# kernel-matrix-benchmarks/kernel-matrix-benchmarks

Hardware: AMD Instinct MI355X
Metric: point-pair interactions/s (N*M/s) + max |err| vs scipy, D=3 Gaussian (higher is better)
Workload: dtype f32

## Files before the change

include/kmvp.h:

```cpp
#ifndef KMVP_H
#define KMVP_H

#include <stdint.h>

#ifdef __cplusplus
extern "C" {
#endif

#define KMVP_ABI_VERSION 1

enum kmvp_status {
  KMVP_OK = 0,
  KMVP_E_INVALID = 1,
  KMVP_E_UNSUPPORTED = 2,
  KMVP_E_DEVICE = 3,
  KMVP_E_COMM = 4,
  KMVP_E_NOMEM = 5,
  KMVP_E_NOT_CONVERGED = 6
};

enum kmvp_dtype {
  KMVP_F32 = 0,
  KMVP_F64 = 1,
  KMVP_BF16 = 2
};

typedef struct kmvp_ctx kmvp_ctx;

int kmvp_abi_version(void);
int kmvp_device_count(void);

kmvp_ctx* kmvp_create(int device, int* status);
void kmvp_destroy(kmvp_ctx* ctx);
const char* kmvp_last_error(const kmvp_ctx* ctx);

int kmvp_set_points(kmvp_ctx* ctx, const void* y, int64_t M, const void* x_or_null, int64_t N,
                    int D, int dtype, int64_t j_offset, int64_t M_total);

int kmvp_fit(kmvp_ctx* ctx, int kernel);

int kmvp_set_signal(kmvp_ctx* ctx, const void* b_or_null, int E);

int kmvp_gaussian(kmvp_ctx* ctx);
int kmvp_gaussian_norm(kmvp_ctx* ctx);
int kmvp_absexp(kmvp_ctx* ctx);
int kmvp_absexp_norm(kmvp_ctx* ctx);
int kmvp_invdist(kmvp_ctx* ctx);
int kmvp_invdist_norm(kmvp_ctx* ctx);
int kmvp_expdot(kmvp_ctx* ctx);
int kmvp_expdot_norm(kmvp_ctx* ctx);
int kmvp_matern32(kmvp_ctx* ctx);
int kmvp_matern32_norm(kmvp_ctx* ctx);
int kmvp_matern52(kmvp_ctx* ctx);
int kmvp_matern52_norm(kmvp_ctx* ctx);

int kmvp_gaussian_grad(kmvp_ctx* ctx);
int kmvp_absexp_grad(kmvp_ctx* ctx);
int kmvp_invdist_grad(kmvp_ctx* ctx);
int kmvp_matern32_grad(kmvp_ctx* ctx);
int kmvp_matern52_grad(kmvp_ctx* ctx);

int kmvp_gaussian_dscale(kmvp_ctx* ctx);
int kmvp_absexp_dscale(kmvp_ctx* ctx);
int kmvp_matern32_dscale(kmvp_ctx* ctx);
int kmvp_matern52_dscale(kmvp_ctx* ctx);

int kmvp_gaussian_logsumexp(kmvp_ctx* ctx);
int kmvp_absexp_logsumexp(kmvp_ctx* ctx);

int kmvp_gaussian_logsumexp_grad(kmvp_ctx* ctx);
int kmvp_absexp_logsumexp_grad(kmvp_ctx* ctx);

int kmvp_nearest(kmvp_ctx* ctx, int K, int exclude_self, int64_t* out_idx, double* out_sqdist);

int kmvp_set_batches(kmvp_ctx* ctx, int B, const int64_t* y_offsets, const int64_t* x_offsets_or_null);

int kmvp_kmeans(kmvp_ctx* ctx, int C, const double* weights_or_null, double tol, int maxit, double* centroids,
                int64_t* labels, double* cluster_weight_or_null, int* iters, double* inertia, double* shift);

int kmvp_gaussian_meanshift(kmvp_ctx* ctx, double tol, int maxit, double* modes, int* iters, double* step2, int* sweeps,
                            int64_t* target_sweeps);

int kmvp_get_result(kmvp_ctx* ctx, double* out, int64_t out_len);

int kmvp_gaussian_cg_solve(kmvp_ctx* ctx, const void* a, int E, double rtol, int maxit,
                           double* out_b, int* iters, double* resid);
int kmvp_absexp_cg_solve(kmvp_ctx* ctx, const void* a, int E, double rtol, int maxit,
                         double* out_b, int* iters, double* resid);
int kmvp_matern32_cg_solve(kmvp_ctx* ctx, const void* a, int E, double rtol, int maxit,
                           double* out_b, int* iters, double* resid);
int kmvp_matern52_cg_solve(kmvp_ctx* ctx, const void* a, int E, double rtol, int maxit,
                           double* out_b, int* iters, double* resid);
int kmvp_invdist_minres_solve(kmvp_ctx* ctx, const void* a, int E, double rtol, int maxit,
                              double* out_b, int* iters, double* resid);

int kmvp_gaussian_lanczos_quadrature(kmvp_ctx* ctx, const void* z, int P, double rtol, int maxit, double* logquad,
                                     double* invquad, int* steps, double* x_or_null, double* alpha_or_null,
                                     double* beta_or_null);
int kmvp_absexp_lanczos_quadrature(kmvp_ctx* ctx, const void* z, int P, double rtol, int maxit, double* logquad,
                                   double* invquad, int* steps, double* x_or_null, double* alpha_or_null,
                                   double* beta_or_null);
int kmvp_matern32_lanczos_quadrature(kmvp_ctx* ctx, const void* z, int P, double rtol, int maxit, double* logquad,
                                     double* invquad, int* steps, double* x_or_null, double* alpha_or_null,
                                     double* beta_or_null);
int kmvp_matern52_lanczos_quadrature(kmvp_ctx* ctx, const void* z, int P, double rtol, int maxit, double* logquad,
                                     double* invquad, int* steps, double* x_or_null, double* alpha_or_null,
                                     double* beta_or_null);

int kmvp_gaussian_sinkhorn(kmvp_ctx* ctx, const double* log_a_or_null, const double* log_b_or_null, double tol, int maxit,
                           double* u, double* v, int* iters, double* err);
int kmvp_absexp_sinkhorn(kmvp_ctx* ctx, const double* log_a_or_null, const double* log_b_or_null, double tol, int maxit,
                         double* u, double* v, int* iters, double* err);

int kmvp_set_solver_diagonal(kmvp_ctx* ctx, const double* d_or_null, int64_t n, double ridge);

#define KMVP_PRECOND_MAX_RANK 128
int kmvp_set_solver_preconditioner(kmvp_ctx* ctx, int rank);
int kmvp_get_solver_preconditioner(kmvp_ctx* ctx, int* rank_built, int64_t* pivots_or_null, double* factor_or_null);
double kmvp_last_preconditioner_ms(const kmvp_ctx* ctx);

int kmvp_gaussian_lanczos_quadrature_precond(kmvp_ctx* ctx, const double* g, const double* h, int P, double rtol, int maxit,
                                             double* logdet_p, double* logquad, double* invquad, double* wnorm2, int* steps,
                                             double* x_or_null, double* pz_or_null, double* alpha_or_null,
                                             double* beta_or_null);
int kmvp_absexp_lanczos_quadrature_precond(kmvp_ctx* ctx, const double* g, const double* h, int P, double rtol, int maxit,
                                           double* logdet_p, double* logquad, double* invquad, double* wnorm2, int* steps,
                                           double* x_or_null, double* pz_or_null, double* alpha_or_null,
                                           double* beta_or_null);
int kmvp_matern32_lanczos_quadrature_precond(kmvp_ctx* ctx, const double* g, const double* h, int P, double rtol, int maxit,
                                             double* logdet_p, double* logquad, double* invquad, double* wnorm2, int* steps,
                                             double* x_or_null, double* pz_or_null, double* alpha_or_null,
                                             double* beta_or_null);
int kmvp_matern52_lanczos_quadrature_precond(kmvp_ctx* ctx, const double* g, const double* h, int P, double rtol, int maxit,
                                             double* logdet_p, double* logquad, double* invquad, double* wnorm2, int* steps,
                                             double* x_or_null, double* pz_or_null, double* alpha_or_null,
                                             double* beta_or_null);

enum kmvp_eig_operator { KMVP_EIG_KERNEL = 0, KMVP_EIG_CENTERED = 1, KMVP_EIG_NORMALIZED = 2 };
int kmvp_gaussian_eigsh(kmvp_ctx* ctx, int k, int op, const double* v0, double tol, int maxit, double* eigenvalues,
                        double* eigenvectors, double* resid, int* steps, double* alpha_or_null, double* beta_or_null,
                        double* degree_or_null);
int kmvp_absexp_eigsh(kmvp_ctx* ctx, int k, int op, const double* v0, double tol, int maxit, double* eigenvalues,
                      double* eigenvectors, double* resid, int* steps, double* alpha_or_null, double* beta_or_null,
                      double* degree_or_null);
int kmvp_matern32_eigsh(kmvp_ctx* ctx, int k, int op, const double* v0, double tol, int maxit, double* eigenvalues,
                        double* eigenvectors, double* resid, int* steps, double* alpha_or_null, double* beta_or_null,
                        double* degree_or_null);
int kmvp_matern52_eigsh(kmvp_ctx* ctx, int k, int op, const double* v0, double tol, int maxit, double* eigenvalues,
                        double* eigenvectors, double* resid, int* steps, double* alpha_or_null, double* beta_or_null,
                        double* degree_or_null);

#define KMVP_UNIQUE_ID_BYTES 128
int kmvp_comm_get_unique_id(void* id128);
int kmvp_comm_init(kmvp_ctx* ctx, const void* id128, int rank, int world);
int kmvp_comm_world(const kmvp_ctx* ctx);
int kmvp_comm_rank(const kmvp_ctx* ctx);
enum kmvp_reduce_op { KMVP_OP_SUM = 0, KMVP_OP_MIN = 1 };
typedef int (*kmvp_host_allreduce_fn)(void* user, double* buf, int64_t count, int op);
int kmvp_comm_init_host(kmvp_ctx* ctx, kmvp_host_allreduce_fn fn, void* user, int rank, int world);

int kmvp_set_option(kmvp_ctx* ctx, const char* key, int64_t value);

int64_t kmvp_device_bytes(const kmvp_ctx* ctx);
double kmvp_last_kernel_ms(const kmvp_ctx* ctx);
double kmvp_last_total_ms(const kmvp_ctx* ctx);
double kmvp_last_allreduce_ms(const kmvp_ctx* ctx);
const char* kmvp_last_kernel_name(const kmvp_ctx* ctx);
const char* kmvp_last_dispatch_note(const kmvp_ctx* ctx);


int kmvp_cell_layout(kmvp_ctx* ctx, int64_t* info, double* sigma_b, int32_t* source_cell, int32_t* target_cell,
                     double* source_centres, int64_t source_cap, double* target_centres, int64_t target_cap);

#ifdef __cplusplus
}
#endif
#endif
```

kernel_matrix_benchmarks_amd/_lib.py:

```python
import ctypes
import os

import numpy as np

_HERE = os.path.dirname(os.path.abspath(__file__))
LIB_PATH = os.environ.get("KMVP_LIB", os.path.join(_HERE, "libkmvp.so"))

KMVP_F32, KMVP_F64, KMVP_BF16 = 0, 1, 2
STATUS = {
    0: "OK", 1: "INVALID", 2: "UNSUPPORTED", 3: "DEVICE", 4: "COMM", 5: "NOMEM", 6: "NOT_CONVERGED",
}
UNIQUE_ID_BYTES = 128

_c = ctypes
SYMBOLS = [
    ("kmvp_abi_version", _c.c_int, []),
    ("kmvp_device_count", _c.c_int, []),
    ("kmvp_create", _c.c_void_p, [_c.c_int, _c.POINTER(_c.c_int)]),
    ("kmvp_destroy", None, [_c.c_void_p]),
    ("kmvp_last_error", _c.c_char_p, [_c.c_void_p]),
    ("kmvp_set_points", _c.c_int, [_c.c_void_p, _c.c_void_p, _c.c_int64, _c.c_void_p, _c.c_int64,
                                   _c.c_int, _c.c_int, _c.c_int64, _c.c_int64]),
    ("kmvp_fit", _c.c_int, [_c.c_void_p, _c.c_int]),
    ("kmvp_set_signal", _c.c_int, [_c.c_void_p, _c.c_void_p, _c.c_int]),
    ("kmvp_gaussian", _c.c_int, [_c.c_void_p]),
    ("kmvp_gaussian_norm", _c.c_int, [_c.c_void_p]),
    ("kmvp_absexp", _c.c_int, [_c.c_void_p]),
    ("kmvp_absexp_norm", _c.c_int, [_c.c_void_p]),
    ("kmvp_invdist", _c.c_int, [_c.c_void_p]),
    ("kmvp_invdist_norm", _c.c_int, [_c.c_void_p]),
    ("kmvp_expdot", _c.c_int, [_c.c_void_p]),
    ("kmvp_expdot_norm", _c.c_int, [_c.c_void_p]),
    ("kmvp_matern32", _c.c_int, [_c.c_void_p]),
    ("kmvp_matern32_norm", _c.c_int, [_c.c_void_p]),
    ("kmvp_matern52", _c.c_int, [_c.c_void_p]),
    ("kmvp_matern52_norm", _c.c_int, [_c.c_void_p]),
    ("kmvp_gaussian_grad", _c.c_int, [_c.c_void_p]),
    ("kmvp_absexp_grad", _c.c_int, [_c.c_void_p]),
    ("kmvp_invdist_grad", _c.c_int, [_c.c_void_p]),
    ("kmvp_matern32_grad", _c.c_int, [_c.c_void_p]),
    ("kmvp_matern52_grad", _c.c_int, [_c.c_void_p]),
    ("kmvp_gaussian_dscale", _c.c_int, [_c.c_void_p]),
    ("kmvp_absexp_dscale", _c.c_int, [_c.c_void_p]),
    ("kmvp_matern32_dscale", _c.c_int, [_c.c_void_p]),
    ("kmvp_matern52_dscale", _c.c_int, [_c.c_void_p]),
    ("kmvp_gaussian_logsumexp", _c.c_int, [_c.c_void_p]),
    ("kmvp_absexp_logsumexp", _c.c_int, [_c.c_void_p]),
    ("kmvp_gaussian_logsumexp_grad", _c.c_int, [_c.c_void_p]),
    ("kmvp_absexp_logsumexp_grad", _c.c_int, [_c.c_void_p]),
    ("kmvp_nearest", _c.c_int, [_c.c_void_p, _c.c_int, _c.c_int, _c.c_void_p, _c.c_void_p]),
    ("kmvp_set_batches", _c.c_int, [_c.c_void_p, _c.c_int, _c.c_void_p, _c.c_void_p]),
    ("kmvp_kmeans", _c.c_int, [_c.c_void_p, _c.c_int, _c.c_void_p, _c.c_double, _c.c_int, _c.c_void_p, _c.c_void_p,
                               _c.c_void_p, _c.POINTER(_c.c_int), _c.POINTER(_c.c_double), _c.POINTER(_c.c_double)]),
    ("kmvp_gaussian_meanshift", _c.c_int, [_c.c_void_p, _c.c_double, _c.c_int, _c.c_void_p, _c.c_void_p, _c.c_void_p,
                                           _c.POINTER(_c.c_int), _c.POINTER(_c.c_int64)]),
    ("kmvp_get_result", _c.c_int, [_c.c_void_p, _c.c_void_p, _c.c_int64]),
    ("kmvp_gaussian_cg_solve", _c.c_int, [_c.c_void_p, _c.c_void_p, _c.c_int, _c.c_double, _c.c_int,
                                          _c.c_void_p, _c.POINTER(_c.c_int), _c.POINTER(_c.c_double)]),
    ("kmvp_absexp_cg_solve", _c.c_int, [_c.c_void_p, _c.c_void_p, _c.c_int, _c.c_double, _c.c_int,
                                        _c.c_void_p, _c.POINTER(_c.c_int), _c.POINTER(_c.c_double)]),
    ("kmvp_matern32_cg_solve", _c.c_int, [_c.c_void_p, _c.c_void_p, _c.c_int, _c.c_double, _c.c_int,
                                          _c.c_void_p, _c.POINTER(_c.c_int), _c.POINTER(_c.c_double)]),
    ("kmvp_matern52_cg_solve", _c.c_int, [_c.c_void_p, _c.c_void_p, _c.c_int, _c.c_double, _c.c_int,
                                          _c.c_void_p, _c.POINTER(_c.c_int), _c.POINTER(_c.c_double)]),
    ("kmvp_invdist_minres_solve", _c.c_int, [_c.c_void_p, _c.c_void_p, _c.c_int, _c.c_double, _c.c_int,
                                             _c.c_void_p, _c.POINTER(_c.c_int), _c.POINTER(_c.c_double)]),
    ("kmvp_gaussian_lanczos_quadrature", _c.c_int, [_c.c_void_p, _c.c_void_p, _c.c_int, _c.c_double, _c.c_int] + [_c.c_void_p] * 6),
    ("kmvp_absexp_lanczos_quadrature", _c.c_int, [_c.c_void_p, _c.c_void_p, _c.c_int, _c.c_double, _c.c_int] + [_c.c_void_p] * 6),
    ("kmvp_matern32_lanczos_quadrature", _c.c_int, [_c.c_void_p, _c.c_void_p, _c.c_int, _c.c_double, _c.c_int] + [_c.c_void_p] * 6),
    ("kmvp_matern52_lanczos_quadrature", _c.c_int, [_c.c_void_p, _c.c_void_p, _c.c_int, _c.c_double, _c.c_int] + [_c.c_void_p] * 6),
    ("kmvp_gaussian_eigsh", _c.c_int, [_c.c_void_p, _c.c_int, _c.c_int, _c.c_void_p, _c.c_double, _c.c_int] + [_c.c_void_p] * 7),
    ("kmvp_absexp_eigsh", _c.c_int, [_c.c_void_p, _c.c_int, _c.c_int, _c.c_void_p, _c.c_double, _c.c_int] + [_c.c_void_p] * 7),
    ("kmvp_matern32_eigsh", _c.c_int, [_c.c_void_p, _c.c_int, _c.c_int, _c.c_void_p, _c.c_double, _c.c_int] + [_c.c_void_p] * 7),
    ("kmvp_matern52_eigsh", _c.c_int, [_c.c_void_p, _c.c_int, _c.c_int, _c.c_void_p, _c.c_double, _c.c_int] + [_c.c_void_p] * 7),
    ("kmvp_gaussian_lanczos_quadrature_precond", _c.c_int, [_c.c_void_p, _c.c_void_p, _c.c_void_p, _c.c_int, _c.c_double, _c.c_int] + [_c.c_void_p] * 9),
    ("kmvp_absexp_lanczos_quadrature_precond", _c.c_int, [_c.c_void_p, _c.c_void_p, _c.c_void_p, _c.c_int, _c.c_double, _c.c_int] + [_c.c_void_p] * 9),
    ("kmvp_matern32_lanczos_quadrature_precond", _c.c_int, [_c.c_void_p, _c.c_void_p, _c.c_void_p, _c.c_int, _c.c_double, _c.c_int] + [_c.c_void_p] * 9),
    ("kmvp_matern52_lanczos_quadrature_precond", _c.c_int, [_c.c_void_p, _c.c_void_p, _c.c_void_p, _c.c_int, _c.c_double, _c.c_int] + [_c.c_void_p] * 9),
    ("kmvp_gaussian_sinkhorn", _c.c_int, [_c.c_void_p, _c.c_void_p, _c.c_void_p, _c.c_double, _c.c_int, _c.c_void_p,
                                          _c.c_void_p, _c.POINTER(_c.c_int), _c.POINTER(_c.c_double)]),
    ("kmvp_absexp_sinkhorn", _c.c_int, [_c.c_void_p, _c.c_void_p, _c.c_void_p, _c.c_double, _c.c_int, _c.c_void_p,
                                        _c.c_void_p, _c.POINTER(_c.c_int), _c.POINTER(_c.c_double)]),
    ("kmvp_set_solver_diagonal", _c.c_int, [_c.c_void_p, _c.c_void_p, _c.c_int64, _c.c_double]),
    ("kmvp_set_solver_preconditioner", _c.c_int, [_c.c_void_p, _c.c_int]),
    ("kmvp_get_solver_preconditioner", _c.c_int, [_c.c_void_p, _c.POINTER(_c.c_int), _c.c_void_p, _c.c_void_p]),
    ("kmvp_last_preconditioner_ms", _c.c_double, [_c.c_void_p]),
    ("kmvp_comm_get_unique_id", _c.c_int, [_c.c_void_p]),
    ("kmvp_comm_init", _c.c_int, [_c.c_void_p, _c.c_void_p, _c.c_int, _c.c_int]),
    ("kmvp_comm_init_host", _c.c_int, [_c.c_void_p, _c.c_void_p, _c.c_void_p, _c.c_int, _c.c_int]),
    ("kmvp_comm_world", _c.c_int, [_c.c_void_p]),
    ("kmvp_comm_rank", _c.c_int, [_c.c_void_p]),
    ("kmvp_last_allreduce_ms", _c.c_double, [_c.c_void_p]),
    ("kmvp_set_option", _c.c_int, [_c.c_void_p, _c.c_char_p, _c.c_int64]),
    ("kmvp_device_bytes", _c.c_int64, [_c.c_void_p]),
    ("kmvp_last_kernel_ms", _c.c_double, [_c.c_void_p]),
    ("kmvp_last_total_ms", _c.c_double, [_c.c_void_p]),
    ("kmvp_cell_layout", _c.c_int, [_c.c_void_p, _c.c_void_p, _c.POINTER(_c.c_double), _c.c_void_p, _c.c_void_p, _c.c_void_p,
                                    _c.c_int64, _c.c_void_p, _c.c_int64]),
    ("kmvp_last_kernel_name", _c.c_char_p, [_c.c_void_p]),
    ("kmvp_last_dispatch_note", _c.c_char_p, [_c.c_void_p]),
]

HOST_ALLREDUCE_FN = _c.CFUNCTYPE(_c.c_int, _c.c_void_p, _c.POINTER(_c.c_double), _c.c_int64, _c.c_int)
OP_SUM, OP_MIN = 0, 1
FIT_CODES = {"gaussian": 0, "absolute-exponential": 1, "inverse-distance": 2, "matern-3/2": 3, "matern-5/2": 4}

EIG_OPERATORS = {"kernel": 0, "centered": 1, "normalized": 2}

_lib = None


class KmvpError(RuntimeError):
    def __init__(self, code, message):
        super().__init__(f"libkmvp: {STATUS.get(code, code)}: {message}")
        self.code = code


def load():
    global _lib
    if _lib is None:
        if not os.path.exists(LIB_PATH):
            raise ImportError(
                f"{LIB_PATH} is missing: build it with `python -c 'import __graft_entry__ as g; g.build()'` "
                "(or make -C kernel_matrix_benchmarks_amd/csrc).  There is no CPU fallback."
            )
        lib = ctypes.CDLL(LIB_PATH)
        for name, restype, argtypes in SYMBOLS:
            fn = getattr(lib, name)
            fn.restype = restype
            fn.argtypes = argtypes
        _lib = lib
    return _lib


def dtype_code(precision):
    if isinstance(precision, str) and precision.lower() in ("bfloat16", "bf16"):
        return KMVP_BF16, np.dtype(np.float32)
    dt = np.dtype(precision)
    if dt == np.float16:
        return KMVP_F32, np.dtype(np.float32)
    if dt == np.float64:
        return KMVP_F64, dt
    if dt == np.float32:
        return KMVP_F32, dt
    raise NotImplementedError(f"precision {precision!r} is not supported by the MI355X backend")


def input_rounding(precision):
    if isinstance(precision, str) and precision.lower() in ("bfloat16", "bf16"):
        return None
    return np.dtype(np.float16) if np.dtype(precision) == np.float16 else None


def batch_offsets(offsets, what, total=None):
    a = np.asarray(offsets)
    if a.ndim != 1 or a.size < 2:
        raise ValueError(f"{what} has shape {a.shape}, expected B + 1 offsets (B >= 1) in one dimension")
    if not np.issubdtype(a.dtype, np.integer):
        raise ValueError(f"{what} has dtype {a.dtype}, expected integers")
    a = np.ascontiguousarray(a, dtype=np.int64)
    if total is not None and (a[0] != 0 or np.any(np.diff(a) < 0) or a[-1] != total):
        raise ValueError(f"{what} must be non-decreasing from 0 to {total}")
    return a


class Context:

    def __init__(self, device=0):
        self._lib = load()
        status = ctypes.c_int(0)
        self._ctx = self._lib.kmvp_create(int(device), ctypes.byref(status))
        if not self._ctx:
            msg = self._lib.kmvp_last_error(None)
            raise KmvpError(status.value, msg.decode() if msg else "kmvp_create failed")
        self.device = int(device)
        self.comm_world = 0

    def _check(self, rc):
        if rc != 0:
            msg = self._lib.kmvp_last_error(self._ctx)
            raise KmvpError(rc, msg.decode() if msg else "")

    def close(self):
        if getattr(self, "_ctx", None):
            self._lib.kmvp_destroy(self._ctx)
            self._ctx = None

    def __del__(self):
        try:
            self.close()
        except Exception:
            pass

    def set_points(self, y, x, dtype_code_, j_offset=0, M_total=None):
        M, D = y.shape
        N = M if x is None else x.shape[0]
        if x is not None and x.shape[1] != D:
            raise ValueError(f"target points have {x.shape[1]} coordinates, source points {D}")
        self.M, self.N, self.D = M, N, D
        self._check(self._lib.kmvp_set_points(
            self._ctx, y.ctypes.data, M, None if x is None else x.ctypes.data, N, D, dtype_code_,
            int(j_offset), int(M if M_total is None else M_total)))

    def set_batches(self, y_offsets, x_offsets=None):
        if y_offsets is None:
            if x_offsets is not None:
                raise ValueError("target offsets without source offsets")
            self._check(self._lib.kmvp_set_batches(self._ctx, 0, None, None))
            return
        y_offsets = batch_offsets(y_offsets, "source_batches")
        if x_offsets is not None:
            x_offsets = batch_offsets(x_offsets, "target_batches")
            if x_offsets.size != y_offsets.size:
                raise ValueError(f"target_batches has {x_offsets.size} offsets, source_batches {y_offsets.size}: both hold B + 1")
        self._check(self._lib.kmvp_set_batches(self._ctx, y_offsets.size - 1, y_offsets.ctypes.data,
                                               None if x_offsets is None else x_offsets.ctypes.data))

    def fit(self, kernel):
        self._check(self._lib.kmvp_fit(self._ctx, FIT_CODES[kernel]))

    def set_signal(self, b):
        if b is None:
            self._check(self._lib.kmvp_set_signal(self._ctx, None, 1))
        else:
            if b.ndim != 2 or b.shape[0] != getattr(self, "M", b.shape[0]):
                raise ValueError(f"source_signal has shape {b.shape}, expected ({getattr(self, 'M', '?')}, E): one row per "
                                 "source point")
            self._check(self._lib.kmvp_set_signal(self._ctx, b.ctypes.data, b.shape[1]))

    def run(self, kernel, normalize_rows):
        entry = {
            ("gaussian", False): self._lib.kmvp_gaussian,
            ("gaussian", True): self._lib.kmvp_gaussian_norm,
            ("absolute-exponential", False): self._lib.kmvp_absexp,
            ("absolute-exponential", True): self._lib.kmvp_absexp_norm,
            ("inverse-distance", False): self._lib.kmvp_invdist,
            ("inverse-distance", True): self._lib.kmvp_invdist_norm,
            ("exp-dot", False): self._lib.kmvp_expdot,
            ("exp-dot", True): self._lib.kmvp_expdot_norm,
            ("matern-3/2", False): self._lib.kmvp_matern32,
            ("matern-3/2", True): self._lib.kmvp_matern32_norm,
            ("matern-5/2", False): self._lib.kmvp_matern52,
            ("matern-5/2", True): self._lib.kmvp_matern52_norm,
        }[(kernel, bool(normalize_rows))]
        self._check(entry(self._ctx))

    def run_grad(self, kernel):
        entry = {
            "gaussian": self._lib.kmvp_gaussian_grad,
            "absolute-exponential": self._lib.kmvp_absexp_grad,
            "inverse-distance": self._lib.kmvp_invdist_grad,
# ... 187 lines not shown
        def vector(a, n, what):
            if a is None:
                return None
            a = np.ascontiguousarray(a, dtype=np.float64)
            if a.shape != (n,):
                raise ValueError(f"{what} has shape {a.shape}, expected ({n},)")
            return a

        N, M = getattr(self, "N", 0), getattr(self, "M", 0)
        log_a, log_b = vector(log_a, N, "log_a"), vector(log_b, M, "log_b")
        u = np.zeros(N, dtype=np.float64) if u0 is None else vector(u0, N, "u0").copy()
        v = np.zeros(M, dtype=np.float64)
        iters = ctypes.c_int(0)
        err = ctypes.c_double(0.0)
        rc = entry(self._ctx, None if log_a is None else log_a.ctypes.data, None if log_b is None else log_b.ctypes.data,
                   float(tol), int(maxit), u.ctypes.data, v.ctypes.data, ctypes.byref(iters), ctypes.byref(err))
        if rc not in (0, 6):
            self._check(rc)
        return u, v, iters.value, err.value, rc == 0

    def kmeans(self, C, centroids0, weights, tol, maxit):
        C = int(C)
        N, D = getattr(self, "N", 0), getattr(self, "D", 0)
        cent = np.array(centroids0, dtype=np.float64, order="C", ndmin=2)
        if C >= 1 and cent.shape != (C, D):
            raise ValueError(f"the initial centroids have shape {cent.shape}, expected ({C}, {D})")
        if weights is not None:
            weights = np.ascontiguousarray(weights, dtype=np.float64)
            if weights.shape != (N,):
                raise ValueError(f"weights has shape {weights.shape}, expected ({N},)")
        labels = np.full(N, -1, dtype=np.int64)
        cluster_weight = np.zeros(max(C, 0), dtype=np.float64)
        iters = ctypes.c_int(0)
        inertia, shift = ctypes.c_double(0.0), ctypes.c_double(0.0)
        rc = self._lib.kmvp_kmeans(self._ctx, C, None if weights is None else weights.ctypes.data, float(tol), int(maxit),
                                   cent.ctypes.data, labels.ctypes.data, cluster_weight.ctypes.data, ctypes.byref(iters),
                                   ctypes.byref(inertia), ctypes.byref(shift))
        if rc not in (0, 6):
            self._check(rc)
        return cent, labels, cluster_weight, iters.value, inertia.value, shift.value, rc == 0

    def meanshift(self, tol, maxit):
        N, D = int(getattr(self, "N", 0)), int(getattr(self, "D", 0))
        modes = np.full((N, D), np.nan, dtype=np.float64)
        iters = np.zeros(N, dtype=np.intc)
        step2 = np.full(N, np.nan, dtype=np.float64)
        sweeps = ctypes.c_int(0)
        target_sweeps = ctypes.c_int64(0)
        rc = self._lib.kmvp_gaussian_meanshift(self._ctx, float(tol), int(maxit), modes.ctypes.data, iters.ctypes.data,
                                               step2.ctypes.data, ctypes.byref(sweeps), ctypes.byref(target_sweeps))
        if rc not in (0, 6):
            self._check(rc)
        return {"modes": modes, "iters": iters.astype(np.int64), "step2": step2, "sweeps": sweeps.value,
                "target_sweeps": target_sweeps.value, "converged": rc == 0}

    def set_solver_diagonal(self, d_or_none, ridge=0.0):
        if d_or_none is None:
            self._check(self._lib.kmvp_set_solver_diagonal(self._ctx, None, 0, float(ridge)))
            return
        d = np.ascontiguousarray(d_or_none, dtype=np.float64)
        if d.ndim != 1:
            raise ValueError(f"the solver diagonal has shape {d.shape}, expected one value per point")
        self._check(self._lib.kmvp_set_solver_diagonal(self._ctx, d.ctypes.data, d.size, float(ridge)))

    def set_solver_preconditioner(self, rank):
        self._check(self._lib.kmvp_set_solver_preconditioner(self._ctx, int(rank)))

    def get_solver_preconditioner(self):
        built = ctypes.c_int(0)
        self._check(self._lib.kmvp_get_solver_preconditioner(self._ctx, ctypes.byref(built), None, None))
        pivots = np.empty(built.value, dtype=np.int64)
        factor = np.empty((built.value, int(getattr(self, "N", 0))), dtype=np.float64)
        if built.value:
            self._check(self._lib.kmvp_get_solver_preconditioner(self._ctx, ctypes.byref(built), pivots.ctypes.data,
                                                                 factor.ctypes.data))
        return built.value, pivots, factor

    @property
    def last_preconditioner_rank(self):
        built = ctypes.c_int(0)
        self._check(self._lib.kmvp_get_solver_preconditioner(self._ctx, ctypes.byref(built), None, None))
        return built.value

    @property
    def last_preconditioner_ms(self):
        return float(self._lib.kmvp_last_preconditioner_ms(self._ctx))

    def comm_init(self, unique_id, rank, world):
        buf = (ctypes.c_char * UNIQUE_ID_BYTES).from_buffer_copy(unique_id)
        self._check(self._lib.kmvp_comm_init(self._ctx, buf, int(rank), int(world)))
        self.comm_world = int(world)

    def comm_init_host(self, allreduce, rank, world):

        def trampoline(_user, buf, count, op):
            try:
                allreduce(np.ctypeslib.as_array(buf, shape=(int(count),)), int(op))
                return 0
            except Exception as e:
                self._host_error = e
                return 1

        self._host_cb = HOST_ALLREDUCE_FN(trampoline)
        self._check(self._lib.kmvp_comm_init_host(self._ctx, ctypes.cast(self._host_cb, ctypes.c_void_p), None,
                                                  int(rank), int(world)))
        self.comm_world = int(world)

    @property
    def rccl_ranks(self):
        return int(self._lib.kmvp_comm_world(self._ctx))

    @property
    def last_allreduce_ms(self):
        return float(self._lib.kmvp_last_allreduce_ms(self._ctx))

    def set_option(self, key, value):
        self._check(self._lib.kmvp_set_option(self._ctx, key.encode(), int(value)))

    @property
    def device_bytes(self):
        return int(self._lib.kmvp_device_bytes(self._ctx))

    @property
    def last_kernel_ms(self):
        return float(self._lib.kmvp_last_kernel_ms(self._ctx))

    @property
    def last_total_ms(self):
        return float(self._lib.kmvp_last_total_ms(self._ctx))

    @property
    def last_kernel_name(self):
        return self._lib.kmvp_last_kernel_name(self._ctx).decode()

    @property
    def last_dispatch_note(self):
        return self._lib.kmvp_last_dispatch_note(self._ctx).decode()

    def cell_layout(self):
        if not self._ctx:
            raise ValueError("the context is closed")
        info = np.zeros(8, dtype=np.int64)
        sigma = ctypes.c_double(0.0)
        self._check(self._lib.kmvp_cell_layout(self._ctx, info.ctypes.data, ctypes.byref(sigma), None, None, None, 0, None, 0))
        ns, nt = int(info[0]), int(info[1])
        scell, tcell = np.empty(self.M, dtype=np.int32), np.empty(self.N, dtype=np.int32)
        scen, tcen = np.empty((max(ns, 1), 3)), np.empty((max(nt, 1), 3))
        self._check(self._lib.kmvp_cell_layout(self._ctx, info.ctypes.data, ctypes.byref(sigma), scell.ctypes.data,
                                               tcell.ctypes.data, scen.ctypes.data, ns, tcen.ctypes.data, nt))
        return {"source_cell": scell, "target_cell": tcell, "source_centres": scen[:ns], "target_centres": tcen[:nt],
                "count_cut": bool(info[2]), "tiles_per_wavefront": int(info[3]), "tile_points": int(info[4]),
                "image": int(info[5]), "main_tiles": int(info[6]), "rest_tiles": int(info[7]), "sigma_b": float(sigma.value)}


def comm_unique_id():
    buf = ctypes.create_string_buffer(UNIQUE_ID_BYTES)
    rc = load().kmvp_comm_get_unique_id(buf)
    if rc != 0:
        msg = load().kmvp_last_error(None)
        raise KmvpError(rc, msg.decode() if msg else "")
    return bytes(buf.raw)


def device_count():
    n = load().kmvp_device_count()
    return max(0, n)
```

kernel_matrix_benchmarks_amd/csrc/kmvp_api.hip:

```cpp
#include "kmvp_ctx.hpp"

namespace kmvp {

Rccl g_rccl;

namespace {
thread_local std::string g_create_error;
}

int fail(kmvp_ctx* c, int code, const std::string& msg) {
  if (c) c->err = msg;
  else g_create_error = msg;
  return code;
}
const char* create_error() { return g_create_error.c_str(); }

int ensure(kmvp_ctx* c, DevBuf& b, size_t bytes) {
  if (bytes <= b.cap && b.p) return KMVP_OK;
  if (b.p) {
    HIP_TRY(c, hipFree(b.p));
    b.p = nullptr;
    b.cap = 0;
  }
  if (bytes == 0) bytes = 16;
  HIP_TRY(c, hipMalloc(&b.p, bytes));
  b.cap = bytes;
  return KMVP_OK;
}

void release(DevBuf& b) {
  if (b.p) (void)hipFree(b.p);
  b.p = nullptr;
  b.cap = 0;
}

}

using namespace kmvp;

extern "C" {

int kmvp_abi_version(void) { return KMVP_ABI_VERSION; }

int kmvp_device_count(void) {
  int n = 0;
  if (hipGetDeviceCount(&n) != hipSuccess) return -KMVP_E_DEVICE;
  return n;
}

kmvp_ctx* kmvp_create(int device, int* status) {
  int n = 0;
  hipError_t e = hipGetDeviceCount(&n);
  if (e != hipSuccess || n <= 0) {
    fail(nullptr, KMVP_E_DEVICE, std::string("no HIP device: ") + hipGetErrorString(e));
    if (status) *status = KMVP_E_DEVICE;
    return nullptr;
  }
  if (device < 0 || device >= n) {
    fail(nullptr, KMVP_E_INVALID, "device index out of range");
    if (status) *status = KMVP_E_INVALID;
    return nullptr;
  }
  kmvp_ctx* c = new kmvp_ctx();
  c->device = device;
  bool ok = hipSetDevice(device) == hipSuccess &&
            hipStreamCreateWithFlags(&c->stream, hipStreamNonBlocking) == hipSuccess;
  for (int i = 0; ok && i < 5; ++i) ok = hipEventCreate(&c->ev[i]) == hipSuccess;
  if (!ok) {
    fail(nullptr, KMVP_E_DEVICE, "cannot create stream/events on the device");
    if (status) *status = KMVP_E_DEVICE;
    kmvp_destroy(c);
    return nullptr;
  }
  if (status) *status = KMVP_OK;
  return c;
}

void kmvp_destroy(kmvp_ctx* c) {
  if (!c) return;
  (void)hipSetDevice(c->device);
  if (c->stream) (void)hipStreamSynchronize(c->stream);
  if (c->comm && g_rccl.CommDestroy) g_rccl.CommDestroy(c->comm);
  for (DevBuf* b : {&c->y_raw, &c->x_raw, &c->b_raw, &c->xs, &c->rec, &c->x_scaled, &c->y_scaled,
                    &c->part, &c->partd, &c->aux, &c->sortbuf, &c->perm, &c->sums, &c->out, &c->scratch, &c->sdiag, &c->precond, &c->knn, &c->xchg, &c->kexp, &c->kshift, &c->xchgk, &c->kflag,
                    &c->sk_xs_x, &c->sk_rec_y, &c->sk_xs_y, &c->sk_rec_x, &c->sk_state, &c->km_xs, &c->km_rec, &c->km_part, &c->km_state, &c->ms_xs, &c->ms_state, &c->ms_tmp, &c->bt_tiles, &c->bt_tmap, &c->bt_smap, &c->bt_xs, &c->bt_rec,
                    &c->cell_tperm, &c->cell_sperm, &c->cell_tgrp, &c->cell_sgrp, &c->cell_slot, &c->cell_tmeta, &c->cell_sums, &c->cell_skey, &c->cell_scentre, &c->cell_scale, &c->cell_tcentre, &c->cell_scentre32})
    release(*b);
  for (int i = 0; i < 5; ++i)
    if (c->ev[i]) (void)hipEventDestroy(c->ev[i]);
  if (c->stream) (void)hipStreamDestroy(c->stream);
  delete c;
}

const char* kmvp_last_error(const kmvp_ctx* c) { return c ? c->err.c_str() : create_error(); }

int kmvp_set_points(kmvp_ctx* c, const void* y, int64_t M, const void* x_or_null, int64_t N, int D,
                    int dtype, int64_t j_offset, int64_t M_total) {
  if (!c) return KMVP_E_INVALID;
  if (dtype != KMVP_F32 && dtype != KMVP_F64 && dtype != KMVP_BF16)
    return fail(c, KMVP_E_INVALID, "unknown dtype");
  if (M < 0 || N < 0 || D < 1) return fail(c, KMVP_E_INVALID, "bad shape");
  if ((M > 0 && !y) || (N > 0 && !x_or_null && N != M))
    return fail(c, KMVP_E_INVALID, "same_points (x == NULL) needs N == M");
  if (M_total < M || j_offset < 0 || j_offset + M > M_total)
    return fail(c, KMVP_E_INVALID, "shard [j_offset, j_offset+M) is outside [0, M_total)");
  HIP_TRY(c, hipSetDevice(c->device));
  const size_t es = elem_size(dtype);
  int rc;
  if ((rc = ensure(c, c->y_raw, (size_t)M * D * es))) return rc;
  if (M > 0) HIP_TRY(c, hipMemcpyAsync(c->y_raw.p, y, (size_t)M * D * es, hipMemcpyHostToDevice, c->stream));
  c->same_points = (x_or_null == nullptr);
  if (!c->same_points) {
    if ((rc = ensure(c, c->x_raw, (size_t)N * D * es))) return rc;
    if (N > 0) HIP_TRY(c, hipMemcpyAsync(c->x_raw.p, x_or_null, (size_t)N * D * es, hipMemcpyHostToDevice, c->stream));
  }
  if ((rc = measure_clouds(c, dtype, M, N, D))) return rc;
  HIP_TRY(c, hipStreamSynchronize(c->stream));
  c->dtype = dtype;
  c->D = D;
  c->M = M;
  c->N = N;
  c->j_offset = j_offset;
  c->m_total = M_total;
  c->have_points = true;
  c->have_signal = false;
  c->diag_on = false;
  c->diag_n = 0;
  c->diag_ridge = c->diag_min = 0.0;
  c->precond_rank = 0;
  c->pc_used = 0;
  c->bt_on = false;
  c->bt_B = 0;
  ++c->points_ver;
  return KMVP_OK;
}

int kmvp_fit(kmvp_ctx* c, int kernel) {
  if (!c) return KMVP_E_INVALID;
  if (!c->have_points) return fail(c, KMVP_E_INVALID, "kmvp_set_points has not been called");
  if (kernel < 0 || kernel > 4) return fail(c, KMVP_E_INVALID, "kernel must be 0, 1, 2, 3 or 4");
  if (kernel > 2) return KMVP_OK;
  HIP_TRY(c, hipSetDevice(c->device));
  return prepare_points(c, kernel);
}

int kmvp_set_signal(kmvp_ctx* c, const void* b_or_null, int E) {
  if (!c) return KMVP_E_INVALID;
  if (!c->have_points) return fail(c, KMVP_E_INVALID, "kmvp_set_points must come first");
  if (E < 1) return fail(c, KMVP_E_INVALID, "E must be >= 1");
  if (!b_or_null && E != 1) return fail(c, KMVP_E_INVALID, "density estimation (b == NULL) needs E == 1");
  HIP_TRY(c, hipSetDevice(c->device));
  c->density = (b_or_null == nullptr);
  c->E = E;
  if (!c->density) {
    const size_t bytes = (size_t)c->M * E * elem_size(c->dtype);
    int rc = ensure(c, c->b_raw, bytes);
    if (rc) return rc;
    if (bytes) HIP_TRY(c, hipMemcpyAsync(c->b_raw.p, b_or_null, bytes, hipMemcpyHostToDevice, c->stream));
    HIP_TRY(c, hipStreamSynchronize(c->stream));
  }
  c->have_signal = true;
  ++c->signal_ver;
  return KMVP_OK;
}

static inline bool batched(const kmvp_ctx* c) { return c && c->bt_on; }
#define KMVP_NOT_BATCHED(c, what)                   \
  do {                                              \
    if (int rc_ = batches_refuse((c), (what))) return rc_; \
  } while (0)

int kmvp_set_batches(kmvp_ctx* c, int B, const int64_t* y_offsets, const int64_t* x_offsets_or_null) {
  return set_batches(c, B, y_offsets, x_offsets_or_null);
}

int kmvp_gaussian(kmvp_ctx* c) { return batched(c) ? run_product_batched(c, K_GAUSSIAN, false) : run_product(c, K_GAUSSIAN, false); }
int kmvp_gaussian_norm(kmvp_ctx* c) { return batched(c) ? run_product_batched(c, K_GAUSSIAN, true) : run_product(c, K_GAUSSIAN, true); }
int kmvp_absexp(kmvp_ctx* c) { return batched(c) ? run_product_batched(c, K_ABSEXP, false) : run_product(c, K_ABSEXP, false); }
int kmvp_absexp_norm(kmvp_ctx* c) { return batched(c) ? run_product_batched(c, K_ABSEXP, true) : run_product(c, K_ABSEXP, true); }
int kmvp_invdist(kmvp_ctx* c) { KMVP_NOT_BATCHED(c, "the inverse-distance product"); return run_product(c, K_INVDIST, false); }
int kmvp_invdist_norm(kmvp_ctx* c) { KMVP_NOT_BATCHED(c, "the inverse-distance product"); return run_product(c, K_INVDIST, true); }
int kmvp_expdot(kmvp_ctx* c) { KMVP_NOT_BATCHED(c, "exp(<x,y>)"); return run_product(c, K_EXPDOT, false); }
int kmvp_expdot_norm(kmvp_ctx* c) { KMVP_NOT_BATCHED(c, "exp(<x,y>)"); return run_product(c, K_EXPDOT, true); }
int kmvp_matern32(kmvp_ctx* c) { return batched(c) ? run_product_batched(c, K_MATERN32, false) : run_product(c, K_MATERN32, false); }
int kmvp_matern32_norm(kmvp_ctx* c) { return batched(c) ? run_product_batched(c, K_MATERN32, true) : run_product(c, K_MATERN32, true); }
int kmvp_matern52(kmvp_ctx* c) { return batched(c) ? run_product_batched(c, K_MATERN52, false) : run_product(c, K_MATERN52, false); }
int kmvp_matern52_norm(kmvp_ctx* c) { return batched(c) ? run_product_batched(c, K_MATERN52, true) : run_product(c, K_MATERN52, true); }
int kmvp_gaussian_grad(kmvp_ctx* c) { KMVP_NOT_BATCHED(c, "the gradient"); return run_gradient(c, K_GAUSSIAN); }
int kmvp_absexp_grad(kmvp_ctx* c) { KMVP_NOT_BATCHED(c, "the gradient"); return run_gradient(c, K_ABSEXP); }
int kmvp_invdist_grad(kmvp_ctx* c) { KMVP_NOT_BATCHED(c, "the gradient"); return run_gradient(c, K_INVDIST); }
int kmvp_matern32_grad(kmvp_ctx* c) { KMVP_NOT_BATCHED(c, "the gradient"); return run_gradient(c, K_MATERN32); }
int kmvp_matern52_grad(kmvp_ctx* c) { KMVP_NOT_BATCHED(c, "the gradient"); return run_gradient(c, K_MATERN52); }
int kmvp_gaussian_dscale(kmvp_ctx* c) { KMVP_NOT_BATCHED(c, "the length-scale derivative"); return run_dscale(c, K_GAUSSIAN); }
int kmvp_absexp_dscale(kmvp_ctx* c) { KMVP_NOT_BATCHED(c, "the length-scale derivative"); return run_dscale(c, K_ABSEXP); }
int kmvp_matern32_dscale(kmvp_ctx* c) { KMVP_NOT_BATCHED(c, "the length-scale derivative"); return run_dscale(c, K_MATERN32); }
int kmvp_matern52_dscale(kmvp_ctx* c) { KMVP_NOT_BATCHED(c, "the length-scale derivative"); return run_dscale(c, K_MATERN52); }
int kmvp_gaussian_logsumexp(kmvp_ctx* c) { KMVP_NOT_BATCHED(c, "the log-sum-exp"); return run_logsumexp(c, K_GAUSSIAN); }
int kmvp_absexp_logsumexp(kmvp_ctx* c) { KMVP_NOT_BATCHED(c, "the log-sum-exp"); return run_logsumexp(c, K_ABSEXP); }
int kmvp_gaussian_logsumexp_grad(kmvp_ctx* c) { KMVP_NOT_BATCHED(c, "the gradient of the log-sum-exp"); return run_logsumexp_grad(c, K_GAUSSIAN); }
int kmvp_absexp_logsumexp_grad(kmvp_ctx* c) { KMVP_NOT_BATCHED(c, "the gradient of the log-sum-exp"); return run_logsumexp_grad(c, K_ABSEXP); }
int kmvp_nearest(kmvp_ctx* c, int K, int exclude_self, int64_t* out_idx, double* out_sqdist) {
  if (batched(c)) return run_nearest_batched(c, K, exclude_self, out_idx, out_sqdist);
  return run_nearest(c, K, exclude_self, out_idx, out_sqdist);
}
int kmvp_kmeans(kmvp_ctx* c, int C, const double* weights, double tol, int maxit, double* centroids, int64_t* labels,
                double* cluster_weight, int* iters, double* inertia, double* shift) {
  KMVP_NOT_BATCHED(c, "k-means");
  return kmeans_solve(c, C, weights, tol, maxit, centroids, labels, cluster_weight, iters, inertia, shift);
}
int kmvp_gaussian_meanshift(kmvp_ctx* c, double tol, int maxit, double* modes, int* iters, double* step2, int* sweeps,
                            int64_t* target_sweeps) {
  KMVP_NOT_BATCHED(c, "mean-shift");
  return meanshift_solve(c, tol, maxit, modes, iters, step2, sweeps, target_sweeps);
}

int kmvp_get_result(kmvp_ctx* c, double* out, int64_t out_len) {
  if (!c) return KMVP_E_INVALID;
  const int64_t n = c->out_n * c->out_e;
  if (!c->out.p && n > 0) return fail(c, KMVP_E_INVALID, "no result: run a product first");
  if (out_len < n || (n > 0 && !out)) return fail(c, KMVP_E_INVALID, "output buffer too small");
// ... 74 lines not shown
    return cg_lanczos_precond(c, K, g, h, P, rtol, maxit, logdet_p, logquad, invquad, wnorm2, steps, x, pz, alpha, beta);    \
  }
KMVP_LANCZOS_PRECOND_ENTRY(gaussian, K_GAUSSIAN)
KMVP_LANCZOS_PRECOND_ENTRY(absexp, K_ABSEXP)
KMVP_LANCZOS_PRECOND_ENTRY(matern32, K_MATERN32)
KMVP_LANCZOS_PRECOND_ENTRY(matern52, K_MATERN52)
#undef KMVP_LANCZOS_PRECOND_ENTRY

int kmvp_gaussian_sinkhorn(kmvp_ctx* c, const double* log_a, const double* log_b, double tol, int maxit, double* u, double* v,
                           int* iters, double* err) {
  KMVP_NOT_BATCHED(c, "the Sinkhorn iteration");
  return sinkhorn_solve(c, K_GAUSSIAN, log_a, log_b, tol, maxit, u, v, iters, err);
}
int kmvp_absexp_sinkhorn(kmvp_ctx* c, const double* log_a, const double* log_b, double tol, int maxit, double* u, double* v,
                         int* iters, double* err) {
  KMVP_NOT_BATCHED(c, "the Sinkhorn iteration");
  return sinkhorn_solve(c, K_ABSEXP, log_a, log_b, tol, maxit, u, v, iters, err);
}

int kmvp_set_solver_diagonal(kmvp_ctx* c, const double* d, int64_t n, double ridge) {
  if (!c) return KMVP_E_INVALID;
  if (!std::isfinite(ridge)) return fail(c, KMVP_E_INVALID, "solver diagonal: ridge is not finite");
  if (n < 0 || (d == nullptr) != (n == 0)) return fail(c, KMVP_E_INVALID, "solver diagonal: pass n values, or NULL and n = 0");
  ++c->diag_ver;
  if (!d) {
    c->diag_on = ridge != 0.0;
    c->diag_n = 0;
    c->diag_ridge = c->diag_min = ridge;
    return KMVP_OK;
  }
  std::vector<double> eff((size_t)n);
  double lo = INFINITY;
  for (int64_t i = 0; i < n; ++i) {
    eff[i] = ridge + d[i];
    if (!std::isfinite(eff[i])) return fail(c, KMVP_E_INVALID, "solver diagonal: d[" + std::to_string(i) + "] is not finite");
    lo = std::min(lo, eff[i]);
  }
  HIP_TRY(c, hipSetDevice(c->device));
  if (int rc = ensure(c, c->sdiag, sizeof(double) * (size_t)n)) return rc;
  c->diag_on = false;
  HIP_TRY(c, hipMemcpyAsync(c->sdiag.p, eff.data(), sizeof(double) * (size_t)n, hipMemcpyHostToDevice, c->stream));
  HIP_TRY(c, hipStreamSynchronize(c->stream));
  c->diag_on = true;
  c->diag_n = n;
  c->diag_ridge = ridge;
  c->diag_min = lo;
  return KMVP_OK;
}

int kmvp_set_solver_preconditioner(kmvp_ctx* c, int rank) {
  if (!c) return KMVP_E_INVALID;
  if (rank < 0) return fail(c, KMVP_E_INVALID, "preconditioner: rank must be >= 0");
  if (rank > KMVP_PRECOND_MAX_RANK)
    return fail(c, KMVP_E_UNSUPPORTED, "preconditioner: rank " + std::to_string(rank) + " is beyond " + std::to_string(KMVP_PRECOND_MAX_RANK));
  c->precond_rank = rank;
  return KMVP_OK;
}
int kmvp_get_solver_preconditioner(kmvp_ctx* c, int* rank_built, int64_t* pivots, double* factor) {
  return precond_read(c, rank_built, pivots, factor);
}
double kmvp_last_preconditioner_ms(const kmvp_ctx* c) { return c ? c->last_precond_ms : 0.0; }

int kmvp_comm_get_unique_id(void* id128) {
  if (!id128) return KMVP_E_INVALID;
  if (!g_rccl.load()) return fail(nullptr, KMVP_E_COMM, g_rccl.error);
  static_assert(sizeof(ncclUniqueId) == KMVP_UNIQUE_ID_BYTES, "ncclUniqueId size");
  ncclUniqueId id;
  ncclResult_t r = g_rccl.GetUniqueId(&id);
  if (r != ncclSuccess) return fail(nullptr, KMVP_E_COMM, std::string("ncclGetUniqueId: ") + g_rccl.GetErrorString(r));
  memcpy(id128, &id, sizeof(id));
  return KMVP_OK;
}

int kmvp_comm_init(kmvp_ctx* c, const void* id128, int rank, int world) {
  if (!c || !id128 || world < 1 || rank < 0 || rank >= world) return fail(c, KMVP_E_INVALID, "bad communicator arguments");
  if (!g_rccl.load()) return fail(c, KMVP_E_COMM, g_rccl.error);
  HIP_TRY(c, hipSetDevice(c->device));
  if (c->comm) {
    g_rccl.CommDestroy(c->comm);
    c->comm = nullptr;
  }
  c->host_xchg = nullptr;
  c->host_user = nullptr;
  ncclUniqueId id;
  memcpy(&id, id128, sizeof(id));
  ncclResult_t r = g_rccl.CommInitRank(&c->comm, world, id, rank);
  if (r != ncclSuccess) {
    c->comm = nullptr;
    return fail(c, KMVP_E_COMM, std::string("ncclCommInitRank: ") + g_rccl.GetErrorString(r));
  }
  int count = -1, user_rank = -1, dev = -1;
  ncclResult_t r1 = g_rccl.CommCount(c->comm, &count);
  ncclResult_t r2 = g_rccl.CommUserRank(c->comm, &user_rank);
  (void)g_rccl.CommCuDevice(c->comm, &dev);
  if (r1 != ncclSuccess || r2 != ncclSuccess || count != world || user_rank != rank) {
    g_rccl.CommDestroy(c->comm);
    c->comm = nullptr;
    c->comm_count = 1;
    c->rank = 0;
    c->world = 1;
    return fail(c, KMVP_E_COMM, "RCCL communicator mismatch: asked for rank " + std::to_string(rank) + " of " +
                                    std::to_string(world) + " on device " + std::to_string(c->device) + ", RCCL reports rank " +
                                    std::to_string(user_rank) + " of " + std::to_string(count) + " on device " +
                                    std::to_string(dev));
  }
  c->comm_count = count;
  c->rank = rank;
  c->world = world;
  return KMVP_OK;
}

int kmvp_comm_init_host(kmvp_ctx* c, kmvp_host_allreduce_fn fn, void* user, int rank, int world) {
  if (!c || !fn || world < 1 || rank < 0 || rank >= world) return fail(c, KMVP_E_INVALID, "bad communicator arguments");
  if (c->comm) {
    g_rccl.CommDestroy(c->comm);
    c->comm = nullptr;
  }
  c->host_xchg = fn;
  c->host_user = user;
  c->comm_count = world;
  c->rank = rank;
  c->world = world;
  return KMVP_OK;
}

int kmvp_comm_world(const kmvp_ctx* c) { return (c && c->exchanges()) ? c->comm_count : 1; }
int kmvp_comm_rank(const kmvp_ctx* c) { return (c && c->exchanges()) ? c->rank : 0; }

int kmvp_set_option(kmvp_ctx* c, const char* key, int64_t value) {
  if (!c || !key) return KMVP_E_INVALID;
  const std::string k(key);
  if (k == "feed") {
    if (value < -1 || value > 1) return fail(c, KMVP_E_INVALID, "feed must be -1 (auto), 0 or 1");
    c->opt_feed = (int)value;
  } else if (k == "targets_per_lane") {
    if (value != 0 && value != 1 && value != 2 && value != 4 && value != 8)
      return fail(c, KMVP_E_INVALID, "targets_per_lane must be 0 (auto), 1, 2, 4 or 8");
    c->opt_T = (int)value;
  } else if (k == "segments") {
    if (value < 0 || value > 65535) return fail(c, KMVP_E_INVALID, "segments out of range");
    c->opt_segments = (int)value;
  } else if (k == "fast_sqdists") {
    if (value < -1 || value > 4) return fail(c, KMVP_E_INVALID, "fast_sqdists must be -1 (auto), 0, 1, 2, 3 or 4");
    c->opt_fast = (int)value;
  } else if (k == "cellmm_shape") {
    if (value < -1 || value > 1) return fail(c, KMVP_E_INVALID, "cellmm_shape must be -1 (by size), 0 (32x32x16) or 1 (16x16x32)");
    c->opt_cellmm_shape = (int)value;
  } else if (k == "cell_fused") {
    if (value < -1 || value > 1) return fail(c, KMVP_E_INVALID, "cell_fused must be -1 (automatic), 0 (two launches) or 1 (one launch where it applies)");
    c->opt_cell_fused = (int)value;
  } else if (k == "cell_balance") {
    if (value < -1 || value > 1) return fail(c, KMVP_E_INVALID, "cell_balance must be -1 (automatic), 0 (never) or 1 (wherever count-cut cells apply)");
    c->opt_cell_balance = (int)value;
  } else if (k == "cell_shared_build") {
    if (value < -1 || value > 1) return fail(c, KMVP_E_INVALID, "cell_shared_build must be -1 (automatic), 0 (never) or 1 (wherever a workgroup is one-cell)");
    c->opt_cell_shared_build = (int)value;
  } else if (k == "mfma_variant") {
    if (value != -1 && value != 0 && value != 1 && value != 4 && value != 5)
      return fail(c, KMVP_E_INVALID, "mfma_variant must be -1 (by kernel), 0, 1, 4 or 5");
    c->opt_mfma_variant = (int)value;
  } else if (k == "same_points_global") {
    c->opt_same_global = value != 0;
  } else if (k == "partial_shard") {
    c->opt_partial = value != 0;
  } else if (k == "fast_tiles") {
    if (value != 0 && value != 1 && value != 2 && value != 4 && value != 8)
      return fail(c, KMVP_E_INVALID, "fast_tiles must be 0 (auto), 1, 2, 4 or 8");
    c->opt_fast_tiles = (int)value;
  } else if (k == "meanshift_compact") {
    if (value < -1 || value > 1) return fail(c, KMVP_E_INVALID, "meanshift_compact must be -1 (default), 0 or 1");
    c->opt_meanshift_compact = (int)value;
  } else if (k == "chunk") {
    if (value < 8 || value > (1 << 24)) return fail(c, KMVP_E_INVALID, "chunk out of range");
    c->opt_chunk = (int)value;
  } else {
    return fail(c, KMVP_E_INVALID, "unknown option " + k);
  }
  return KMVP_OK;
}

int64_t kmvp_device_bytes(const kmvp_ctx* c) {
  if (!c) return 0;
  size_t t = 0;
  for (const DevBuf* b : {&c->y_raw, &c->x_raw, &c->b_raw, &c->xs, &c->rec, &c->x_scaled,
                          &c->y_scaled, &c->part, &c->partd, &c->aux, &c->sortbuf, &c->perm, &c->sums, &c->out, &c->scratch, &c->sdiag, &c->precond, &c->knn, &c->xchg, &c->kexp, &c->kshift, &c->xchgk, &c->kflag,
                    &c->sk_xs_x, &c->sk_rec_y, &c->sk_xs_y, &c->sk_rec_x, &c->sk_state, &c->km_xs, &c->km_rec, &c->km_part, &c->km_state, &c->ms_xs, &c->ms_state, &c->ms_tmp, &c->bt_tiles, &c->bt_tmap, &c->bt_smap, &c->bt_xs, &c->bt_rec,
                          &c->cell_tperm, &c->cell_sperm, &c->cell_tgrp, &c->cell_sgrp, &c->cell_slot, &c->cell_tmeta, &c->cell_sums, &c->cell_skey, &c->cell_scentre, &c->cell_scale, &c->cell_tcentre, &c->cell_scentre32})
    t += b->cap;
  return (int64_t)t;
}
double kmvp_last_kernel_ms(const kmvp_ctx* c) { return c ? c->last_kernel_ms : 0.0; }
double kmvp_last_total_ms(const kmvp_ctx* c) { return c ? c->last_total_ms : 0.0; }
double kmvp_last_allreduce_ms(const kmvp_ctx* c) { return c ? c->last_allreduce_ms : 0.0; }
int kmvp_cell_layout(kmvp_ctx* c, int64_t* info, double* sigma_b, int32_t* source_cell, int32_t* target_cell,
                     double* source_centres, int64_t source_cap, double* target_centres, int64_t target_cap) {
  if (!c) return KMVP_E_INVALID;
  return cell_layout_read(c, info, sigma_b, source_cell, target_cell, source_centres, source_cap, target_centres, target_cap);
}
const char* kmvp_last_kernel_name(const kmvp_ctx* c) { return c ? c->last_kernel_name : ""; }
const char* kmvp_last_dispatch_note(const kmvp_ctx* c) { return c ? c->note.c_str() : ""; }

}
```

kernel_matrix_benchmarks_amd/csrc/kmvp_cellmm.hpp:

```cpp
#pragma once
#include <hip/hip_runtime.h>
#include <stdint.h>

#include "kmvp_cell.hpp"

namespace kmvp {

#ifndef CMM_BF16
#define CMM_BF16 0
#endif
#if CMM_BF16
typedef __bf16 cmm_half;
#else
typedef _Float16 cmm_half;
#endif
typedef cmm_half f16x8 __attribute__((ext_vector_type(8)));
typedef cmm_half f16x2 __attribute__((ext_vector_type(2)));

constexpr int CMM_STAGE_TILES = 12;
constexpr int CMM_STAGE_BYTES = 8192;
constexpr int CMM_E_OFF = 0;
constexpr int CMM_B_OFF = CMM_STAGE_TILES * CELL_TILE * 16;
constexpr int CMM_HDR_OFF = CMM_B_OFF + CMM_STAGE_TILES * CELL_TILE * 4;
static_assert(CMM_HDR_OFF + CMM_STAGE_TILES * 16 <= CMM_STAGE_BYTES, "stage image too small");
// ... 142 lines not shown
  float S0c = 0.f;
  float D1[3] = {0.f, 0.f, 0.f};

  auto fold = [&]() {
    const float s0 = cellmm_half_sum(S0) * CMM_TARGET_SCALE;
#pragma unroll
    for (int tt = 0; tt < TT; ++tt) {
      const f32x16 d = acc[tt];
      f32x2 p0 = f32x2{d[0], d[1]} + f32x2{d[2], d[3]};
      f32x2 p1 = f32x2{d[4], d[5]} + f32x2{d[6], d[7]};
      f32x2 p2 = f32x2{d[8], d[9]} + f32x2{d[10], d[11]};
      f32x2 p3 = f32x2{d[12], d[13]} + f32x2{d[14], d[15]};
      p0 = p0 + p1;
      p2 = p2 + p3;
      p0 = p0 + p2;
      const float v = cellmm_cross_half_add(p0[0] + p0[1]);
      outd[tt] += (double)(U[tt] * ((v - vprev[tt]) + s0));
      vprev[tt] = v;
    }
    S0 = 0.f;
    S0c = 0.f;
  };
  auto new_cell = [&](const f32x4 cs, int ks) {
    if (key_s >= 0) fold();
    key_s = ks;
#pragma unroll
    for (int c = 0; c < 3; ++c) D1[c] = (cT[c] - cs[c]) * LOG2E;
#pragma unroll
    for (int tt = 0; tt < TT; ++tt) {
      f32x4 dv;
      if constexpr (!HOLD_D) dv = *reinterpret_cast<const f32x4*>(&dsh[wave][tt][r][0]);
      float s2 = 0.f;
#pragma unroll
      for (int c = 0; c < 3; ++c) {
        float df;
        if constexpr (HOLD_D) df = dl[tt][c] + (cT[c] - cs[c]);
        else df = dv[c] + (cT[c] - cs[c]);
        s2 = fmaf(df, df, s2);
      }
      U[tt] = kexp2(s2 * -LOG2E);
    }
  };

  for (int64_t s = s_begin; s < s_end; ++s) {
    const int buf = (int)((s - s_begin) & 1);
    if (s + 1 < s_end) fetch(s + 1);
    const unsigned char* base = &lds[buf][0];
    const unsigned char* p_ef = base + CMM_E_OFF + r * 16;
    const unsigned char* p_b = base + CMM_B_OFF + r * 4;
    const f32x4* hdr = reinterpret_cast<const f32x4*>(base + CMM_HDR_OFF);
#pragma unroll 1
    for (int q = 0; q < CMM_STAGE_TILES; ++q) {
      const f32x4 cs = hdr[q];
      const int ks = __builtin_amdgcn_readfirstlane(__float_as_int(cs[3]));
      if (ks < 0) break;
      if (ks != key_s) new_cell(cs, ks);
      const f32x4 ef = *reinterpret_cast<const f32x4*>(p_ef);
      const float bq = *reinterpret_cast<const float*>(p_b);
      p_ef += CELL_TILE * 16;
      p_b += CELL_TILE * 4;
      const f32x4 a14 = h ? f32x4{ef[2], ef[0] * ef[2], ef[2] * ef[2], ef[0] * ef[1]}
                          : f32x4{ef[0], ef[1], ef[0] * ef[0], ef[1] * ef[1]};
      const float a5 = h ? ef[1] * ef[2] : ef[1];
      const float arg = fmaf(ef[0], D1[0], fmaf(ef[1], D1[1], fmaf(ef[2], D1[2], ef[3])));
      const float wb = kexp2(arg) * bq;
      {
        const float yk = wb - S0c;
        const float tk = S0 + yk;
        S0c = (tk - S0) - yk;
        S0 = tk;
      }
      const float u1 = a14[0] * wb, u2 = a14[1] * wb;
      const f16x2 R0 = cellmm_pk(u1, u2);
      const float c1 = (float)R0[0], c2 = (float)R0[1];
      const f16x2 R1 = cellmm_pk(u1 - c1, u2 - c2);
      const f16x2 R3 = cellmm_pk(a14[2] * wb, a14[3] * wb);
      const f16x2 R2 = cellmm_pk(c1, a5 * wb);
      i32x4 yw;
      yw[0] = __builtin_bit_cast(int, R0);
      yw[1] = __builtin_bit_cast(int, R1);
      yw[2] = __builtin_bit_cast(int, R2);
      yw[3] = __builtin_bit_cast(int, R3);
      const f16x8 ya = __builtin_bit_cast(f16x8, yw);
#pragma unroll
      for (int tt = 0; tt < TT; ++tt) {
#if CMM_BF16
        acc[tt] = __builtin_amdgcn_mfma_f32_32x32x16_bf16(ya, xb[tt], acc[tt], 0, 0, 0);
#else
        acc[tt] = __builtin_amdgcn_mfma_f32_32x32x16_f16(ya, xb[tt], acc[tt], 0, 0, 0);
#endif
      }
    }
    if (s + 1 < s_end) commit(buf ^ 1);
    __syncthreads();
  }
  if (key_s >= 0) fold();

  const double inv = (double)a.scale[1];
#pragma unroll
  for (int tt = 0; tt < TT; ++tt)
    if (h == 0) a.part[(int64_t)seg * a.n_slots + (tile0 + tt - a.tile_base) * CELL_TILE + r] = outd[tt] * inv;
}


__device__ __forceinline__ float cellmm16_fold4(float a, float b, float c, float d) {
  const auto p = __builtin_amdgcn_permlane16_swap(__float_as_uint(a), __float_as_uint(b), false, false);
  const float w0 = __uint_as_float(p[0]) + __uint_as_float(p[1]);
  const auto q = __builtin_amdgcn_permlane16_swap(__float_as_uint(c), __float_as_uint(d), false, false);
  const float w1 = __uint_as_float(q[0]) + __uint_as_float(q[1]);
  const auto r = __builtin_amdgcn_permlane32_swap(__float_as_uint(w0), __float_as_uint(w1), false, false);
  return __uint_as_float(r[0]) + __uint_as_float(r[1]);
}
__device__ __forceinline__ float cellmm16_sources_sum(float v) {
  v += cellmm_dpp<0x111, 0xf>(v);
  v += cellmm_dpp<0x112, 0xf>(v);
  v += cellmm_dpp<0x114, 0xf>(v);
  v += cellmm_dpp<0x118, 0xf>(v);
  return __int_as_float(__builtin_amdgcn_readlane(__float_as_int(v), 15)) +
         __int_as_float(__builtin_amdgcn_readlane(__float_as_int(v), 47));
}

__device__ __forceinline__ void cellmm16_operand(const f32x4 ef, float bq, float d1x, float d1y, float d1z, int h, f16x8& ya,
                                                 float& wexp) {
  const float m0 = h ? ef[2] : ef[0];
  const float m1 = h ? ef[0] : ef[1];
  const float m2 = h ? ef[2] : 1.f;
  const f32x4 a14 = f32x4{m0, m1 * m2, m0 * m0, m1 * ef[1]};
  const float a5 = ef[1] * m2;
  const float arg = fmaf(ef[0], d1x, fmaf(ef[1], d1y, fmaf(ef[2], d1z, ef[3])));
  wexp = kexp2(arg);
  const float wb = wexp * bq;
  const float u1 = a14[0] * wb, u2 = a14[1] * wb;
  const f16x2 R0 = cellmm_pk(u1, u2);
  const float c1 = (float)R0[0], c2 = (float)R0[1];
  const f16x2 R1 = cellmm_pk(fmaf(a14[0], wb, -c1), fmaf(a14[1], wb, -c2));
  const f16x2 R3 = cellmm_pk(a14[2] * wb, a14[3] * wb);
  const f16x2 R2 = cellmm_pk(c1, a5 * wb);
  i32x4 yw;
  yw[0] = __builtin_bit_cast(int, R0);
  yw[1] = __builtin_bit_cast(int, R1);
  yw[2] = __builtin_bit_cast(int, R2);
  yw[3] = __builtin_bit_cast(int, R3);
  ya = __builtin_bit_cast(f16x8, yw);
}
__device__ __forceinline__ void cellmm16_weight_sum(float bq, float wexp, float& S0, float& S0c) {
  const float yk = fmaf(bq, wexp, -S0c);
  const float tk = S0 + yk;
  S0c = (tk - S0) - yk;
  S0 = tk;
}

#ifndef CMM16_NOFOLD
#define CMM16_NOFOLD 0
#endif
#ifndef CMM16_BUILD_PROBE
#define CMM16_BUILD_PROBE 0
#endif

constexpr int CMM16_ABUF_BYTES = CMM_STAGE_TILES * 64 * 16;
constexpr int CMM16_WBUF_OFF = 2 * CMM16_ABUF_BYTES;
constexpr int CMM16_WBUF_BYTES = CMM_STAGE_TILES * CELL_TILE * 8;
constexpr int CMM16_SHARED_LDS_BYTES = CMM16_WBUF_OFF + 2 * CMM16_WBUF_BYTES;
constexpr int CMM16_SHARED_OWN = CMM_STAGE_TILES / WAVES_PER_BLOCK;
static_assert(CMM_STAGE_TILES % WAVES_PER_BLOCK == 0 && CMM_STAGE_TILES <= 64, "a stage's tiles: equal shares, one header lane each");
constexpr bool cellmm16_has_shared(int TT) { return TT >= 8; }
constexpr int cellmm16_lds_bytes(int TT) { return cellmm16_has_shared(TT) ? CMM16_SHARED_LDS_BYTES : 2 * CMM_STAGE_BYTES; }

template <int TT, bool SHARED>
__device__ __forceinline__ void cellmm16_body(const CellmmArgs& a, int bid, unsigned char* lds) {
  static_assert(!CMM_BF16, "f16 operands only");
  static_assert(!SHARED || cellmm16_has_shared(TT), "no shared-build body at this tile count");
  constexpr int SB = CMM_STAGE_BYTES;
  constexpr int PIECES = SB / (16 * BLOCK_THREADS);
  constexpr float LOG2E = 1.4426950408889634f;
  constexpr int HT = 2 * TT;
  constexpr int NG = (HT + 3) / 4;
  constexpr int OWN = CMM16_SHARED_OWN;

  int tb, seg;
  block_to_work(bid, a.segments, a.tile_blocks, tb, seg);
  const int lane = threadIdx.x & 63;
  const int wave = threadIdx.x >> 6;
  const int cc = lane & 15;
  const int kg = lane >> 4;
  const int h = kg & 1;
  const int rs = 16 * (kg >> 1) + cc;
  const int64_t tile0 = a.tile_base + ((int64_t)tb * WAVES_PER_BLOCK + wave) * TT;

  float cT[3];
  f16x8 xb[HT];
#pragma unroll
  for (int u = 0; u < HT; ++u) {
    const f32x4 v = *reinterpret_cast<const f32x4*>(a.xd + ((tile0 + (u >> 1)) * CELL_TILE + 16 * (u & 1) + cc) * 4);
    xb[u] = cellmm_target_operand(v, h);
  }
  {
    const f32x4 m = *reinterpret_cast<const f32x4*>(a.tmeta + tile0 * 4);
#pragma unroll
    for (int c = 0; c < 3; ++c) cT[c] = __int_as_float(__builtin_amdgcn_readfirstlane(__float_as_int(m[c])));
  }
  float dl[NG][3], U[NG], vprev[NG];
  double outd[NG];
#pragma unroll
  for (int g = 0; g < NG; ++g) {
    const int u = 4 * g + kg < HT ? 4 * g + kg : HT - 1;
    const f32x4 v = *reinterpret_cast<const f32x4*>(a.xd + ((tile0 + (u >> 1)) * CELL_TILE + 16 * (u & 1) + cc) * 4);
#pragma unroll
    for (int c = 0; c < 3; ++c) dl[g][c] = v[c];
    U[g] = 0.f;
    vprev[g] = 0.f;
    outd[g] = 0.0;
  }

  f32x4 acc[HT];
#pragma unroll
  for (int u = 0; u < HT; ++u)
#pragma unroll
    for (int k = 0; k < 4; ++k) acc[u][k] = 0.f;

  const int64_t s_begin = (int64_t)seg * a.seg_stages;
  int64_t s_end = s_begin + a.seg_stages;
  if (s_end > a.m_stages) s_end = a.m_stages;

  f32x4 pre[SHARED ? 1 : PIECES];
  auto fetch = [&](int64_t s) {
    const unsigned char* src = a.img + s * SB;
#pragma unroll
    for (int p = 0; p < PIECES; ++p)
      pre[p] = *reinterpret_cast<const f32x4*>(src + (p * BLOCK_THREADS + (int)threadIdx.x) * 16);
  };
  auto commit = [&](int buf) {
#pragma unroll
    for (int p = 0; p < PIECES; ++p)
      *reinterpret_cast<f32x4*>(lds + buf * SB + (p * BLOCK_THREADS + (int)threadIdx.x) * 16) = pre[p];
  };

  const int wave_u = __builtin_amdgcn_readfirstlane(wave);
  const int hl = lane < CMM_STAGE_TILES ? lane : 0;
  f32x4 raw_ef[SHARED ? OWN : 1];
  float raw_b[SHARED ? OWN : 1];
  f32x4 hcur = {0.f, 0.f, 0.f, 0.f}, hnext = hcur, hfar = hcur;
  auto load_hdr = [&](int64_t s) { return *reinterpret_cast<const f32x4*>(a.img + s * SB + CMM_HDR_OFF + hl * 16); };
  auto load_raw = [&](int64_t s, int j) {
    const unsigned char* src = a.img + s * SB;
    const int row = (wave_u * OWN + j) * CELL_TILE + rs;
    raw_ef[j] = *reinterpret_cast<const f32x4*>(src + CMM_E_OFF + row * 16);
    raw_b[j] = *reinterpret_cast<const float*>(src + CMM_B_OFF + row * 4);
  };
  auto build_tile = [&](int buf, const f32x4 hd, int j) {
    const int t = wave_u * OWN + j;
    if (__builtin_amdgcn_readlane(__float_as_int(hd[3]), t) < 0) return;
    float d1[3];
#pragma unroll
    for (int c = 0; c < 3; ++c)
      d1[c] = (cT[c] - __int_as_float(__builtin_amdgcn_readlane(__float_as_int(hd[c]), t))) * LOG2E;
    f16x8 ya;
    float wexp;
    cellmm16_operand(raw_ef[j], raw_b[j], d1[0], d1[1], d1[2], h, ya, wexp);
    *reinterpret_cast<f16x8*>(lds + buf * CMM16_ABUF_BYTES + (t * 64 + lane) * 16) = ya;
    if (h == 0)
      *reinterpret_cast<f32x2*>(lds + CMM16_WBUF_OFF + buf * CMM16_WBUF_BYTES + (t * CELL_TILE + rs) * 8) = f32x2{raw_b[j], wexp};
  };

  if constexpr (SHARED) {
    if (s_begin < s_end) {
      hcur = load_hdr(s_begin);
#pragma unroll
      for (int j = 0; j < OWN; ++j) load_raw(s_begin, j);
#pragma unroll
      for (int j = 0; j < OWN; ++j) build_tile(0, hcur, j);
      if (s_begin + 1 < s_end) {
        hnext = load_hdr(s_begin + 1);
#pragma unroll
        for (int j = 0; j < OWN; ++j) load_raw(s_begin + 1, j);
      }
    }
  } else {
    if (s_begin < s_end) {
      fetch(s_begin);
      commit(0);
    }
  }
  __syncthreads();

  int key_s = -2;
  float S0 = 0.f, S0c = 0.f;
  float D1[3] = {0.f, 0.f, 0.f};
#if CMM16_BUILD_PROBE
  f16x8 ya_probe = {};
  float wexp_probe = 0.f;
#endif

  auto fold = [&]() {
#if CMM16_NOFOLD
    asm volatile("" ::"v"(S0), "v"(S0c));
#else
    const float s0 = cellmm16_sources_sum(S0) * CMM_TARGET_SCALE;
    float x[4 * NG];
#pragma unroll
    for (int u = 0; u < 4 * NG; ++u) x[u] = u < HT ? (acc[u][0] + acc[u][1]) + (acc[u][2] + acc[u][3]) : 0.f;
#pragma unroll
    for (int g = 0; g < NG; ++g) {
      const float v = cellmm16_fold4(x[4 * g], x[4 * g + 1], x[4 * g + 2], x[4 * g + 3]);
      outd[g] += (double)(U[g] * ((v - vprev[g]) + s0));
      vprev[g] = v;
    }
#endif
    S0 = 0.f;
    S0c = 0.f;
  };
  auto new_cell = [&](const f32x4 cs, int ks) {
    if (key_s >= 0) fold();
    key_s = ks;
#pragma unroll
    for (int c = 0; c < 3; ++c) D1[c] = (cT[c] - cs[c]) * LOG2E;
#if !CMM16_NOFOLD
#pragma unroll
    for (int g = 0; g < NG; ++g) {
      float s2 = 0.f;
#pragma unroll
      for (int c = 0; c < 3; ++c) {
        const float df = dl[g][c] + (cT[c] - cs[c]);
        s2 = fmaf(df, df, s2);
      }
      U[g] = kexp2(s2 * -LOG2E);
    }
#endif
  };

  for (int64_t s = s_begin; s < s_end; ++s) {
    const int buf = (int)((s - s_begin) & 1);
    if constexpr (SHARED) {
      if (s + 1 < s_end) {
#pragma unroll
        for (int j = 0; j < OWN; ++j) build_tile(buf ^ 1, hnext, j);
      }
      if (s + 2 < s_end) {
        hfar = load_hdr(s + 2);
#pragma unroll
        for (int j = 0; j < OWN; ++j) load_raw(s + 2, j);
      }
      const unsigned char* p_ya = lds + buf * CMM16_ABUF_BYTES + lane * 16;
      const unsigned char* p_w = lds + CMM16_WBUF_OFF + buf * CMM16_WBUF_BYTES + rs * 8;
      const int keys = lane < CMM_STAGE_TILES ? __float_as_int(hcur[3]) : -1;
#pragma unroll 1
      for (int q = 0; q < CMM_STAGE_TILES; ++q) {
        const int ks = __builtin_amdgcn_readlane(keys, q);
        if (ks < 0) break;
        if (ks != key_s) {
          f32x4 cs;
#pragma unroll
          for (int c = 0; c < 3; ++c) cs[c] = __int_as_float(__builtin_amdgcn_readlane(__float_as_int(hcur[c]), q));
          cs[3] = 0.f;
          new_cell(cs, ks);
        }
        const f16x8 ya = *reinterpret_cast<const f16x8*>(p_ya);
        const f32x2 w = *reinterpret_cast<const f32x2*>(p_w);
        p_ya += 64 * 16;
        p_w += CELL_TILE * 8;
        cellmm16_weight_sum(w[0], w[1], S0, S0c);
#pragma unroll
        for (int u = 0; u < HT; ++u) acc[u] = __builtin_amdgcn_mfma_f32_16x16x32_f16(ya, xb[u], acc[u], 0, 0, 0);
      }
      hcur = hnext;
      hnext = hfar;
    } else {
      if (s + 1 < s_end) fetch(s + 1);
      const unsigned char* base = lds + buf * SB;
      const unsigned char* p_ef = base + CMM_E_OFF + rs * 16;
      const unsigned char* p_b = base + CMM_B_OFF + rs * 4;
      const f32x4* hdr = reinterpret_cast<const f32x4*>(base + CMM_HDR_OFF);
      const int keys = lane < CMM_STAGE_TILES ? __float_as_int(hdr[hl][3]) : -1;
#pragma unroll 1
      for (int q = 0; q < CMM_STAGE_TILES; ++q) {
        const int ks = __builtin_amdgcn_readlane(keys, q);
        if (ks < 0) break;
        if (ks != key_s) new_cell(hdr[q], ks);
        const f32x4 ef = *reinterpret_cast<const f32x4*>(p_ef);
        const float bq = *reinterpret_cast<const float*>(p_b);
        p_ef += CELL_TILE * 16;
        p_b += CELL_TILE * 4;
#if CMM16_BUILD_PROBE
        if ((q & 3) == wave_u) {
          cellmm16_operand(ef, bq, D1[0], D1[1], D1[2], h, ya_probe, wexp_probe);
        } else {
          asm volatile("" ::"v"(ef[0]), "v"(ef[1]), "v"(ef[2]), "v"(ef[3]));
        }
        asm volatile("" ::"v"(bq), "v"(S0));
        const f16x8 ya = ya_probe;
        const float wexp = wexp_probe;
#else
        f16x8 ya;
        float wexp;
        cellmm16_operand(ef, bq, D1[0], D1[1], D1[2], h, ya, wexp);
#endif
        cellmm16_weight_sum(bq, wexp, S0, S0c);
#pragma unroll
        for (int u = 0; u < HT; ++u) acc[u] = __builtin_amdgcn_mfma_f32_16x16x32_f16(ya, xb[u], acc[u], 0, 0, 0);
      }
      if (s + 1 < s_end) commit(buf ^ 1);
    }
    __syncthreads();
  }
  if (key_s >= 0) fold();
#if CMM16_NOFOLD
#pragma unroll
  for (int u = 0; u < HT; ++u) asm volatile("" ::"v"(acc[u][0]), "v"(acc[u][1]), "v"(acc[u][2]), "v"(acc[u][3]));
#endif

  const double inv = (double)a.scale[1];
#pragma unroll
  for (int g = 0; g < NG; ++g)
    if (4 * g + kg < HT)
      a.part[(int64_t)seg * a.n_slots + (tile0 + 2 * g + (kg >> 1) - a.tile_base) * CELL_TILE + 16 * h + cc] = outd[g] * inv;
}

template <int TT>
__device__ __forceinline__ bool cellmm16_one_cell(const CellmmArgs& a, int bid) {
  int tb, seg;
  block_to_work(bid, a.segments, a.tile_blocks, tb, seg);
  const int* m = reinterpret_cast<const int*>(a.tmeta) + (a.tile_base + (int64_t)tb * WAVES_PER_BLOCK * TT) * 4;
  int differ = 0;
#pragma unroll
  for (int w = 1; w < WAVES_PER_BLOCK; ++w)
#pragma unroll
    for (int c = 0; c < 3; ++c) differ |= m[(int64_t)w * TT * 4 + c] ^ m[c];
  return __builtin_amdgcn_readfirstlane(differ) == 0;
}

template <int TT>
__global__ void __launch_bounds__(BLOCK_THREADS) __attribute__((amdgpu_waves_per_eu(TT >= 8 ? 2 : 1)))
cellmm16_kernel(const CellmmArgs a, const CellmmArgs rest, const int main_grid) {
  __shared__ __attribute__((aligned(16))) unsigned char lds[cellmm16_lds_bytes(TT)];
  if constexpr (TT > CELL_REST_TT) {
    const FusedCellWork w = fused_cell_work((int64_t)blockIdx.x, (int64_t)main_grid);
    if (w.list) {
      cellmm16_body<CELL_REST_TT, false>(rest, (int)w.local, lds);
      return;
    }
  }
  if constexpr (cellmm16_has_shared(TT)) {
    if (a.shared_build && cellmm16_one_cell<TT>(a, (int)blockIdx.x)) {
      cellmm16_body<TT, true>(a, (int)blockIdx.x, lds);
      return;
    }
  }
  cellmm16_body<TT, false>(a, (int)blockIdx.x, lds);
}

hipError_t launch_cellmm_gaussian(int TT, int shape, const CellmmArgs& args, dim3 grid, hipStream_t stream, const char** kernel_name);
hipError_t launch_cellmm16_fused(int TT, const CellmmArgs& main, const CellmmArgs& rest, int64_t main_grid, int64_t rest_grid,
                                 hipStream_t stream, const char** kernel_name);

}
```

kernel_matrix_benchmarks_amd/csrc/kmvp_cellmm_inst.hip:

```cpp
#include <stdlib.h>
#include "kmvp_internal.hpp"
#include "kmvp_cellmm.hpp"

namespace kmvp {

static size_t cmm_dbg_lds() {
  static const size_t v = getenv("KMVP_DBG_LDS") ? (size_t)atol(getenv("KMVP_DBG_LDS")) : 0;
  return v;
}
template <typename K, typename... Rest>
static void cmm_launch(K kernel, const CellmmArgs& args, dim3 grid, hipStream_t stream, Rest... rest) {
  if (cmm_dbg_lds()) (void)hipFuncSetAttribute((const void*)kernel, hipFuncAttributeMaxDynamicSharedMemorySize, (int)cmm_dbg_lds());
  hipLaunchKernelGGL(kernel, grid, dim3(BLOCK_THREADS), cmm_dbg_lds(), stream, args, rest...);
}

hipError_t launch_cellmm_gaussian(int TT, int shape, const CellmmArgs& args, dim3 grid, hipStream_t stream, const char** kernel_name) {
  if (kernel_name) *kernel_name = shape == 1 ? "cellmm16_kernel" : "cellmm_kernel";
  if (shape == 1) {
    const int all = (int)grid.x;
    switch (TT) {
      case 1: cmm_launch(cellmm16_kernel<1>, args, grid, stream, args, all); break;
      case 2: cmm_launch(cellmm16_kernel<2>, args, grid, stream, args, all); break;
      case 4: cmm_launch(cellmm16_kernel<4>, args, grid, stream, args, all); break;
      case 8: cmm_launch(cellmm16_kernel<8>, args, grid, stream, args, all); break;
      default: return hipErrorInvalidValue;
    }
    return hipGetLastError();
  }
  switch (TT) {
    case 1: cmm_launch(cellmm_kernel<1>, args, grid, stream); break;
    case 2: cmm_launch(cellmm_kernel<2>, args, grid, stream); break;
    case 4: cmm_launch(cellmm_kernel<4>, args, grid, stream); break;
    case 8: cmm_launch(cellmm_kernel<8>, args, grid, stream); break;
    default: return hipErrorInvalidValue;
  }
  return hipGetLastError();
}

hipError_t launch_cellmm16_fused(int TT, const CellmmArgs& main, const CellmmArgs& rest, int64_t main_grid, int64_t rest_grid,
                                 hipStream_t stream, const char** kernel_name) {
  if (kernel_name) *kernel_name = "cellmm16_kernel";
  if (main_grid + rest_grid > MAX_GRID) return hipErrorInvalidConfiguration;
  const dim3 grid((unsigned)(main_grid + rest_grid));
  switch (TT) {
    case 4: cmm_launch(cellmm16_kernel<4>, main, grid, stream, rest, (int)main_grid); break;
    case 8: cmm_launch(cellmm16_kernel<8>, main, grid, stream, rest, (int)main_grid); break;
    default: return hipErrorInvalidValue;
  }
  return hipGetLastError();
}

}
```

kernel_matrix_benchmarks_amd/csrc/kmvp_ctx.hpp:

```cpp
#pragma once
#include <dlfcn.h>
#include <hip/hip_runtime.h>
#include <rccl/rccl.h>
#include <stdint.h>
#include <stdlib.h>
#include <string.h>

#include <algorithm>
#include <cmath>
#include <string>
#include <vector>

#include "../../include/kmvp.h"
#include "kmvp_internal.hpp"

namespace kmvp {

enum : int { LAYOUT_LOWD = 0, LAYOUT_FAST = 1, LAYOUT_MFMA = 2, LAYOUT_CFAST = 3, LAYOUT_CELL = 4, LAYOUT_CELL64 = 5, LAYOUT_CELLMM = 6, LAYOUT_FASTMM = 7, LAYOUT_CFASTMM = 8 };

struct DevBuf {
  void* p = nullptr;
  size_t cap = 0;
};

struct Rccl {
  void* handle = nullptr;
  ncclResult_t (*GetUniqueId)(ncclUniqueId*) = nullptr;
  ncclResult_t (*CommInitRank)(ncclComm_t*, int, ncclUniqueId, int) = nullptr;
  ncclResult_t (*AllReduce)(const void*, void*, size_t, ncclDataType_t, ncclRedOp_t, ncclComm_t,
                            hipStream_t) = nullptr;
  ncclResult_t (*CommDestroy)(ncclComm_t) = nullptr;
  ncclResult_t (*CommCount)(const ncclComm_t, int*) = nullptr;
  ncclResult_t (*CommUserRank)(const ncclComm_t, int*) = nullptr;
  ncclResult_t (*CommCuDevice)(const ncclComm_t, int*) = nullptr;
  const char* (*GetErrorString)(ncclResult_t) = nullptr;
  std::string error, path;
  bool load() {
    if (handle) return true;
    std::vector<std::string> names;
    Dl_info info;
    if (dladdr((void*)&hipGetDeviceCount, &info) && info.dli_fname) {
      char resolved[4096];
      std::string hip_path = realpath(info.dli_fname, resolved) ? resolved : info.dli_fname;
      const size_t slash = hip_path.rfind('/');
      if (slash != std::string::npos) {
        const std::string dir = hip_path.substr(0, slash + 1);
        names.push_back(dir + "librccl.so.1");
        names.push_back(dir + "librccl.so");
      }
    }
    names.push_back("librccl.so.1");
    names.push_back("librccl.so");
    names.push_back("/opt/rocm/lib/librccl.so.1");
    for (const std::string& n : names) {
      handle = dlopen(n.c_str(), RTLD_NOW | RTLD_LOCAL);
      if (handle) {
        path = n;
        break;
      }
    }
    if (!handle) {
      error = std::string("cannot load librccl: ") + dlerror();
      return false;
    }
    GetUniqueId = (decltype(GetUniqueId))dlsym(handle, "ncclGetUniqueId");
    CommInitRank = (decltype(CommInitRank))dlsym(handle, "ncclCommInitRank");
    AllReduce = (decltype(AllReduce))dlsym(handle, "ncclAllReduce");
    CommDestroy = (decltype(CommDestroy))dlsym(handle, "ncclCommDestroy");
    GetErrorString = (decltype(GetErrorString))dlsym(handle, "ncclGetErrorString");
    CommCount = (decltype(CommCount))dlsym(handle, "ncclCommCount");
    CommUserRank = (decltype(CommUserRank))dlsym(handle, "ncclCommUserRank");
    CommCuDevice = (decltype(CommCuDevice))dlsym(handle, "ncclCommCuDevice");
    if (!GetUniqueId || !CommInitRank || !AllReduce || !CommDestroy || !GetErrorString || !CommCount || !CommUserRank ||
        !CommCuDevice) {
      error = "librccl lacks an expected symbol";
      return false;
    }
    return true;
  }
};extern Rccl g_rccl;

}

struct kmvp_ctx {
  using DevBuf = kmvp::DevBuf;
  int device = 0;
  hipStream_t stream = nullptr;
  hipEvent_t ev[5] = {nullptr, nullptr, nullptr, nullptr, nullptr};
  std::string err;

  int dtype = -1;
  int D = 0, E = 0;
  int64_t M = 0, N = 0, j_offset = 0, m_total = 0;
  bool same_points = false;
  bool have_points = false, have_signal = false, density = false;
  bool async_product = false;
  bool diag_on = false;
  int64_t diag_n = 0;
  double diag_ridge = 0.0, diag_min = 0.0;

  DevBuf y_raw, x_raw, b_raw;
  DevBuf xs, rec;
  DevBuf partd;
  DevBuf aux;
  DevBuf sortbuf, perm;
  DevBuf x_scaled, y_scaled;
  DevBuf cell_tperm, cell_sperm, cell_tgrp, cell_sgrp, cell_slot, cell_tmeta, cell_sums, cell_skey, cell_scentre, cell_scale;
  DevBuf cell_tcentre, cell_scentre32;
  DevBuf part, sums, out;
  DevBuf xchg;
  DevBuf kexp, kshift, xchgk;
  DevBuf kflag;
  DevBuf scratch;
  DevBuf knn;
  DevBuf sdiag;
  DevBuf precond;
  int precond_rank = 0;
  int pc_built = 0;
  int pc_used = 0;
  int pc_kernel = -1, pc_rank = 0;
  uint64_t pc_points_ver = 0, pc_diag_ver = 0;
  uint64_t diag_ver = 0;
  float last_precond_ms = 0.f;
  double pc_logdet_c = 0.0;
  DevBuf sk_xs_x, sk_rec_y, sk_xs_y, sk_rec_x, sk_state;
  uint64_t sk_points_ver = 0;
  DevBuf km_xs, km_rec, km_part, km_state;
  uint64_t km_points_ver = 0;
  DevBuf ms_xs, ms_state, ms_tmp;
  DevBuf bt_tiles, bt_tmap, bt_smap, bt_xs, bt_rec;
  bool bt_on = false;
  int bt_B = 0;
  int64_t bt_n_pad = 0, bt_m_alloc = 0;
  uint64_t bt_ver = 0;
  uint64_t bt_xs_points_ver = 0, bt_xs_ver = 0;
  uint64_t bt_rec_points_ver = 0, bt_rec_ver = 0;
  int bt_rec_R = 0;
  uint64_t bt_sig_ver = 0;
  int bt_sig_EB = -1;
  uint64_t points_ver = 0, signal_ver = 0;
  int packed_layout = -1;
  int packed_kernel = -1, packed_sig = -1, packed_T = -1;
  uint64_t packed_points_ver = 0, packed_signal_ver = 0;
  int gen_kernel = -1;
  uint64_t gen_points_ver = 0;
  int64_t out_n = 0;
  int out_e = 0;

  int opt_feed = -1, opt_T = 0, opt_segments = 0, opt_chunk = 512;
  int opt_fast = -1, opt_fast_tiles = 0;
  int opt_cellmm_shape = -1;
  int opt_cell_shared_build = -1;
  int opt_cell_balance = -1;
  int opt_cell_fused = -1;
  int opt_mfma_variant = -1;
  int opt_meanshift_compact = -1;
  int opt_same_global = 0;
  int opt_partial = 0;
  uint64_t perm_ver = 0;
  uint64_t cell_ver = 0;
  int cell_state = 0;
  int cell_balance_req = -1;
  bool cell_balanced = false;
  float cell_zw = 0.f;
  int cell_tt = 0, cell_tt_req = 0;
  float cell_lo[3] = {0.f, 0.f, 0.f}, cell_hh[3] = {1.f, 1.f, 1.f};
  int cell_g[3] = {1, 1, 1};
  int64_t cell_n_tiles = 0, cell_m_tiles = 0;
  int64_t cell_n_main = 0, cell_n_rest = 0;
  float cloud_radius2 = INFINITY;
  uint64_t centre_ver = 0;

  ncclComm_t comm = nullptr;
  int rank = 0, world = 1;
  kmvp_host_allreduce_fn host_xchg = nullptr;
  void* host_user = nullptr;
  std::vector<double> host_buf;
  bool exchanges() const { return comm != nullptr || host_xchg != nullptr; }

  int comm_count = 1;
  float last_kernel_ms = 0.f, last_total_ms = 0.f, last_allreduce_ms = 0.f;
  const char* last_kernel_name = "";
  std::string note;
};

namespace kmvp {

int fail(kmvp_ctx* c, int code, const std::string& msg);
const char* create_error();

#define HIP_TRY(c, expr)                                                                     \
  do {                                                                                       \
    hipError_t e_ = (expr);                                                                  \
    if (e_ != hipSuccess)                                                                    \
      return kmvp::fail((c), e_ == hipErrorOutOfMemory ? KMVP_E_NOMEM : KMVP_E_DEVICE,       \
                        std::string(#expr) + ": " + hipGetErrorString(e_));                  \
  } while (0)

inline size_t elem_size(int dtype) { return dtype == KMVP_F64 ? 8 : 4; }
inline unsigned blocks_for(int64_t n, int threads = 256) { return (unsigned)((n + threads - 1) / threads); }

int ensure(kmvp_ctx* c, DevBuf& b, size_t bytes);
void release(DevBuf& b);

struct PackKey {
  int layout, kernel, T;
};
inline bool points_stale(const kmvp_ctx* c, PackKey k) {
  return c->packed_points_ver != c->points_ver || c->packed_kernel != k.kernel || c->packed_layout != k.layout ||
         c->packed_T != k.T;
}
inline bool signal_stale(const kmvp_ctx* c, PackKey k, int sig) {
  return points_stale(c, k) || sig < 0 || c->packed_signal_ver != c->signal_ver || c->packed_sig != sig;
}
inline void record_packed(kmvp_ctx* c, PackKey k, int sig) {
  c->packed_points_ver = c->points_ver;
  c->packed_signal_ver = c->signal_ver;
  c->packed_layout = k.layout;
  c->packed_kernel = k.kernel;
  c->packed_T = k.T;
  c->packed_sig = sig;
}

int run_product(kmvp_ctx* c, int kernel, bool normalise);
int measure_clouds(kmvp_ctx* c, int dtype, int64_t M, int64_t N, int D);
int prepare_points(kmvp_ctx* c, int kernel);
int run_gradient(kmvp_ctx* c, int kernel);
int run_dscale(kmvp_ctx* c, int kernel);
int run_logsumexp(kmvp_ctx* c, int kernel);
int run_logsumexp_grad(kmvp_ctx* c, int kernel);
int run_nearest(kmvp_ctx* c, int K, int exclude_self, int64_t* out_idx, double* out_sqdist);

struct Diag {
  const double* dg;
  double ridge;
  __device__ __forceinline__ double at(int64_t i) const { return dg ? dg[i] : ridge; }
};
inline Diag solver_diag(const kmvp_ctx* c) { return Diag{c->diag_n ? (const double*)c->sdiag.p : nullptr, c->diag_ridge}; }

int precond_prepare(kmvp_ctx* c, int kernel);
constexpr int PC_APPLY_BLOCKS = 256;
inline size_t precond_scratch(int R, int E) { return (size_t)(PC_APPLY_BLOCKS + 1) * (size_t)R * (size_t)E; }
void precond_apply(kmvp_ctx* c, const double* r, double* z, int E, double* scratch, double* rz_partial, int rz_blocks,
                   const double* stop);
void precond_probes(kmvp_ctx* c, const double* g, const double* h, int P, double* z);
constexpr int PC_LOGD_BLOCKS = 64;
void precond_logdiag(kmvp_ctx* c, double* out);
int precond_read(kmvp_ctx* c, int* rank_built, int64_t* pivots, double* factor);

int cell_layout_read(kmvp_ctx* c, int64_t* info, double* sigma_b, int32_t* source_cell, int32_t* target_cell,
                     double* source_centres, int64_t source_cap, double* target_centres, int64_t target_cap);

int cg_solve(kmvp_ctx* c, int kernel, const void* a_host, int E, double rtol, int maxit, double* out_b,
             int* iters, double* resid);
int minres_solve(kmvp_ctx* c, int kernel, const void* a_host, int E, double rtol, int maxit,
                 double* out_b, int* iters, double* resid);
int cg_lanczos(kmvp_ctx* c, int kernel, const void* z_host, int P, double rtol, int maxit, double* logquad, double* invquad,
               int* steps, double* x_out, double* alpha_out, double* beta_out);
int cg_lanczos_precond(kmvp_ctx* c, int kernel, const double* g_host, const double* h_host, int P, double rtol, int maxit,
                       double* logdet_p, double* logquad, double* invquad, double* wnorm2, int* steps, double* x_out,
                       double* pz_out, double* alpha_out, double* beta_out);
struct Krylov {
  int64_t m = 0;
  int E = 0;
  size_t n = 0;
  size_t stop = 0;
  double *vecs = nullptr, *partial = nullptr, *state = nullptr;
  double* vec(int i) const { return vecs + (size_t)i * n; }
};
struct SolveGuard {
  kmvp_ctx* c;
  ~SolveGuard() { c->async_product = false; c->have_signal = false; }
};
int solver_shape(kmvp_ctx* c);
int cg_apply(kmvp_ctx* c, int kernel, const double* v, const Krylov& k);

int eigsh_solve(kmvp_ctx* c, int kernel, int k, int op, const double* v0, double tol, int maxit, double* eigenvalues,
                double* eigenvectors, double* resid, int* steps, double* alpha_out, double* beta_out, double* degree_out);

int sinkhorn_solve(kmvp_ctx* c, int kernel, const double* log_a, const double* log_b, double tol, int maxit, double* u,
                   double* v, int* iters, double* err);

int kmeans_solve(kmvp_ctx* c, int C, const double* weights, double tol, int maxit, double* centroids, int64_t* labels,
                 double* cluster_weight, int* iters, double* inertia, double* shift);

int set_batches(kmvp_ctx* c, int B, const int64_t* y_offsets, const int64_t* x_offsets_or_null);
int run_product_batched(kmvp_ctx* c, int kernel, bool normalise);
int run_nearest_batched(kmvp_ctx* c, int K, int exclude_self, int64_t* out_idx, double* out_sqdist);
int batches_refuse(kmvp_ctx* c, const char* what);

int meanshift_solve(kmvp_ctx* c, double tol, int maxit, double* modes, int* iters, double* step2, int* sweeps,
                    int64_t* target_sweeps);

}
```

kernel_matrix_benchmarks_amd/csrc/kmvp_plan.hpp:

```cpp
#pragma once
#include <algorithm>
#include <cstdint>
#include <vector>

namespace kmvp {

constexpr int WAVES_PER_BLOCK = 4;
constexpr int CELL_TILE = 32;
constexpr int CELL_REST_TT = 2;
constexpr int STAGED_TILE = 32;
constexpr int64_t SMALL_PROBLEM_TARGETS = 32768;
constexpr int SEG_SPLIT_FROM = 16;
constexpr int64_t MAX_GRID = 0x7fffffff;

inline int64_t round_up(int64_t v, int64_t q) { return (v + q - 1) / q * q; }
inline bool small_problem(int64_t N) { return N < SMALL_PROBLEM_TARGETS; }


struct SegmentRule {
  int64_t stage_bytes;
  int cols;
  int64_t min_seg = 1;
  bool small = false;
  int64_t l2_seg_bytes = 2 << 20;
  int64_t target_blocks = 16384;
  SegmentRule(int64_t stage_bytes_, int cols_) : stage_bytes(stage_bytes_), cols(cols_) {}
};

inline int choose_segments(int opt_segments, int64_t tile_blocks, int64_t units, int64_t n_pad, const SegmentRule& r) {
  int64_t seg;
  if (opt_segments > 0) {
    seg = opt_segments;
  } else {
    seg = 8 * std::max<int64_t>(1, (units * r.stage_bytes + 8 * r.l2_seg_bytes - 1) / (8 * r.l2_seg_bytes));
    const int64_t target_blocks = r.small ? 4096 : r.target_blocks;
    const int64_t for_parallelism = (target_blocks + tile_blocks - 1) / tile_blocks;
    if (for_parallelism > seg) seg = (for_parallelism + 7) / 8 * 8;
    const int64_t cap_len = std::max<int64_t>(1, units / r.min_seg);
    const int64_t cap_mem = std::max<int64_t>(1, (int64_t)(4e9 / ((double)r.cols * n_pad * 8)));
    seg = std::min(seg, std::min(cap_len, cap_mem));
    if (seg >= 8) seg = seg / 8 * 8;
  }
  seg = std::max<int64_t>(1, std::min<int64_t>(seg, 65535));
  return (int)seg;
}

inline int settle_segments(int64_t units, int seg) {
  auto settled = [&](int64_t cand) { return (units + (units + cand - 1) / cand - 1) / ((units + cand - 1) / cand); };
  if (seg >= 8 && units >= 8)
    for (int step = 0; step <= 64; step += 8)
      for (int64_t cand : {(int64_t)seg + step, (int64_t)seg - step})
        if (cand >= 8 && cand <= units && cand % 8 == 0 && settled(cand) == cand) return (int)cand;
  seg = (int)std::max<int64_t>(1, std::min<int64_t>(seg, std::max<int64_t>(units, 1)));
  return (int)settled(seg);
}

inline int stage_segments(int opt_segments, int64_t tile_blocks, int64_t m_stages, int64_t n_pad, const SegmentRule& r) {
  return settle_segments(m_stages, choose_segments(opt_segments, tile_blocks, m_stages, n_pad, r));
}


struct StagePlan {
  int64_t n_pad, tile_blocks, m_stages, seg_stages, grid;
  int TT, segments;
  bool ok;
};
inline StagePlan plan_stages(int64_t N, int64_t m_stages, int opt_tiles, int tt_max, int tt_default, int opt_segments,
                             SegmentRule r) {
  StagePlan p;
  r.small = small_problem(N);
  if (r.small) r.min_seg = 1;
  p.TT = opt_tiles > 0 ? std::min(opt_tiles, tt_max) : (r.small ? 1 : std::min(tt_default, tt_max));
  const int64_t tile = (int64_t)STAGED_TILE * p.TT * WAVES_PER_BLOCK;
  p.n_pad = round_up(N, tile);
  p.tile_blocks = p.n_pad / tile;
  p.m_stages = m_stages;
  p.segments = stage_segments(opt_segments, p.tile_blocks, m_stages, p.n_pad, r);
  p.seg_stages = (m_stages + p.segments - 1) / p.segments;
  p.grid = p.tile_blocks * p.segments;
  p.ok = p.grid <= MAX_GRID;
  return p;
}


template <class F>
void for_each_key_run(const unsigned* keys, int64_t n, F&& f) {
  for (int64_t p = 0; p < n;) {
    int64_t e = p + 1;
    while (e < n && keys[e] == keys[p]) ++e;
    f(p, e - p, keys[p]);
    p = e;
  }
}

struct TileList {
  std::vector<int> start, count;
  std::vector<unsigned> key;
  size_t size() const { return start.size(); }
  void reserve(size_t tiles) {
    start.reserve(tiles);
    count.reserve(tiles);
    key.reserve(tiles);
  }
  void add_cell(int64_t first, int64_t at, int64_t end, unsigned k, int64_t live, int64_t empty, int tile) {
    for (int64_t t = 0; t < live; ++t, at += tile) push((int)at, (int)std::min<int64_t>(tile, end - at), k);
    for (int64_t t = 0; t < empty; ++t) push((int)first, 0, k);
  }
  void pad_to(size_t mult) {
    while (!start.empty() && start.size() % mult) push(start.back(), 0, key.back());
  }
  void append(const TileList& o) {
    start.insert(start.end(), o.start.begin(), o.start.end());
    count.insert(count.end(), o.count.begin(), o.count.end());
    key.insert(key.end(), o.key.begin(), o.key.end());
  }

 private:
  void push(int s, int c, unsigned k) {
    start.push_back(s);
    count.push_back(c);
    key.push_back(k);
  }
};

inline TileList cell_tiles(const unsigned* keys, int64_t n, int tile = CELL_TILE) {
  TileList l;
  l.reserve((size_t)n / 24 + 16);
  for_each_key_run(keys, n, [&](int64_t p, int64_t cnt, unsigned k) { l.add_cell(p, p, p + cnt, k, (cnt + tile - 1) / tile, 0, tile); });
  return l;
}

struct CellTiles {
  int64_t main_live, main_empty, rest_live, rest_empty;
};
inline CellTiles split_cell_tiles(int64_t tiles, int TT) {
  const int64_t rem = tiles % TT;
  if (TT > CELL_REST_TT && rem > 0 && rem <= TT / 2) return {tiles - rem, 0, rem, round_up(rem, CELL_REST_TT) - rem};
  return {tiles, round_up(tiles, TT) - tiles, 0, 0};
}

inline void cell_split_count(const unsigned* keys, int64_t n, int TT, int64_t* n_main, int64_t* n_rest) {
  *n_main = *n_rest = 0;
  for_each_key_run(keys, n, [&](int64_t, int64_t cnt, unsigned) {
    const CellTiles s = split_cell_tiles((cnt + CELL_TILE - 1) / CELL_TILE, TT);
    *n_main += s.main_live + s.main_empty;
    *n_rest += s.rest_live + s.rest_empty;
  });
}

inline TileList cell_tiles_split(const unsigned* keys, int64_t n, int TT, int64_t* n_main, int64_t* n_rest) {
  TileList main, rest;
  main.reserve((size_t)n / 24 + 64);
  for_each_key_run(keys, n, [&](int64_t p, int64_t cnt, unsigned k) {
    const CellTiles s = split_cell_tiles((cnt + CELL_TILE - 1) / CELL_TILE, TT);
    main.add_cell(p, p, p + cnt, k, s.main_live, s.main_empty, CELL_TILE);
    rest.add_cell(p, p + s.main_live * CELL_TILE, p + cnt, k, s.rest_live, s.rest_empty, CELL_TILE);
  });
  main.pad_to((size_t)TT * WAVES_PER_BLOCK);
  rest.pad_to((size_t)CELL_REST_TT * WAVES_PER_BLOCK);
  *n_main = (int64_t)main.size();
  *n_rest = (int64_t)rest.size();
  main.append(rest);
  return main;
}

struct CellSplit {
  int64_t m_stages, n_slots;
  int64_t blocks[2], slots[2], seg_stages[2];
  int segments[2];
  int64_t grid(int r) const { return blocks[r] * segments[r]; }
  size_t region_offset(int cols, int r) const { return r ? (size_t)segments[0] * cols * slots[0] : 0; }
  size_t part_doubles(int cols) const { return ((size_t)segments[0] * slots[0] + (size_t)segments[1] * slots[1]) * cols; }
};

inline CellSplit cell_split(int64_t N, int64_t m_tiles, int64_t n_main, int64_t n_rest, int tt, int opt_segments,
                            int stage_tiles, SegmentRule main) {
  CellSplit s;
  main.small = small_problem(N);
  if (main.small) main.min_seg = 1;
  s.m_stages = (m_tiles + stage_tiles - 1) / stage_tiles;
  s.n_slots = (n_main + n_rest) * CELL_TILE;
  s.blocks[0] = n_main / (tt * WAVES_PER_BLOCK);
  s.blocks[1] = n_rest / (CELL_REST_TT * WAVES_PER_BLOCK);
  s.slots[0] = n_main * CELL_TILE;
  s.slots[1] = n_rest * CELL_TILE;
  s.segments[0] = stage_segments(opt_segments, std::max<int64_t>(1, s.blocks[0]), s.m_stages, s.n_slots, main);
  s.seg_stages[0] = (s.m_stages + s.segments[0] - 1) / s.segments[0];
  s.segments[1] = 0;
  s.seg_stages[1] = 1;
  if (s.blocks[1] > 0) {
    SegmentRule rest = main;
    rest.min_seg = 1;
    rest.target_blocks = 1536;
    const int seg = choose_segments(opt_segments, s.blocks[1], s.m_stages, s.n_slots, rest);
    s.seg_stages[1] = (s.m_stages + seg - 1) / seg;
    s.segments[1] = (int)((s.m_stages + s.seg_stages[1] - 1) / s.seg_stages[1]);
  }
  return s;
}


struct FusedCellWork {
  int list;
  int64_t local;
};
constexpr FusedCellWork fused_cell_work(int64_t bid, int64_t main_grid) {
  return bid < main_grid ? FusedCellWork{0, bid} : FusedCellWork{1, bid - main_grid};
}

struct FusedCellGrid {
  bool fused;
  int64_t main_grid, rest_grid, total;
};
inline FusedCellGrid fused_cell_grid(const CellSplit& s, int tt, int opt_fused) {
  FusedCellGrid g;
  g.main_grid = s.grid(0);
  g.rest_grid = s.grid(1);
  g.total = g.main_grid + g.rest_grid;
  g.fused = opt_fused != 0 && tt > CELL_REST_TT && s.blocks[1] > 0 && g.total <= MAX_GRID;
  return g;
}


constexpr int CELL_SHARED_TT = 8;

constexpr bool cell_shared_build(int tt, int opt) { return opt != 0 && tt >= CELL_SHARED_TT; }

inline int64_t count_one_cell_blocks(const unsigned* keys, int64_t n_main, int tt) {
  const int64_t per_block = (int64_t)tt * WAVES_PER_BLOCK;
  int64_t one = 0;
  for (int64_t t = 0; t + per_block <= n_main; t += per_block) {
    bool same = true;
    for (int w = 1; w < WAVES_PER_BLOCK; ++w) same = same && keys[t + (int64_t)w * tt] == keys[t];
    one += same ? 1 : 0;
  }
  return one;
}


constexpr int CELL_ZQ_BITS = 12;
constexpr int CELL_ZQ = 1 << CELL_ZQ_BITS;
constexpr int CELL_BALANCE_MIN_CAP = 16;

struct CountCell {
  int64_t first, count;
  int zlo, zhi;
  unsigned column;
};

inline std::vector<CountCell> count_cut_cells(const unsigned* fine, int64_t n, int cap, int64_t quantum, int64_t full) {
  std::vector<CountCell> cells;
  cells.reserve((size_t)(n / std::max<int64_t>(full, 1)) + 16);
  const unsigned zmask = (unsigned)CELL_ZQ - 1u;
  for (int64_t p = 0; p < n;) {
    const unsigned column = fine[p] >> CELL_ZQ_BITS;
    const int zlo = (int)(fine[p] & zmask);
    int64_t e = p + 1;
    while (e < n && e - p < full && (fine[e] >> CELL_ZQ_BITS) == column && (int)(fine[e] & zmask) - zlo < cap) ++e;
    const bool by_cap = e < n && e - p < full && (fine[e] >> CELL_ZQ_BITS) == column;
    int64_t count = e - p;
    if (by_cap && count >= quantum) count = count / quantum * quantum;
    cells.push_back({p, count, zlo, (int)(fine[p + count - 1] & zmask), column});
    p += count;
  }
  return cells;
}

inline float count_cell_zcentre(double lo, double bw, int zlo, int zhi) { return (float)(lo + 0.5 * (double)(zlo + zhi + 1) * bw); }

inline TileList count_cell_source_tiles(const std::vector<CountCell>& cells, int tile = CELL_TILE) {
  TileList l;
  l.reserve(cells.size() * 33 + 16);
  for (size_t i = 0; i < cells.size(); ++i) {
    const CountCell& c = cells[i];
    l.add_cell(c.first, c.first, c.first + c.count, (unsigned)i, (c.count + tile - 1) / tile, 0, tile);
  }
  return l;
}

inline TileList count_cell_target_tiles(const std::vector<CountCell>& cells, int TT, int64_t* n_main, int64_t* n_rest) {
  TileList main, rest;
  main.reserve(cells.size() * 33 + 64);
  const int64_t per_block = (int64_t)TT * WAVES_PER_BLOCK;
  for (int pass = 0; pass < 2; ++pass)
    for (size_t i = 0; i < cells.size(); ++i) {
      const CountCell& c = cells[i];
      const CellTiles s = split_cell_tiles((c.count + CELL_TILE - 1) / CELL_TILE, TT);
      const int64_t m = s.main_live + s.main_empty;
      if ((m > 0 && m % per_block == 0) != (pass == 0)) continue;
      main.add_cell(c.first, c.first, c.first + c.count, (unsigned)i, s.main_live, s.main_empty, CELL_TILE);
      rest.add_cell(c.first, c.first + s.main_live * CELL_TILE, c.first + c.count, (unsigned)i, s.rest_live, s.rest_empty, CELL_TILE);
    }
  main.pad_to((size_t)per_block);
  rest.pad_to((size_t)CELL_REST_TT * WAVES_PER_BLOCK);
  *n_main = (int64_t)main.size();
  *n_rest = (int64_t)rest.size();
  main.append(rest);
  return main;
}

constexpr bool cell_balance_applies(int D, bool f32, int tt, int cap) {
  return D == 3 && f32 && tt == CELL_SHARED_TT && cap >= CELL_BALANCE_MIN_CAP;
}
constexpr int64_t CELLMM16_AUTO_N = 500000, CELLMM16_AUTO_M = 100000;
constexpr bool cell_balance_taken(int opt, bool applies, int64_t N, int64_t M) {
  return opt != 0 && applies && (opt > 0 || (N >= CELLMM16_AUTO_N && M >= CELLMM16_AUTO_M));
}

}
```

kernel_matrix_benchmarks_amd/csrc/kmvp_product.hip:

```cpp
#include "kmvp_ctx.hpp"
#include <array>
#include <cstring>
#include <map>
#include <vector>
#include "kmvp_cell_pack.hpp"
#include "kmvp_cell64_pack.hpp"
#include "kmvp_cellmm_pack.hpp"
#include "kmvp_cfast_pack.hpp"
#include "kmvp_fast_pack.hpp"
#include "kmvp_fastmm_pack.hpp"
#include "kmvp_cfastmm_pack.hpp"
#include "kmvp_mfma_pack.hpp"

namespace kmvp {
namespace {

template <typename real>
hipError_t launch_lowd(int kernel, int D, int E, int sig, LowdTuning tune,
                       const LowdArgs<real>& args, dim3 grid, hipStream_t s, const char** name);
template <>
hipError_t launch_lowd<float>(int kernel, int D, int E, int sig, LowdTuning tune,
                              const LowdArgs<float>& args, dim3 grid, hipStream_t s,
                              const char** name) {
  switch (kernel) {
// ... 1174 lines not shown
bool cell_make_grid(const float* aux, int D, float h_max, CellGrid& grid) {
  for (int a = 0; a < 3; ++a) {
    grid.lo[a] = 0.f;
    grid.g[a] = 1;
    grid.h[a] = h_max;
    grid.inv_h[a] = 1.f / h_max;
  }
  for (int a = 0; a < D; ++a) {
    const float half = aux[FAST_AUX_HALF + a];
    grid.lo[a] = aux[a] - half;
    const double cells = std::max(1.0, std::ceil(2.0 * half / h_max));
    if (!(cells <= CELL_MAX_GRID)) return false;
    grid.g[a] = (int)cells;
    if (half > 0.f) {
      grid.h[a] = (float)(2.0 * half / cells);
      grid.inv_h[a] = 1.f / grid.h[a];
    }
  }
  return true;
}
void cell_store_grid(kmvp_ctx* c, const CellGrid& grid) {
  for (int a = 0; a < 3; ++a) {
    c->cell_lo[a] = grid.lo[a];
    c->cell_g[a] = grid.g[a];
    c->cell_hh[a] = grid.h[a];
  }
}
void cell_load_grid(const kmvp_ctx* c, CellGrid& grid) {
  for (int a = 0; a < 3; ++a) {
    grid.lo[a] = c->cell_lo[a];
    grid.g[a] = c->cell_g[a];
    grid.h[a] = c->cell_hh[a];
    grid.inv_h[a] = 1.f / c->cell_hh[a];
  }
  grid.centres = nullptr;
}
CellGrid cell_side_grid(const kmvp_ctx* c, CellGrid grid, bool targets) {
  if (c->cell_balanced) grid.centres = (const float*)((targets && !c->same_points) ? c->cell_tcentre.p : c->cell_scentre32.p);
  return grid;
}


constexpr float CELL_Z_WIDTH_MAX = 0.125f;
constexpr float CMM_F_LATTICE = 0.104f;
int cell_balance_cap(const CellGrid& grid, double* zq_per_unit, double* bucket) {
  const double room = 2.0 * CELL_T_MAX - (double)grid.h[0] * grid.h[0] - (double)grid.h[1] * grid.h[1];
  const double extent = (double)grid.g[2] * grid.h[2];
  *bucket = extent / CELL_ZQ;
  *zq_per_unit = CELL_ZQ / extent;
  if (!(room > 0.0) || !(extent > 0.0)) return 0;
  const double width = std::min(std::sqrt(room), (double)CELL_Z_WIDTH_MAX);
  return (int)std::min<double>(CELL_ZQ, std::floor(width / *bucket));
}

int upload_cell_centres(kmvp_ctx* c, const CellGrid& grid, double bucket, const std::vector<CountCell>& cells, kmvp_ctx::DevBuf& buf) {
  std::vector<float> tab(4 * std::max<size_t>(cells.size(), 1), 0.f);
  for (size_t i = 0; i < cells.size(); ++i) {
    tab[4 * i + 0] = cell_centre(cells[i].column, 0, grid);
    tab[4 * i + 1] = cell_centre(cells[i].column, 1, grid);
    tab[4 * i + 2] = count_cell_zcentre(grid.lo[2], bucket, cells[i].zlo, cells[i].zhi);
  }
  int rc;
  if ((rc = ensure(c, buf, tab.size() * sizeof(float)))) return rc;
  HIP_TRY(c, hipMemcpyAsync(buf.p, tab.data(), tab.size() * sizeof(float), hipMemcpyHostToDevice, c->stream));
  HIP_TRY(c, hipStreamSynchronize(c->stream));
  return KMVP_OK;
}

int cell_prepare_balanced(kmvp_ctx* c, const CellGrid& grid, int TT, int cap, double zq_per_unit, double bucket) {
  const int64_t quantum = (int64_t)CELL_TILE * TT, full = quantum * WAVES_PER_BLOCK;
  int rc;
  std::vector<unsigned> keys;
  if ((rc = cell_sort(c, c->y_raw.p, c->M, grid, c->cell_sperm, keys, nullptr, zq_per_unit))) return rc;
  std::vector<CountCell> cells = count_cut_cells(keys.data(), c->M, cap, c->same_points ? quantum : (int64_t)CELL_TILE, full);
  const TileList sources = count_cell_source_tiles(cells);
  if ((rc = upload_tiles(c, sources, c->cell_sgrp))) return rc;
  c->cell_m_tiles = (int64_t)sources.size();
  if ((rc = upload_cell_centres(c, grid, bucket, cells, c->cell_scentre32))) return rc;
  if (!c->same_points) {
    if ((rc = cell_sort(c, c->x_raw.p, c->N, grid, c->cell_tperm, keys, nullptr, zq_per_unit))) return rc;
    cells = count_cut_cells(keys.data(), c->N, cap, quantum, full);
    if ((rc = upload_cell_centres(c, grid, bucket, cells, c->cell_tcentre))) return rc;
  }
  return upload_tiles(c, count_cell_target_tiles(cells, TT, &c->cell_n_main, &c->cell_n_rest), c->cell_tgrp);
}

inline double cell_ps_per_tile(int TT) { return TT >= 8 ? CMM_PS_PER_TILE_MAIN : (TT >= 4 ? CMM_PS_PER_TILE_TT4 : CMM_PS_PER_TILE_REST); }

int cell_prepare(kmvp_ctx* c, int TT) {
  if (c->cell_ver == c->points_ver && c->cell_state != 0 && c->cell_balance_req == c->opt_cell_balance &&
      (c->cell_state < 0 || c->cell_tt_req == TT))
    return KMVP_OK;
  c->cell_tt_req = TT;
  c->cell_balance_req = c->opt_cell_balance;
  c->cell_ver = c->points_ver;
  c->cell_state = -1;
  const int D = c->D;
  if (D > CELL_MAX_D || !(c->cloud_radius2 < INFINITY) || c->N > 0x3fffffff || c->M > 0x3fffffff) return KMVP_OK;
  float aux[FAST_AUX_FLOATS];
  HIP_TRY(c, hipMemcpyAsync(aux, c->aux.p, sizeof(aux), hipMemcpyDeviceToHost, c->stream));
  HIP_TRY(c, hipStreamSynchronize(c->stream));
  CellGrid grid;
  if (!cell_make_grid(aux, D, (float)(std::sqrt(2.f * CELL_T_MAX / (float)D)), grid)) return KMVP_OK;
  int rc;
  std::vector<unsigned> keys;
  if ((rc = cell_sort(c, c->y_raw.p, c->M, grid, c->cell_sperm, keys))) return rc;
  const TileList sources = cell_tiles(keys.data(), c->M);
  if ((rc = upload_tiles(c, sources, c->cell_sgrp))) return rc;
  c->cell_m_tiles = (int64_t)sources.size();
  if (!c->same_points && (rc = cell_sort(c, c->x_raw.p, c->N, grid, c->cell_tperm, keys))) return rc;
  if (TT == 0) {
    double best = INFINITY;
    for (int t : {8, 4, 2}) {
      int64_t nm, nr;
      cell_split_count(keys.data(), (int64_t)keys.size(), t, &nm, &nr);
      const double cost = cell_ps_per_tile(t) * (double)nm + cell_ps_per_tile(2) * (double)nr;
      if (cost < best) {
        best = cost;
        TT = t;
      }
    }
  }
  double zq_per_unit, bucket;
  const int cap = cell_balance_cap(grid, &zq_per_unit, &bucket);
  c->cell_balanced = false;
  if (cell_balance_taken(c->opt_cell_balance, cell_balance_applies(D, c->dtype == KMVP_F32, TT, cap), c->N, c->M)) {
    c->cell_balanced = true;
    c->cell_zw = (float)((double)cap * bucket);
    if ((rc = cell_prepare_balanced(c, grid, TT, cap, zq_per_unit, bucket))) return rc;
  } else if ((rc = upload_tiles(c, cell_tiles_split(keys.data(), (int64_t)keys.size(), TT, &c->cell_n_main, &c->cell_n_rest), c->cell_tgrp)))
    return rc;
  c->cell_n_tiles = c->cell_n_main + c->cell_n_rest;
  c->cell_tt = TT;
  cell_store_grid(c, grid);
  c->cell_state = 1;
  c->packed_layout = -1;
  return KMVP_OK;
}

double cell_padding(const kmvp_ctx* c) {
  const double t = (double)c->cell_n_tiles * CELL_TILE / (double)std::max<int64_t>(c->N, 1);
  const double s = (double)c->cell_m_tiles * CELL_TILE / (double)std::max<int64_t>(c->M, 1);
  return std::max(t, s);
}

CellSplit cell_plan(const kmvp_ctx* c, int stage_tiles, SegmentRule main) {
  return cell_split(c->N, c->cell_m_tiles, c->cell_n_main, c->cell_n_rest, c->cell_tt, c->opt_segments, stage_tiles, main);
}
double* cell_region(const kmvp_ctx* c, const CellSplit& s, int cols, int r) { return (double*)c->part.p + s.region_offset(cols, r); }
template <class Args>
void cell_args(const kmvp_ctx* c, const CellSplit& s, int cols, int r, Args& a) {
  a.part = cell_region(c, s, cols, r);
  a.n_slots = s.slots[r];
  a.tile_base = r ? c->cell_n_main : 0;
  a.seg_stages = s.seg_stages[r];
  a.segments = s.segments[r];
  a.tile_blocks = (int)s.blocks[r];
}
inline int cell_tt(const kmvp_ctx* c, int r) { return r ? CELL_REST_TT : c->cell_tt; }

int pack_cell_targets(kmvp_ctx* c, const CellGrid& grid) {
  const int64_t n_tiles = c->cell_n_tiles;
  const float* x_raw = (const float*)(c->same_points ? c->y_raw.p : c->x_raw.p);
  const int* tperm = (const int*)(c->same_points ? c->cell_sperm.p : c->cell_tperm.p);
  const int* tgrp = (const int*)c->cell_tgrp.p;
  int rc;
  if ((rc = ensure(c, c->xs, (size_t)n_tiles * CELL_TILE * 4 * sizeof(float)))) return rc;
  if ((rc = ensure(c, c->cell_tmeta, (size_t)n_tiles * 4 * sizeof(float)))) return rc;
  if ((rc = ensure(c, c->cell_slot, (size_t)c->N * sizeof(int)))) return rc;
  hipLaunchKernelGGL(pack_cell_targets_kernel, dim3((unsigned)n_tiles), dim3(CELL_TILE), 0, c->stream, x_raw, tperm,
                     tgrp, tgrp + n_tiles, (const unsigned*)(tgrp + 2 * n_tiles), n_tiles, c->D,
                     cell_side_grid(c, grid, true), (float*)c->xs.p, (float*)c->cell_tmeta.p, (int*)c->cell_slot.p);
  return KMVP_OK;
}


int run_product_cell(kmvp_ctx* c, int sig) {
  const int D = c->D;
  const int E = 1;
  const int NE = sig == SIG_NORM ? 2 : 1;
  const int64_t N = c->N;
  SegmentRule rule(CELL_STAGE_BYTES, NE);
  rule.min_seg = 4;
  const CellSplit s = cell_plan(c, CELL_STAGE_TILES, rule);
  const int64_t m_stages = s.m_stages, n_slots = s.n_slots;
  int rc;
  CellGrid grid;
  cell_load_grid(c, grid);

  const PackKey key = {LAYOUT_CELL, K_GAUSSIAN, c->cell_tt};
  const int* sgrp = (const int*)c->cell_sgrp.p;
  if (points_stale(c, key) && (rc = pack_cell_targets(c, grid))) return rc;
  if (signal_stale(c, key, sig)) {
    if ((rc = ensure(c, c->rec, (size_t)m_stages * CELL_STAGE_BYTES))) return rc;
    hipLaunchKernelGGL(pack_cell_sources_kernel, dim3((unsigned)(m_stages * CELL_STAGE_TILES)), dim3(CELL_TILE), 0,
                       c->stream, (const float*)c->y_raw.p,
                       sig == SIG_DENSITY ? (const float*)nullptr : (const float*)c->b_raw.p,
                       (const int*)c->cell_sperm.p, sgrp, sgrp + c->cell_m_tiles,
                       (const unsigned*)(sgrp + 2 * c->cell_m_tiles), c->cell_m_tiles, D, cell_side_grid(c, grid, false),
                       (unsigned char*)c->rec.p);
  }
  HIP_TRY(c, hipGetLastError());
  record_packed(c, key, sig);

  if ((rc = ensure(c, c->part, s.part_doubles(NE) * sizeof(double)))) return rc;
  CellArgs a;
  a.xd = (const float*)c->xs.p;
  a.tmeta = (const float*)c->cell_tmeta.p;
  a.img = (const unsigned char*)c->rec.p;
  a.m_stages = m_stages;
  a.chunk_stages = std::max(1, c->opt_chunk / (CELL_TILE * CELL_STAGE_TILES));
  HIP_TRY(c, mark(c, 0));
  hipError_t le = hipSuccess;
  for (int r = 0; r < 2 && le == hipSuccess; ++r)
    if (s.blocks[r] > 0) {
      cell_args(c, s, NE, r, a);
      le = launch_cell_gaussian(sig, cell_tt(c, r), a, dim3((unsigned)s.grid(r)), c->stream, &c->last_kernel_name);
    }
  if (le == hipErrorInvalidValue) return fail(c, KMVP_E_UNSUPPORTED, "fast_tiles must be 1, 2, 4 or 8");
  HIP_TRY(c, le);
  HIP_TRY(c, mark(c, 1));

  if ((rc = ensure(c, c->sums, (size_t)NE * N * sizeof(double)))) return rc;
  if ((rc = ensure(c, c->cell_sums, (size_t)NE * n_slots * sizeof(double)))) return rc;
  for (int r = 0; r < 2; ++r)
    if (s.blocks[r] > 0)
      hipLaunchKernelGGL(reduce_region_kernel, dim3(blocks_for((int64_t)NE * s.slots[r])), dim3(256), 0, c->stream,
                         (const double*)cell_region(c, s, NE, r), (double*)c->cell_sums.p, s.slots[r], NE, s.segments[r], n_slots,
                         r ? s.slots[0] : (int64_t)0);
  hipLaunchKernelGGL(gather_cells_kernel, dim3(blocks_for((int64_t)NE * N)), dim3(256), 0, c->stream,
                     (const double*)c->cell_sums.p, (const int*)c->cell_slot.p, (double*)c->sums.p, N, n_slots, NE);
  HIP_TRY(c, hipGetLastError());
  return finish_product(c, (int64_t)NE * N, N, N, E, sig);
}


int cellmm_wlog2(const kmvp_ctx* c) {
  double arg = 0.0;
  for (int a = 0; a < c->D; ++a) {
    const double w = (c->cell_balanced && a == 2) ? (double)c->cell_zw : (double)c->cell_hh[a];
    arg += w * ((double)c->cell_g[a] * c->cell_hh[a]);
  }
  return (int)std::ceil(arg * 1.4426950408889634);
}
float cellmm_fmax(const kmvp_ctx* c) { return c->cell_balanced ? std::max(CMM_F_LATTICE, c->cell_zw) : CMM_F_LATTICE; }

int run_product_cellmm(kmvp_ctx* c, int sig) {
  const int D = c->D;
  const int E = sig == SIG_DENSITY ? 1 : c->E;
  const int NE = sig == SIG_NORM ? E + 1 : E;
  const int64_t N = c->N;
  const int TT = c->cell_tt;
  SegmentRule rule(CMM_STAGE_BYTES, 1);
  rule.min_seg = 2;
  rule.l2_seg_bytes = 3 << 20;
  rule.target_blocks = 7168;
  const CellSplit s = cell_plan(c, CMM_STAGE_TILES, rule);
  const int64_t m_stages = s.m_stages, n_slots = s.n_slots;
  int rc;
  CellGrid grid;
  cell_load_grid(c, grid);

  const PackKey key = {LAYOUT_CELLMM, K_GAUSSIAN, TT};
  const int image_sig = NE > 1 ? -1 : sig;
  const bool sig_stale = signal_stale(c, key, image_sig);
  const int* sgrp = (const int*)c->cell_sgrp.p;
  if ((rc = ensure(c, c->cell_scale, 64))) return rc;
  float* scale = (float*)c->cell_scale.p;
  unsigned* bmax = (unsigned*)c->cell_scale.p + 4;
  HIP_TRY(c, mark(c, 0));
  if (points_stale(c, key)) {
    if ((rc = pack_cell_targets(c, grid))) return rc;
    if ((rc = ensure(c, c->rec, (size_t)m_stages * CMM_STAGE_BYTES))) return rc;
    hipLaunchKernelGGL(pack_cellmm_points_kernel, dim3((unsigned)(m_stages * CMM_STAGE_TILES)), dim3(CELL_TILE), 0,
                       c->stream, (const float*)c->y_raw.p, (const int*)c->cell_sperm.p, sgrp, sgrp + c->cell_m_tiles,
                       (const unsigned*)(sgrp + 2 * c->cell_m_tiles), c->cell_m_tiles, D, cell_side_grid(c, grid, false),
                       (unsigned char*)c->rec.p);
    HIP_TRY(c, hipGetLastError());
  }
  record_packed(c, key, image_sig);

  if ((rc = ensure(c, c->part, s.part_doubles(1) * sizeof(double)))) return rc;
  if ((rc = ensure(c, c->sums, (size_t)NE * N * sizeof(double)))) return rc;
  if ((rc = ensure(c, c->cell_sums, (size_t)NE * n_slots * sizeof(double)))) return rc;
  const int shape = c->opt_cellmm_shape >= 0 ? c->opt_cellmm_shape : ((TT >= 8 && c->N >= CELLMM16_AUTO_N && c->M >= CELLMM16_AUTO_M) ? 1 : 0);
  FusedCellGrid fg = fused_cell_grid(s, TT, c->opt_cell_fused);
  if (shape != 1) fg.fused = false;
  CellmmArgs a;
  a.xd = (const float*)c->xs.p;
  a.tmeta = (const float*)c->cell_tmeta.p;
  a.img = (const unsigned char*)c->rec.p;
  a.scale = scale;
  a.m_stages = m_stages;
  a.shared_build = cell_shared_build(TT, c->opt_cell_shared_build) ? 1 : 0;
  if (NE == 1 && !sig_stale) HIP_TRY(c, mark(c, 0));
  for (int col = 0; col < NE; ++col) {
    if (sig_stale) {
      const float* b = (sig == SIG_DENSITY || col == E) ? (const float*)nullptr : (const float*)c->b_raw.p;
      HIP_TRY(c, hipMemsetAsync(bmax, 0, sizeof(unsigned), c->stream));
      if (b)
        hipLaunchKernelGGL(cellmm_absmax_kernel, dim3((unsigned)std::min<int64_t>(1024, (c->M + 255) / 256)), dim3(256), 0,
                           c->stream, b, c->M, E, col, bmax);
      hipLaunchKernelGGL(cellmm_scale_kernel, dim3(1), dim3(1), 0, c->stream, (const unsigned*)bmax, cellmm_wlog2(c),
                         cellmm_fmax(c), b ? 0 : 1, scale);
      hipLaunchKernelGGL(pack_cellmm_signal_kernel, dim3((unsigned)(m_stages * CMM_STAGE_TILES)), dim3(CELL_TILE), 0,
                         c->stream, b, E, col, (const int*)c->cell_sperm.p, sgrp, sgrp + c->cell_m_tiles, c->cell_m_tiles,
                         (const float*)scale, (unsigned char*)c->rec.p);
      HIP_TRY(c, hipGetLastError());
      if (NE == 1) HIP_TRY(c, mark(c, 0));
    }
    hipError_t le = hipSuccess;
    if (fg.fused) {
      CellmmArgs ar = a;
      cell_args(c, s, 1, 0, a);
      cell_args(c, s, 1, 1, ar);
      le = launch_cellmm16_fused(TT, a, ar, fg.main_grid, fg.rest_grid, c->stream, &c->last_kernel_name);
    } else {
      for (int r = 0; r < 2 && le == hipSuccess; ++r)
        if (s.blocks[r] > 0) {
          cell_args(c, s, 1, r, a);
          le = launch_cellmm_gaussian(cell_tt(c, r), shape, a, dim3((unsigned)s.grid(r)), c->stream, &c->last_kernel_name);
        }
    }
    if (le == hipErrorInvalidValue) return fail(c, KMVP_E_UNSUPPORTED, "fast_tiles must be 1, 2, 4 or 8");
    HIP_TRY(c, le);
    if (NE == 1) HIP_TRY(c, mark(c, 1));
    double* col_sums = (double*)c->cell_sums.p + (size_t)col * n_slots;
    for (int r = 0; r < 2; ++r)
      if (s.blocks[r] > 0)
        hipLaunchKernelGGL(reduce_segments_kernel, dim3(blocks_for(s.slots[r])), dim3(256), 0, c->stream,
                           (const double*)cell_region(c, s, 1, r), col_sums + (r ? s.slots[0] : 0), s.slots[r], s.segments[r], 0);
    HIP_TRY(c, hipGetLastError());
  }
  if (NE > 1) HIP_TRY(c, mark(c, 1));

  hipLaunchKernelGGL(gather_cells_kernel, dim3(blocks_for((int64_t)NE * N)), dim3(256), 0, c->stream,
                     (const double*)c->cell_sums.p, (const int*)c->cell_slot.p, (double*)c->sums.p, N, n_slots, NE);
  HIP_TRY(c, hipGetLastError());
  return finish_product(c, (int64_t)NE * N, N, N, E, sig);
}


int cell64_prepare(kmvp_ctx* c) {
  if (c->cell_ver == c->points_ver && c->cell_state != 0) return KMVP_OK;
  c->cell_ver = c->points_ver;
  c->cell_state = -1;
  const int D = c->D;
  if (D > CELL_MAX_D || !(c->cloud_radius2 < INFINITY) || c->N > 0x3fffffff || c->M > 0x3fffffff) return KMVP_OK;
  float aux[FAST_AUX_FLOATS];
  HIP_TRY(c, hipMemcpyAsync(aux, c->aux.p, sizeof(aux), hipMemcpyDeviceToHost, c->stream));
  HIP_TRY(c, hipStreamSynchronize(c->stream));
  CellGrid grid;
  if (!cell_make_grid(aux, D, (float)((float)std::sqrt(2.0 * CELL64_T_MAX / (double)D)), grid)) return KMVP_OK;
  int rc;
  std::vector<unsigned> keys;
  if ((rc = cell_sort(c, c->y_raw.p, c->M, grid, c->cell_sperm, keys, &c->cell_skey))) return rc;
  std::vector<int> runs;
  std::vector<double> centres;
  for_each_key_run(keys.data(), c->M, [&](int64_t first, int64_t count, unsigned key) {
    runs.push_back((int)first);
    runs.push_back((int)count);
    for (int a = 0; a < 3; ++a) centres.push_back(a < D ? cell64_centre(key, a, grid) : 0.0);
    centres.push_back(0.0);
  });
  c->cell_m_tiles = (int64_t)runs.size() / 2;
  if ((rc = ensure(c, c->cell_sgrp, runs.size() * sizeof(int)))) return rc;
  if ((rc = ensure(c, c->cell_scentre, centres.size() * sizeof(double)))) return rc;
  HIP_TRY(c, hipMemcpyAsync(c->cell_sgrp.p, runs.data(), runs.size() * sizeof(int), hipMemcpyHostToDevice, c->stream));
  HIP_TRY(c, hipMemcpyAsync(c->cell_scentre.p, centres.data(), centres.size() * sizeof(double), hipMemcpyHostToDevice, c->stream));
  HIP_TRY(c, hipStreamSynchronize(c->stream));
  if (!c->same_points && (rc = cell_sort(c, c->x_raw.p, c->N, grid, c->cell_tperm, keys))) return rc;
  const TileList targets = cell_tiles(keys.data(), (int64_t)keys.size(), CELL64_TILE);
  if ((rc = upload_tiles(c, targets, c->cell_tgrp))) return rc;
  c->cell_n_tiles = (int64_t)targets.size();
  c->cell_tt = 1;
  cell_store_grid(c, grid);
  c->cell_state = 1;
  c->packed_layout = -1;
  return KMVP_OK;
}

int run_product_cell64(kmvp_ctx* c, int sig) {
  const int D = c->D;
  const int NE = sig == SIG_NORM ? 2 : 1;
  const int64_t N = c->N, M = c->M;
  const int64_t n_tiles = round_up(c->cell_n_tiles, WAVES_PER_BLOCK);
  const int64_t n_slots = n_tiles * CELL64_TILE;
  const int64_t tile_blocks = n_tiles / WAVES_PER_BLOCK;
  const int n_scells = (int)c->cell_m_tiles;
  int rc;
  CellGrid grid;
  cell_load_grid(c, grid);
  int64_t seg = c->opt_segments > 0 ? c->opt_segments : (8192 + tile_blocks - 1) / tile_blocks;
  seg = std::max<int64_t>(1, std::min<int64_t>(seg, n_scells));
  const int seg_cells = (int)((n_scells + seg - 1) / seg);
  const int segments = (n_scells + seg_cells - 1) / seg_cells;

  const PackKey key = {LAYOUT_CELL64, K_GAUSSIAN, 1};
  const double* x_raw = (const double*)(c->same_points ? c->y_raw.p : c->x_raw.p);
  const int* tperm = (const int*)(c->same_points ? c->cell_sperm.p : c->cell_tperm.p);
  const int* tgrp = (const int*)c->cell_tgrp.p;
  if (points_stale(c, key)) {
    if ((rc = ensure(c, c->xs, (size_t)n_slots * 4 * sizeof(double)))) return rc;
    if ((rc = ensure(c, c->cell_tmeta, (size_t)n_tiles * 4 * sizeof(double)))) return rc;
    if ((rc = ensure(c, c->cell_slot, (size_t)N * sizeof(int)))) return rc;
    hipLaunchKernelGGL(pack_cell64_targets_kernel, dim3((unsigned)n_tiles), dim3(CELL64_TILE), 0, c->stream, x_raw, tperm,
                       tgrp, tgrp + c->cell_n_tiles, (const unsigned*)(tgrp + 2 * c->cell_n_tiles), c->cell_n_tiles, D,
                       grid, (double*)c->xs.p, (double*)c->cell_tmeta.p, (int*)c->cell_slot.p);
  }
  if (signal_stale(c, key, sig)) {
    const int64_t m_alloc = M + 64;
    if ((rc = ensure(c, c->rec, (size_t)m_alloc * 4 * sizeof(double)))) return rc;
    hipLaunchKernelGGL(pack_cell64_sources_kernel, dim3(blocks_for(m_alloc)), dim3(256), 0, c->stream,
                       (const double*)c->y_raw.p, sig == SIG_DENSITY ? (const double*)nullptr : (const double*)c->b_raw.p,
                       (const int*)c->cell_sperm.p, (const unsigned*)c->cell_skey.p, M, m_alloc, D, grid, (double*)c->rec.p);
  }
  HIP_TRY(c, hipGetLastError());
  record_packed(c, key, sig);

  if ((rc = ensure(c, c->part, (size_t)segments * NE * n_slots * sizeof(double)))) return rc;
  Cell64Args a;
  a.xd = (const double*)c->xs.p;
  a.tmeta = (const double*)c->cell_tmeta.p;
  a.srec = (const double*)c->rec.p;
  a.scell = (const int*)c->cell_sgrp.p;
  a.scentre = (const double*)c->cell_scentre.p;
  a.part = (double*)c->part.p;
  a.n_slots = n_slots;
  a.n_scells = n_scells;
  a.seg_cells = seg_cells;
  a.segments = segments;
  a.tile_blocks = (int)tile_blocks;
  const dim3 grid_dim((unsigned)(tile_blocks * segments));
  HIP_TRY(c, mark(c, 0));
  HIP_TRY(c, launch_cell64_gaussian(sig, a, grid_dim, c->stream, &c->last_kernel_name));
  HIP_TRY(c, mark(c, 1));

  if ((rc = ensure(c, c->sums, (size_t)NE * N * sizeof(double)))) return rc;
  if ((rc = ensure(c, c->cell_sums, (size_t)NE * n_slots * sizeof(double)))) return rc;
  hipLaunchKernelGGL(reduce_segments_kernel, dim3(blocks_for((int64_t)NE * n_slots)), dim3(256), 0, c->stream,
                     (const double*)c->part.p, (double*)c->cell_sums.p, (int64_t)NE * n_slots, segments, 0);
  hipLaunchKernelGGL(gather_cells_kernel, dim3(blocks_for((int64_t)NE * N)), dim3(256), 0, c->stream,
                     (const double*)c->cell_sums.p, (const int*)c->cell_slot.p, (double*)c->sums.p, N, n_slots, NE);
  HIP_TRY(c, hipGetLastError());
  return finish_product(c, (int64_t)NE * N, N, N, 1, sig);
}


float scaled_radius2(const kmvp_ctx* c, int kernel) {
  const float sc = scale_for<float>(kernel);
  return c->cloud_radius2 * sc * sc;
}
bool radius_ok(const kmvp_ctx* c, int kernel) { return scaled_radius2(c, kernel) <= FAST_AUTO_RADIUS2; }

bool big_clouds(const kmvp_ctx* c) { return c->N >= SMALL_PROBLEM_TARGETS && c->M >= SMALL_PROBLEM_TARGETS; }

int cell_tiles_request(const kmvp_ctx* c) {
  return c->opt_fast_tiles > 0 ? c->opt_fast_tiles : (c->N < SMALL_PROBLEM_TARGETS ? 1 : 0);
}

bool cellmm_in_range(const kmvp_ctx* c) { return radius_ok(c, K_GAUSSIAN) && cellmm_wlog2(c) <= CMM_MAX_WLOG2; }

bool cells_considered(const kmvp_ctx* c, bool several) {
  if (several && (c->opt_fast == 4 || !radius_ok(c, K_GAUSSIAN))) return false;
  return c->opt_fast >= 3 || (c->opt_fast < 0 && radius_ok(c, K_GAUSSIAN) && big_clouds(c));
}

int cells_usable(kmvp_ctx* c, bool several, bool& ok) {
  const bool forced = c->opt_fast >= 3;
  ok = false;
  if (cells_considered(c, several)) {
    const int rc = cell_prepare(c, cell_tiles_request(c));
    if (rc) return rc;
    ok = c->cell_state == 1 && (forced || cell_padding(c) <= CELL_AUTO_MAX_PAD) && (!several || cellmm_in_range(c));
    if (ok) return KMVP_OK;
  }
  char buf[256];
  if (c->opt_fast >= 0 && !forced) {
    snprintf(buf, sizeof buf, "cell form not considered: fast_sqdists = %d was requested", c->opt_fast);
  } else if (!radius_ok(c, K_GAUSSIAN)) {
    snprintf(buf, sizeof buf, "cell form not taken: squared half-diagonal of the clouds' bounding box %.3g > %.3g (radius rule)",
             (double)scaled_radius2(c, K_GAUSSIAN), (double)FAST_AUTO_RADIUS2);
  } else if (!big_clouds(c)) {
    snprintf(buf, sizeof buf, "cell form not taken: fewer than %lld points in a cloud (N = %lld, M = %lld)",
// ... 118 lines not shown
  return finish_product(c, count, N, n_pad, E, sig);
}

}

int measure_clouds(kmvp_ctx* c, int dtype, int64_t M, int64_t N, int D) {
  c->cloud_radius2 = INFINITY;
  const bool f64_cells = dtype == KMVP_F64 && D <= CELL_MAX_D;
  if ((dtype != KMVP_F32 && !f64_cells) || D > FMM_MAX_D || M <= 0 || N <= 0) return KMVP_OK;
  int rc;
  if ((rc = ensure(c, c->aux, (FAST_AUX_FLOATS + 2 * (size_t)FAST_BBOX_BLOCKS * D) * sizeof(float)))) return rc;
  float* part = (float*)c->aux.p + FAST_AUX_FLOATS;
  if (f64_cells)
    hipLaunchKernelGGL((fast_bbox_partial_kernel<double>), dim3(FAST_BBOX_BLOCKS), dim3(256), 0, c->stream,
                       (const double*)c->y_raw.p, M, c->same_points ? (const double*)nullptr : (const double*)c->x_raw.p, N,
                       D, part);
  else
    hipLaunchKernelGGL((fast_bbox_partial_kernel<float>), dim3(FAST_BBOX_BLOCKS), dim3(256), 0, c->stream,
                       (const float*)c->y_raw.p, M, c->same_points ? (const float*)nullptr : (const float*)c->x_raw.p, N,
                       D, part);
  hipLaunchKernelGGL(fast_center_kernel, dim3(1), dim3(FAST_BBOX_BLOCKS), 0, c->stream, (const float*)part, D,
                     (float*)c->aux.p);
  HIP_TRY(c, hipGetLastError());
  HIP_TRY(c, hipMemcpyAsync(&c->cloud_radius2, (float*)c->aux.p + FAST_AUX_RADIUS2, sizeof(float),
                            hipMemcpyDeviceToHost, c->stream));
  c->centre_ver = c->points_ver + 1;
  return KMVP_OK;
}

int prepare_points(kmvp_ctx* c, int kernel) {
  if (kernel != K_GAUSSIAN || c->D > CELL_MAX_D || c->N == 0 || c->M == 0 || c->centre_ver != c->points_ver) return KMVP_OK;
  if (c->dtype == KMVP_F32 && cells_considered(c, false)) return cell_prepare(c, cell_tiles_request(c));
  if (c->dtype == KMVP_F64 && cells64_considered(c)) return cell64_prepare(c);
  return KMVP_OK;
}

int cell_layout_read(kmvp_ctx* c, int64_t* info, double* sigma_b, int32_t* source_cell, int32_t* target_cell,
                     double* source_centres, int64_t source_cap, double* target_centres, int64_t target_cap) {
  if (!info) return fail(c, KMVP_E_INVALID, "kmvp_cell_layout: info is NULL");
  const int layout = c->packed_layout;
  const bool f64 = layout == LAYOUT_CELL64;
  if (!c->have_points || c->cell_state != 1 || c->cell_ver != c->points_ver || c->packed_points_ver != c->points_ver ||
      (layout != LAYOUT_CELL && layout != LAYOUT_CELLMM && !f64) || f64 != (c->dtype == KMVP_F64))
    return fail(c, KMVP_E_INVALID, "kmvp_cell_layout: no product on the cell form has run on the current points");
  const int64_t M = c->M, N = c->N;
  const int tile = f64 ? CELL64_TILE : CELL_TILE;
  const int* sperm_d = (const int*)c->cell_sperm.p;
  std::vector<int> sperm((size_t)M);
  HIP_TRY(c, hipMemcpyAsync(sperm.data(), sperm_d, (size_t)M * sizeof(int), hipMemcpyDeviceToHost, c->stream));

  std::vector<int32_t> scell((size_t)M, -1);
  std::vector<double> scen;
  auto assign = [](std::vector<int32_t>& of, int64_t idx, int64_t n, int32_t id) {
    if (idx < 0 || idx >= n) return false;
    of[(size_t)idx] = of[(size_t)idx] == -1 ? id : -2;
    return true;
  };
  bool sound = true;
  if (f64) {
    const int64_t cells = c->cell_m_tiles;
    std::vector<int> runs((size_t)cells * 2);
    std::vector<double> cen((size_t)cells * 4);
    HIP_TRY(c, hipMemcpyAsync(runs.data(), c->cell_sgrp.p, runs.size() * sizeof(int), hipMemcpyDeviceToHost, c->stream));
    HIP_TRY(c, hipMemcpyAsync(cen.data(), c->cell_scentre.p, cen.size() * sizeof(double), hipMemcpyDeviceToHost, c->stream));
    HIP_TRY(c, hipStreamSynchronize(c->stream));
    for (int64_t sc = 0; sc < cells; ++sc) {
      for (int a = 0; a < 3; ++a) scen.push_back(cen[(size_t)sc * 4 + a]);
      for (int64_t p = runs[2 * sc]; p < (int64_t)runs[2 * sc] + runs[2 * sc + 1]; ++p)
        sound = sound && p >= 0 && p < M && assign(scell, sperm[(size_t)p], M, (int32_t)sc);
    }
  } else {
    const int stage_tiles = layout == LAYOUT_CELL ? CELL_STAGE_TILES : CMM_STAGE_TILES;
    const int hdr_off = layout == LAYOUT_CELL ? CELL_HDR_OFF : CMM_HDR_OFF;
    const int stage_bytes = layout == LAYOUT_CELL ? CELL_STAGE_BYTES : CMM_STAGE_BYTES;
    const int64_t m_tiles = c->cell_m_tiles, m_stages = (m_tiles + stage_tiles - 1) / stage_tiles;
    std::vector<int> grp((size_t)m_tiles * 3);
    std::vector<float> hdr((size_t)m_stages * stage_tiles * 4);
    HIP_TRY(c, hipMemcpyAsync(grp.data(), c->cell_sgrp.p, grp.size() * sizeof(int), hipMemcpyDeviceToHost, c->stream));
    if (m_stages > 0)
      HIP_TRY(c, hipMemcpy2DAsync(hdr.data(), (size_t)stage_tiles * 16, (const unsigned char*)c->rec.p + hdr_off, (size_t)stage_bytes,
                                  (size_t)stage_tiles * 16, (size_t)m_stages, hipMemcpyDeviceToHost, c->stream));
    HIP_TRY(c, hipStreamSynchronize(c->stream));
    int key_s = -2;
    for (int64_t t = 0; t < m_tiles; ++t) {
      const float* h = &hdr[(size_t)t * 4];
      int key;
      memcpy(&key, h + 3, sizeof key);
      if (key != key_s) {
        key_s = key;
        for (int a = 0; a < 3; ++a) scen.push_back((double)h[a]);
      }
      const int32_t id = (int32_t)(scen.size() / 3) - 1;
      const int64_t start = grp[(size_t)t], count = grp[(size_t)m_tiles + t];
      sound = sound && key >= 0 && count >= 0 && count <= CELL_TILE && start >= 0 && start + count <= M;
      for (int64_t k = 0; sound && k < count; ++k) sound = assign(scell, sperm[(size_t)(start + k)], M, id);
    }
  }
  if (!sound) return fail(c, KMVP_E_DEVICE, "kmvp_cell_layout: the source tile list points outside the cloud");

  const int64_t n_tiles = f64 ? round_up(c->cell_n_tiles, WAVES_PER_BLOCK) : c->cell_n_tiles;
  std::vector<int> slot((size_t)N);
  std::vector<double> tmeta((size_t)n_tiles * 4);
  HIP_TRY(c, hipMemcpyAsync(slot.data(), c->cell_slot.p, (size_t)N * sizeof(int), hipMemcpyDeviceToHost, c->stream));
  if (f64) {
    HIP_TRY(c, hipMemcpyAsync(tmeta.data(), c->cell_tmeta.p, tmeta.size() * sizeof(double), hipMemcpyDeviceToHost, c->stream));
    HIP_TRY(c, hipStreamSynchronize(c->stream));
  } else {
    std::vector<float> m32((size_t)n_tiles * 4);
    HIP_TRY(c, hipMemcpyAsync(m32.data(), c->cell_tmeta.p, m32.size() * sizeof(float), hipMemcpyDeviceToHost, c->stream));
    HIP_TRY(c, hipStreamSynchronize(c->stream));
    for (size_t q = 0; q < m32.size(); ++q) tmeta[q] = (q & 3) == 3 ? 0.0 : (double)m32[q];
  }
  std::vector<int32_t> tcell((size_t)N, -1);
  std::vector<double> tcen;
  std::map<std::array<double, 3>, int32_t> ids;
  std::vector<char> taken((size_t)n_tiles * tile, 0);
  for (int64_t i = 0; i < N; ++i) {
    const int64_t sl = slot[(size_t)i];
    if (sl < 0 || sl >= n_tiles * tile) continue;
    const double* m = &tmeta[(size_t)(sl / tile) * 4];
    const std::array<double, 3> key = {m[0], m[1], m[2]};
    auto it = ids.find(key);
    if (it == ids.end()) {
      it = ids.emplace(key, (int32_t)(tcen.size() / 3)).first;
      tcen.insert(tcen.end(), key.begin(), key.end());
    }
    tcell[(size_t)i] = taken[(size_t)sl] ? -2 : it->second;
    taken[(size_t)sl] = 1;
  }

  const int64_t ns = (int64_t)scen.size() / 3, nt = (int64_t)tcen.size() / 3;
  info[0] = ns;
  info[1] = nt;
  info[2] = c->cell_balanced ? 1 : 0;
  info[3] = c->cell_tt;
  info[4] = tile;
  info[5] = layout == LAYOUT_CELL ? 0 : (layout == LAYOUT_CELLMM ? 1 : 2);
  info[6] = f64 ? 0 : c->cell_n_main;
  info[7] = f64 ? 0 : c->cell_n_rest;
  if (sigma_b) {
    float sc = 0.f;
    if (layout == LAYOUT_CELLMM) {
      HIP_TRY(c, hipMemcpyAsync(&sc, c->cell_scale.p, sizeof sc, hipMemcpyDeviceToHost, c->stream));
      HIP_TRY(c, hipStreamSynchronize(c->stream));
    }
    *sigma_b = (double)sc;
  }
  if ((source_centres && source_cap < ns) || (target_centres && target_cap < nt))
    return fail(c, KMVP_E_INVALID, "kmvp_cell_layout: room for fewer centres than there are cells (info[0], info[1])");
  if (source_cell) memcpy(source_cell, scell.data(), (size_t)M * sizeof(int32_t));
  if (target_cell) memcpy(target_cell, tcell.data(), (size_t)N * sizeof(int32_t));
  if (source_centres) memcpy(source_centres, scen.data(), scen.size() * sizeof(double));
  if (target_centres) memcpy(target_centres, tcen.data(), tcen.size() * sizeof(double));
  return KMVP_OK;
}

int run_product(kmvp_ctx* c, int kernel, bool normalise) {
  if (!c) return KMVP_E_INVALID;
  c->note.clear();
  if (!c->have_points) return fail(c, KMVP_E_INVALID, "kmvp_set_points has not been called");
  if (!c->have_signal) return fail(c, KMVP_E_INVALID, "kmvp_set_signal has not been called");
  HIP_TRY(c, hipSetDevice(c->device));
  const bool matern = kernel == K_MATERN32 || kernel == K_MATERN52;
  if (matern) {
    if (c->dtype == KMVP_BF16)
      return fail(c, KMVP_E_UNSUPPORTED, "Matern kernels: built for float32 and float64 contexts, not for bfloat16");
    if (c->opt_fast >= 1)
      return fail(c, KMVP_E_UNSUPPORTED, "Matern kernels: fast_sqdists = " + std::to_string(c->opt_fast) +
                                             " asks for a matrix-core form that is not built for them (-1 or 0: the difference form)");
  }
  if (c->M < c->m_total && !(c->exchanges() && c->world > 1) && !c->opt_partial)
    return fail(c, KMVP_E_INVALID,
                "the sources are a shard (M < M_total) but no multi-rank communicator is attached: call kmvp_comm_init, "
                "or set option partial_shard = 1 to get this shard's partial sums on purpose");
  const int sig = c->density ? SIG_DENSITY : (normalise ? SIG_NORM : SIG_PRODUCT);
  if (c->M == 0 && c->N > 0 && c->exchanges() && c->world > 1) {
    const int E = c->density ? 1 : c->E;
    const int64_t NE = sig == SIG_NORM ? E + 1 : E;
    int rc = ensure(c, c->sums, (size_t)NE * c->N * sizeof(double));
    if (rc) return rc;
    HIP_TRY(c, mark(c, 0));
    HIP_TRY(c, hipMemsetAsync(c->sums.p, 0, (size_t)NE * c->N * sizeof(double), c->stream));
    HIP_TRY(c, mark(c, 1));
    c->last_kernel_name = "none";
    if (c->density && normalise) {
    } else if (takes_shifted_tail(c, kernel)) {
      if ((rc = ensure(c, c->kshift, (size_t)c->N * sizeof(double)))) return rc;
      hipLaunchKernelGGL(fill_kernel, dim3(blocks_for(c->N)), dim3(256), 0, c->stream, (double*)c->kshift.p, c->N,
                         (double)INFINITY);
      HIP_TRY(c, hipGetLastError());
      return finish_product_shifted(c, c->N, c->N, E, sig);
    } else {
      return finish_product(c, NE * c->N, c->N, c->N, E, sig);
    }
  }
  if (c->N == 0 || c->M == 0) {
    const int E = c->density ? 1 : c->E;
    int rc = ensure(c, c->out, (size_t)std::max<int64_t>(c->N, 1) * E * sizeof(double));
    if (rc) return rc;
    if (c->N > 0) {
      hipLaunchKernelGGL(fill_kernel, dim3(blocks_for(c->N * E)), dim3(256), 0, c->stream,
                         (double*)c->out.p, c->N * E,
                         normalise ? std::nan("") : 0.0);
      HIP_TRY(c, hipStreamSynchronize(c->stream));
    }
    c->out_n = c->N;
    c->out_e = E;
    c->last_kernel_ms = c->last_total_ms = 0.f;
    return KMVP_OK;
  }
  if (c->density && normalise) {
    int rc = ensure(c, c->out, (size_t)c->N * sizeof(double));
    if (rc) return rc;
    hipLaunchKernelGGL(fill_kernel, dim3(blocks_for(c->N)), dim3(256), 0, c->stream,
                       (double*)c->out.p, c->N, 1.0);
    HIP_TRY(c, hipStreamSynchronize(c->stream));
    c->out_n = c->N;
    c->out_e = 1;
    c->last_kernel_ms = c->last_total_ms = 0.f;
    c->last_kernel_name = "fill_kernel";
    return KMVP_OK;
  }
  if (kernel == K_EXPDOT) {
    if (c->density) return fail(c, KMVP_E_UNSUPPORTED, "exp(<x,y>): pass a signal of ones for density estimation");
    if (c->dtype == KMVP_BF16) return run_product_mfma(c, K_EXPDOT, sig);
    if (c->dtype != KMVP_F32 || c->D > FMM_MAX_D)
      return fail(c, KMVP_E_UNSUPPORTED,
                  "exp(<x,y>) is built for float32 at D <= 64 and for bfloat16 (other cases: the plugin's Gaussian identity)");
    return run_product_fastmm(c, K_GAUSSIAN, sig, true);
  }
  if (c->dtype == KMVP_BF16) return run_product_mfma(c, kernel, sig);
  if (matern) {
    if (c->D <= LOWD_MAX_D && !c->density && c->E > LOWD_MAX_E)
      return c->dtype == KMVP_F64 ? run_product_blocked<double>(c, kernel, sig) : run_product_blocked<float>(c, kernel, sig);
    return c->dtype == KMVP_F64 ? run_product_t<double>(c, kernel, sig) : run_product_t<float>(c, kernel, sig);
  }
  const bool f32 = c->dtype == KMVP_F32 && c->centre_ver == c->points_ver;
  bool cells = false;
  if (f32 && kernel == K_GAUSSIAN && c->D <= CELL_MAX_D) {
    const int rc = cells_usable(c, !c->density && c->E > 1, cells);
    if (rc) return rc;
  }
  if (f32 && kernel == K_GAUSSIAN && !c->density && (c->E > 1 || c->D > FAST_MAX_D) &&
      (c->opt_fast < 0 || c->opt_fast == 1 || c->opt_fast == 3)) {
    const int cols = c->E + (normalise ? 1 : 0);
    const bool fmm_ok = c->D <= FMM_MAX_D && (c->opt_fast == 1 || (c->opt_fast < 0 && radius_ok(c, kernel)));
    const double t_cell = cells ? (double)cols * (double)c->cell_m_tiles *
                                      (cell_ps_per_tile(c->cell_tt) * (double)c->cell_n_main + cell_ps_per_tile(2) * (double)c->cell_n_rest)
                                : INFINITY;
    char cost[224];
    double t_fmm = INFINITY;
    if (fmm_ok) {
      const double tiles = std::ceil((double)c->N / FAST_TILE) * std::ceil((double)c->M / FAST_TILE);
      t_fmm = tiles * ((cols + FMM_MAX_COLS - 1) / FMM_MAX_COLS) * (cols > 16 ? FMM_PS_PER_TILE_32 : FMM_PS_PER_TILE_16);
    }
    snprintf(cost, sizeof cost, " [cost model, %d columns: fastmm_kernel %.3g ms, cellmm_kernel %.3g ms (%lld + %lld target x %lld source tiles)]",
             cols, t_fmm * 1e-9, t_cell * 1e-9, (long long)c->cell_n_main, (long long)c->cell_n_rest, (long long)c->cell_m_tiles);
    if (fmm_ok && (c->opt_fast == 1 || t_fmm <= t_cell)) {
      c->note.clear();
      const int rc = run_product_fastmm(c, K_GAUSSIAN, sig);
      if (c->opt_fast < 0) c->note += cost;
      return rc;
    }
    if (cells) {
      c->note.clear();
      const int rc = run_product_cellmm(c, sig);
      if (c->opt_fast < 0) c->note += cost;
      return rc;
    }
  }
  if (f32 && kernel == K_ABSEXP && !c->density && c->D > CFAST_MAX_D && c->D <= FMM_MAX_D && (c->opt_fast < 0 || c->opt_fast == 1)) {
    const bool pays = c->D > LOWD_MAX_D || c->E + (normalise ? 1 : 0) > LOWD_MAX_E;
    if (radius_ok(c, kernel) && (c->opt_fast == 1 || pays)) {
      c->note.clear();
      return run_product_fastmm(c, K_ABSEXP, sig);
    }
  }
  const bool invdist_square = kernel == K_INVDIST && (c->same_points || c->opt_same_global) && c->N == c->m_total;
  if (f32 && (kernel == K_GAUSSIAN || kernel == K_ABSEXP || invdist_square) && !c->density && c->E > 1 && c->D <= CFAST_MAX_D &&
      (c->opt_fast == 2 || (c->opt_fast < 0 && c->E + (normalise ? 1 : 0) >= CFMM_AUTO_MIN_COLS))) {
    c->note.clear();
    return run_product_cfastmm(c, kernel, sig);
  }
  if (f32 && c->D <= FAST_MAX_D && (c->density || c->E == 1)) {
    const bool global_ok = kernel == K_GAUSSIAN && radius_ok(c, kernel);
    const bool centred_ok = c->D <= CFAST_MAX_D && (kernel != K_INVDIST || invdist_square);
    if (cells) {
      c->note = c->cell_balanced ? "count-cut cells: the lattice's columns cut along z by point count (cell_balance)" : "";
      if (c->opt_fast != 4 && cellmm_in_range(c))
        return run_product_cellmm(c, sig);
      if (c->opt_fast != 4)
        c->note = std::string(c->note.empty() ? "" : c->note + "; ") +
                  "cell_kernel instead of cellmm_kernel: the clouds are outside the radius rule (f16 operand range)";
      return run_product_cell(c, sig);
    }
    if (c->opt_fast == 1 || (c->opt_fast < 0 && global_ok)) return run_product_fast(c, kernel, sig);
    if (centred_ok && (c->opt_fast == 2 || c->opt_fast < 0)) return run_product_cfast(c, kernel, sig);
  }
  if (c->dtype == KMVP_F64 && kernel == K_GAUSSIAN && c->D <= CELL_MAX_D && (c->density || c->E == 1) &&
      c->centre_ver == c->points_ver && cells64_considered(c)) {
    int rc = cell64_prepare(c);
    if (rc) return rc;
    if (c->cell_state == 1 &&
        (c->opt_fast == 3 || (double)c->cell_n_tiles * CELL64_TILE <= CELL_AUTO_MAX_PAD * (double)c->N))
      return run_product_cell64(c, sig);
  }
// ... 286 lines not shown
```

Before: 46270 billion.

## Split partial last wave of fused cellmm16 grid into a finer-segmented tail list

Adds a third cell list (tail) to the fused cellmm16 launch. When the main list's block count does not fill whole rounds of resident workgroups, the leftover target blocks are re-split into more source segments so the last round keeps the device busy. The kernel routes blockIdx into main, tail, or rest arguments, and the reduction and slot offsets are generalised to three lists. The change adds extra segment partials and reduction work for the tail blocks, and relies on a resident-workgroup estimate taken from the CU count. It is enabled automatically for TT=8 at large N and M, and a diagnostic API for reading the lists is added.

Measured after the change: 47750 billion (median of 6 runs). 3.2% higher.

```diff
diff --git a/include/kmvp.h b/include/kmvp.h
--- a/include/kmvp.h
+++ b/include/kmvp.h
@@ -172,6 +172,8 @@
 int kmvp_cell_layout(kmvp_ctx* ctx, int64_t* info, double* sigma_b, int32_t* source_cell, int32_t* target_cell,
                      double* source_centres, int64_t source_cap, double* target_centres, int64_t target_cap);
 
+int kmvp_cell_lists(kmvp_ctx* ctx, int64_t* info, int32_t* target_list);
+
 #ifdef __cplusplus
 }
 #endif
diff --git a/kernel_matrix_benchmarks_amd/_lib.py b/kernel_matrix_benchmarks_amd/_lib.py
--- a/kernel_matrix_benchmarks_amd/_lib.py
+++ b/kernel_matrix_benchmarks_amd/_lib.py
@@ -97,6 +97,7 @@
     ("kmvp_last_total_ms", _c.c_double, [_c.c_void_p]),
     ("kmvp_cell_layout", _c.c_int, [_c.c_void_p, _c.c_void_p, _c.POINTER(_c.c_double), _c.c_void_p, _c.c_void_p, _c.c_void_p,
                                     _c.c_int64, _c.c_void_p, _c.c_int64]),
+    ("kmvp_cell_lists", _c.c_int, [_c.c_void_p, _c.c_void_p, _c.c_void_p]),
     ("kmvp_last_kernel_name", _c.c_char_p, [_c.c_void_p]),
     ("kmvp_last_dispatch_note", _c.c_char_p, [_c.c_void_p]),
 ]
@@ -590,6 +591,15 @@
                 "count_cut": bool(info[2]), "tiles_per_wavefront": int(info[3]), "tile_points": int(info[4]),
                 "image": int(info[5]), "main_tiles": int(info[6]), "rest_tiles": int(info[7]), "sigma_b": float(sigma.value)}
 
+    def cell_lists(self):
+        if not self._ctx:
+            raise ValueError("the context is closed")
+        info = np.zeros(8, dtype=np.int64)
+        lists = np.empty(self.N, dtype=np.int32)
+        self._check(self._lib.kmvp_cell_lists(self._ctx, info.ctypes.data, lists.ctypes.data))
+        return {"blocks": tuple(int(v) for v in info[0:3]), "segments": tuple(int(v) for v in info[3:6]),
+                "resident": int(info[6]), "fused": bool(info[7]), "target_list": lists}
+
 
 def comm_unique_id():
     buf = ctypes.create_string_buffer(UNIQUE_ID_BYTES)
diff --git a/kernel_matrix_benchmarks_amd/csrc/kmvp_api.hip b/kernel_matrix_benchmarks_amd/csrc/kmvp_api.hip
--- a/kernel_matrix_benchmarks_amd/csrc/kmvp_api.hip
+++ b/kernel_matrix_benchmarks_amd/csrc/kmvp_api.hip
@@ -66,6 +66,7 @@
   bool ok = hipSetDevice(device) == hipSuccess &&
             hipStreamCreateWithFlags(&c->stream, hipStreamNonBlocking) == hipSuccess;
   for (int i = 0; ok && i < 5; ++i) ok = hipEventCreate(&c->ev[i]) == hipSuccess;
+  ok = ok && hipDeviceGetAttribute(&c->device_cus, hipDeviceAttributeMultiprocessorCount, device) == hipSuccess;
   if (!ok) {
     fail(nullptr, KMVP_E_DEVICE, "cannot create stream/events on the device");
     if (status) *status = KMVP_E_DEVICE;
@@ -446,6 +447,12 @@
   } else if (k == "cell_balance") {
     if (value < -1 || value > 1) return fail(c, KMVP_E_INVALID, "cell_balance must be -1 (automatic), 0 (never) or 1 (wherever count-cut cells apply)");
     c->opt_cell_balance = (int)value;
+  } else if (k == "cell_tail") {
+    if (value < -1 || value > 1) return fail(c, KMVP_E_INVALID, "cell_tail must be -1 (automatic), 0 (never) or 1 (wherever the fused grid has a partial last round)");
+    c->opt_cell_tail = (int)value;
+  } else if (k == "cell_tail_resident") {
+    if (value < 0 || value > 65536) return fail(c, KMVP_E_INVALID, "cell_tail_resident must be 0 (the device's: two workgroups per compute unit) or a number of workgroups up to 65536");
+    c->opt_cell_tail_resident = (int)value;
   } else if (k == "cell_shared_build") {
     if (value < -1 || value > 1) return fail(c, KMVP_E_INVALID, "cell_shared_build must be -1 (automatic), 0 (never) or 1 (wherever a workgroup is one-cell)");
     c->opt_cell_shared_build = (int)value;
@@ -491,6 +498,11 @@
   if (!c) return KMVP_E_INVALID;
   return cell_layout_read(c, info, sigma_b, source_cell, target_cell, source_centres, source_cap, target_centres, target_cap);
 }
+
+int kmvp_cell_lists(kmvp_ctx* c, int64_t* info, int32_t* target_list) {
+  if (!c) return KMVP_E_INVALID;
+  return cell_lists_read(c, info, target_list);
+}
 const char* kmvp_last_kernel_name(const kmvp_ctx* c) { return c ? c->last_kernel_name : ""; }
 const char* kmvp_last_dispatch_note(const kmvp_ctx* c) { return c ? c->note.c_str() : ""; }
 
diff --git a/kernel_matrix_benchmarks_amd/csrc/kmvp_cellmm.hpp b/kernel_matrix_benchmarks_amd/csrc/kmvp_cellmm.hpp
--- a/kernel_matrix_benchmarks_amd/csrc/kmvp_cellmm.hpp
+++ b/kernel_matrix_benchmarks_amd/csrc/kmvp_cellmm.hpp
@@ -318,6 +318,9 @@
 
 #ifndef CMM16_NOFOLD
 #define CMM16_NOFOLD 0
+#endif
+#ifndef CMM16_WHOLE_ROUNDS
+#define CMM16_WHOLE_ROUNDS 0
 #endif
 #ifndef CMM16_BUILD_PROBE
 #define CMM16_BUILD_PROBE 0
@@ -596,26 +599,36 @@
 
 template <int TT>
 __global__ void __launch_bounds__(BLOCK_THREADS) __attribute__((amdgpu_waves_per_eu(TT >= 8 ? 2 : 1)))
-cellmm16_kernel(const CellmmArgs a, const CellmmArgs rest, const int main_grid) {
+cellmm16_kernel(const CellmmArgs a, const CellmmArgs rest, const int main_grid, const CellmmArgs tail, const int tail_grid) {
   __shared__ __attribute__((aligned(16))) unsigned char lds[cellmm16_lds_bytes(TT)];
+  CellmmArgs m = a;
+  int bid = (int)blockIdx.x;
   if constexpr (TT > CELL_REST_TT) {
-    const FusedCellWork w = fused_cell_work((int64_t)blockIdx.x, (int64_t)main_grid);
-    if (w.list) {
+    const FusedCellWork w = fused_cell_work((int64_t)blockIdx.x, (int64_t)main_grid, (int64_t)tail_grid);
+    if (w.list == 1) {
       cellmm16_body<CELL_REST_TT, false>(rest, (int)w.local, lds);
       return;
     }
+    const bool t = w.list == 2;
+    m.part = t ? tail.part : a.part;
+    m.n_slots = t ? tail.n_slots : a.n_slots;
+    m.tile_base = t ? tail.tile_base : a.tile_base;
+    m.seg_stages = t ? tail.seg_stages : a.seg_stages;
+    m.segments = t ? tail.segments : a.segments;
+    m.tile_blocks = t ? tail.tile_blocks : a.tile_blocks;
+    bid = (int)w.local;
   }
   if constexpr (cellmm16_has_shared(TT)) {
-    if (a.shared_build && cellmm16_one_cell<TT>(a, (int)blockIdx.x)) {
-      cellmm16_body<TT, true>(a, (int)blockIdx.x, lds);
+    if (m.shared_build && cellmm16_one_cell<TT>(m, bid)) {
+      cellmm16_body<TT, true>(m, bid, lds);
       return;
     }
   }
-  cellmm16_body<TT, false>(a, (int)blockIdx.x, lds);
+  cellmm16_body<TT, false>(m, bid, lds);
 }
 
 hipError_t launch_cellmm_gaussian(int TT, int shape, const CellmmArgs& args, dim3 grid, hipStream_t stream, const char** kernel_name);
-hipError_t launch_cellmm16_fused(int TT, const CellmmArgs& main, const CellmmArgs& rest, int64_t main_grid, int64_t rest_grid,
-                                 hipStream_t stream, const char** kernel_name);
-
-}
+hipError_t launch_cellmm16_fused(int TT, const CellmmArgs& main, const CellmmArgs& rest, const CellmmArgs& tail, int64_t main_grid,
+                                 int64_t tail_grid, int64_t rest_grid, hipStream_t stream, const char** kernel_name);
+
+}
diff --git a/kernel_matrix_benchmarks_amd/csrc/kmvp_cellmm_inst.hip b/kernel_matrix_benchmarks_amd/csrc/kmvp_cellmm_inst.hip
--- a/kernel_matrix_benchmarks_amd/csrc/kmvp_cellmm_inst.hip
+++ b/kernel_matrix_benchmarks_amd/csrc/kmvp_cellmm_inst.hip
@@ -19,10 +19,10 @@
   if (shape == 1) {
     const int all = (int)grid.x;
     switch (TT) {
-      case 1: cmm_launch(cellmm16_kernel<1>, args, grid, stream, args, all); break;
-      case 2: cmm_launch(cellmm16_kernel<2>, args, grid, stream, args, all); break;
-      case 4: cmm_launch(cellmm16_kernel<4>, args, grid, stream, args, all); break;
-      case 8: cmm_launch(cellmm16_kernel<8>, args, grid, stream, args, all); break;
+      case 1: cmm_launch(cellmm16_kernel<1>, args, grid, stream, args, all, args, 0); break;
+      case 2: cmm_launch(cellmm16_kernel<2>, args, grid, stream, args, all, args, 0); break;
+      case 4: cmm_launch(cellmm16_kernel<4>, args, grid, stream, args, all, args, 0); break;
+      case 8: cmm_launch(cellmm16_kernel<8>, args, grid, stream, args, all, args, 0); break;
       default: return hipErrorInvalidValue;
     }
     return hipGetLastError();
@@ -37,14 +37,18 @@
   return hipGetLastError();
 }
 
-hipError_t launch_cellmm16_fused(int TT, const CellmmArgs& main, const CellmmArgs& rest, int64_t main_grid, int64_t rest_grid,
-                                 hipStream_t stream, const char** kernel_name) {
+hipError_t launch_cellmm16_fused(int TT, const CellmmArgs& main, const CellmmArgs& rest, const CellmmArgs& tail, int64_t main_grid,
+                                 int64_t tail_grid, int64_t rest_grid, hipStream_t stream, const char** kernel_name) {
   if (kernel_name) *kernel_name = "cellmm16_kernel";
-  if (main_grid + rest_grid > MAX_GRID) return hipErrorInvalidConfiguration;
-  const dim3 grid((unsigned)(main_grid + rest_grid));
+  if (main_grid + tail_grid + rest_grid > MAX_GRID) return hipErrorInvalidConfiguration;
+#if CMM16_WHOLE_ROUNDS
+  const dim3 grid((unsigned)main_grid);
+#else
+  const dim3 grid((unsigned)(main_grid + tail_grid + rest_grid));
+#endif
   switch (TT) {
-    case 4: cmm_launch(cellmm16_kernel<4>, main, grid, stream, rest, (int)main_grid); break;
-    case 8: cmm_launch(cellmm16_kernel<8>, main, grid, stream, rest, (int)main_grid); break;
+    case 4: cmm_launch(cellmm16_kernel<4>, main, grid, stream, rest, (int)main_grid, tail, (int)tail_grid); break;
+    case 8: cmm_launch(cellmm16_kernel<8>, main, grid, stream, rest, (int)main_grid, tail, (int)tail_grid); break;
     default: return hipErrorInvalidValue;
   }
   return hipGetLastError();
diff --git a/kernel_matrix_benchmarks_amd/csrc/kmvp_ctx.hpp b/kernel_matrix_benchmarks_amd/csrc/kmvp_ctx.hpp
--- a/kernel_matrix_benchmarks_amd/csrc/kmvp_ctx.hpp
+++ b/kernel_matrix_benchmarks_amd/csrc/kmvp_ctx.hpp
@@ -153,6 +153,10 @@
   int opt_cell_shared_build = -1;
   int opt_cell_balance = -1;
   int opt_cell_fused = -1;
+  int opt_cell_tail = -1;
+  int opt_cell_tail_resident = 0;
+  int device_cus = 0;
+  int64_t cell_list_info[8] = {0, 0, 0, 0, 0, 0, 0, 0};
   int opt_mfma_variant = -1;
   int opt_meanshift_compact = -1;
   int opt_same_global = 0;
@@ -250,6 +254,7 @@
 
 int cell_layout_read(kmvp_ctx* c, int64_t* info, double* sigma_b, int32_t* source_cell, int32_t* target_cell,
                      double* source_centres, int64_t source_cap, double* target_centres, int64_t target_cap);
+int cell_lists_read(kmvp_ctx* c, int64_t* info, int32_t* target_list);
 
 int cg_solve(kmvp_ctx* c, int kernel, const void* a_host, int E, double rtol, int maxit, double* out_b,
              int* iters, double* resid);
diff --git a/kernel_matrix_benchmarks_amd/csrc/kmvp_plan.hpp b/kernel_matrix_benchmarks_amd/csrc/kmvp_plan.hpp
--- a/kernel_matrix_benchmarks_amd/csrc/kmvp_plan.hpp
+++ b/kernel_matrix_benchmarks_amd/csrc/kmvp_plan.hpp
@@ -164,13 +164,28 @@
   return main;
 }
 
+constexpr int CELL_LISTS = 3;
+constexpr int CELL_LIST_ORDER[CELL_LISTS] = {0, 2, 1};
 struct CellSplit {
   int64_t m_stages, n_slots;
-  int64_t blocks[2], slots[2], seg_stages[2];
-  int segments[2];
+  int64_t blocks[CELL_LISTS], slots[CELL_LISTS], seg_stages[CELL_LISTS];
+  int segments[CELL_LISTS];
   int64_t grid(int r) const { return blocks[r] * segments[r]; }
-  size_t region_offset(int cols, int r) const { return r ? (size_t)segments[0] * cols * slots[0] : 0; }
-  size_t part_doubles(int cols) const { return ((size_t)segments[0] * slots[0] + (size_t)segments[1] * slots[1]) * cols; }
+  int64_t slot_base(int r) const {
+    int64_t at = 0;
+    for (int o = 0; o < CELL_LISTS && CELL_LIST_ORDER[o] != r; ++o) at += slots[CELL_LIST_ORDER[o]];
+    return at;
+  }
+  size_t region_offset(int cols, int r) const {
+    size_t at = 0;
+    for (int o = 0; o < CELL_LISTS && CELL_LIST_ORDER[o] != r; ++o) at += (size_t)segments[CELL_LIST_ORDER[o]] * cols * slots[CELL_LIST_ORDER[o]];
+    return at;
+  }
+  size_t part_doubles(int cols) const {
+    size_t n = 0;
+    for (int r = 0; r < CELL_LISTS; ++r) n += (size_t)segments[r] * slots[r] * cols;
+    return n;
+  }
 };
 
 inline CellSplit cell_split(int64_t N, int64_t m_tiles, int64_t n_main, int64_t n_rest, int tt, int opt_segments,
@@ -196,6 +211,9 @@
     s.seg_stages[1] = (s.m_stages + seg - 1) / seg;
     s.segments[1] = (int)((s.m_stages + s.seg_stages[1] - 1) / s.seg_stages[1]);
   }
+  s.blocks[2] = s.slots[2] = 0;
+  s.segments[2] = 0;
+  s.seg_stages[2] = 1;
   return s;
 }
 
@@ -204,21 +222,82 @@
   int list;
   int64_t local;
 };
-constexpr FusedCellWork fused_cell_work(int64_t bid, int64_t main_grid) {
-  return bid < main_grid ? FusedCellWork{0, bid} : FusedCellWork{1, bid - main_grid};
+constexpr FusedCellWork fused_cell_work(int64_t bid, int64_t main_grid, int64_t tail_grid = 0) {
+  return bid < main_grid               ? FusedCellWork{0, bid}
+         : bid < main_grid + tail_grid ? FusedCellWork{2, bid - main_grid}
+                                       : FusedCellWork{1, bid - main_grid - tail_grid};
 }
 
 struct FusedCellGrid {
   bool fused;
-  int64_t main_grid, rest_grid, total;
+  int64_t main_grid, rest_grid, total, tail_grid;
 };
 inline FusedCellGrid fused_cell_grid(const CellSplit& s, int tt, int opt_fused) {
   FusedCellGrid g;
   g.main_grid = s.grid(0);
   g.rest_grid = s.grid(1);
-  g.total = g.main_grid + g.rest_grid;
+  g.tail_grid = s.grid(2);
+  g.total = g.main_grid + g.tail_grid + g.rest_grid;
   g.fused = opt_fused != 0 && tt > CELL_REST_TT && s.blocks[1] > 0 && g.total <= MAX_GRID;
   return g;
+}
+
+
+constexpr int CELL_TAIL_MAX_SEGMENTS = 64;
+struct CellTail {
+  int64_t b_full, b_tail, seg_stages;
+  int segments;
+};
+inline CellTail cell_tail_plan(int64_t B, int S, int64_t R, int64_t m_stages, int64_t rest_grid, int64_t min_seg) {
+  const CellTail none = {B, 0, 1, 0};
+  if (B <= 0 || S <= 0 || R <= 0) return none;
+  int64_t gcd = R, t = S;
+  while (t) {
+    const int64_t u = gcd % t;
+    gcd = t;
+    t = u;
+  }
+  const int64_t q = R / gcd;
+  const int64_t b_full = B / q * q, b_tail = B - b_full;
+  if (b_full == 0 || b_tail == 0 || (b_full * S) % 8 != 0 || rest_grid >= R) return none;
+  const int64_t cap = std::min<int64_t>(CELL_TAIL_MAX_SEGMENTS, m_stages / std::max<int64_t>(min_seg, 1));
+  for (int64_t k = (R - rest_grid) / (b_tail * S); k >= 2; --k) {
+    const int64_t want = std::min<int64_t>(S * k, cap);
+    if (want <= S) break;
+    const int64_t seg = settle_segments(m_stages, (int)want);
+    if (seg % 8 == 0 && seg > S && seg <= cap && b_tail * seg + rest_grid <= R)
+      return {b_full, b_tail, (m_stages + seg - 1) / seg, (int)seg};
+  }
+  return none;
+}
+
+#ifndef KMVP_CELL_TAIL_AUTO
+#define KMVP_CELL_TAIL_AUTO 1
+#endif
+constexpr bool CELL_TAIL_AUTO = KMVP_CELL_TAIL_AUTO != 0;
+constexpr int CELL_TAIL_AUTO_TT = 8;
+constexpr int64_t CELL_TAIL_AUTO_N = 500000, CELL_TAIL_AUTO_M = 100000;
+constexpr bool cell_tail_taken(int opt, int tt, bool fused, int64_t N, int64_t M) {
+  return fused && tt > CELL_REST_TT &&
+         (opt > 0 || (opt < 0 && CELL_TAIL_AUTO && tt == CELL_TAIL_AUTO_TT && N >= CELL_TAIL_AUTO_N && M >= CELL_TAIL_AUTO_M));
+}
+
+inline int64_t cell_rest_weight(const CellSplit& s, int tt) {
+  const int64_t main_work = std::max<int64_t>(1, s.seg_stages[0] * tt);
+  return (s.grid(1) * s.seg_stages[1] * CELL_REST_TT + main_work - 1) / main_work;
+}
+
+inline bool cell_tail_split(CellSplit& s, int tt, int64_t resident, int64_t min_seg) {
+  const CellTail t = cell_tail_plan(s.blocks[0], s.segments[0], resident, s.m_stages, cell_rest_weight(s, tt), min_seg);
+  if (t.b_tail == 0) return false;
+  const int64_t block_slots = (int64_t)tt * WAVES_PER_BLOCK * CELL_TILE;
+  s.blocks[0] = t.b_full;
+  s.slots[0] = t.b_full * block_slots;
+  s.blocks[2] = t.b_tail;
+  s.slots[2] = t.b_tail * block_slots;
+  s.segments[2] = t.segments;
+  s.seg_stages[2] = t.seg_stages;
+  return true;
 }
 
 
@@ -303,6 +382,7 @@
   return D == 3 && f32 && tt == CELL_SHARED_TT && cap >= CELL_BALANCE_MIN_CAP;
 }
 constexpr int64_t CELLMM16_AUTO_N = 500000, CELLMM16_AUTO_M = 100000;
+static_assert(CELL_TAIL_AUTO_N == CELLMM16_AUTO_N && CELL_TAIL_AUTO_M == CELLMM16_AUTO_M, "one size rule");
 constexpr bool cell_balance_taken(int opt, bool applies, int64_t N, int64_t M) {
   return opt != 0 && applies && (opt > 0 || (N >= CELLMM16_AUTO_N && M >= CELLMM16_AUTO_M));
 }
diff --git a/kernel_matrix_benchmarks_amd/csrc/kmvp_product.hip b/kernel_matrix_benchmarks_amd/csrc/kmvp_product.hip
--- a/kernel_matrix_benchmarks_amd/csrc/kmvp_product.hip
+++ b/kernel_matrix_benchmarks_amd/csrc/kmvp_product.hip
@@ -1350,12 +1350,15 @@
 void cell_args(const kmvp_ctx* c, const CellSplit& s, int cols, int r, Args& a) {
   a.part = cell_region(c, s, cols, r);
   a.n_slots = s.slots[r];
-  a.tile_base = r ? c->cell_n_main : 0;
+  a.tile_base = s.slot_base(r) / CELL_TILE;
   a.seg_stages = s.seg_stages[r];
   a.segments = s.segments[r];
   a.tile_blocks = (int)s.blocks[r];
 }
-inline int cell_tt(const kmvp_ctx* c, int r) { return r ? CELL_REST_TT : c->cell_tt; }
+inline int cell_tt(const kmvp_ctx* c, int r) { return r == 1 ? CELL_REST_TT : c->cell_tt; }
+inline int64_t cell_tail_resident(const kmvp_ctx* c, int tt) {
+  return c->opt_cell_tail_resident > 0 ? c->opt_cell_tail_resident : (int64_t)c->device_cus * (tt >= 8 ? 2 : 4);
+}
 
 int pack_cell_targets(kmvp_ctx* c, const CellGrid& grid) {
   const int64_t n_tiles = c->cell_n_tiles;
@@ -1410,7 +1413,7 @@
   a.chunk_stages = std::max(1, c->opt_chunk / (CELL_TILE * CELL_STAGE_TILES));
   HIP_TRY(c, mark(c, 0));
   hipError_t le = hipSuccess;
-  for (int r = 0; r < 2 && le == hipSuccess; ++r)
+  for (int r = 0; r < CELL_LISTS && le == hipSuccess; ++r)
     if (s.blocks[r] > 0) {
       cell_args(c, s, NE, r, a);
       le = launch_cell_gaussian(sig, cell_tt(c, r), a, dim3((unsigned)s.grid(r)), c->stream, &c->last_kernel_name);
@@ -1421,11 +1424,11 @@
 
   if ((rc = ensure(c, c->sums, (size_t)NE * N * sizeof(double)))) return rc;
   if ((rc = ensure(c, c->cell_sums, (size_t)NE * n_slots * sizeof(double)))) return rc;
-  for (int r = 0; r < 2; ++r)
+  for (int r = 0; r < CELL_LISTS; ++r)
     if (s.blocks[r] > 0)
       hipLaunchKernelGGL(reduce_region_kernel, dim3(blocks_for((int64_t)NE * s.slots[r])), dim3(256), 0, c->stream,
                          (const double*)cell_region(c, s, NE, r), (double*)c->cell_sums.p, s.slots[r], NE, s.segments[r], n_slots,
-                         r ? s.slots[0] : (int64_t)0);
+                         s.slot_base(r));
   hipLaunchKernelGGL(gather_cells_kernel, dim3(blocks_for((int64_t)NE * N)), dim3(256), 0, c->stream,
                      (const double*)c->cell_sums.p, (const int*)c->cell_slot.p, (double*)c->sums.p, N, n_slots, NE);
   HIP_TRY(c, hipGetLastError());
@@ -1453,11 +1456,25 @@
   rule.min_seg = 2;
   rule.l2_seg_bytes = 3 << 20;
   rule.target_blocks = 7168;
-  const CellSplit s = cell_plan(c, CMM_STAGE_TILES, rule);
+  CellSplit s = cell_plan(c, CMM_STAGE_TILES, rule);
   const int64_t m_stages = s.m_stages, n_slots = s.n_slots;
   int rc;
   CellGrid grid;
   cell_load_grid(c, grid);
+  const int shape = c->opt_cellmm_shape >= 0 ? c->opt_cellmm_shape : ((TT >= 8 && c->N >= CELLMM16_AUTO_N && c->M >= CELLMM16_AUTO_M) ? 1 : 0);
+  FusedCellGrid fg = fused_cell_grid(s, TT, c->opt_cell_fused);
+  if (shape != 1) fg.fused = false;
+  const int64_t resident = cell_tail_resident(c, TT);
+  if ((CMM16_WHOLE_ROUNDS || cell_tail_taken(c->opt_cell_tail, TT, fg.fused, c->N, c->M)) && fg.fused &&
+      cell_tail_split(s, TT, resident, small_problem(N) ? 1 : rule.min_seg)) {
+    fg = fused_cell_grid(s, TT, 1);
+    c->note = std::string(c->note.empty() ? "" : c->note + "; ") + "tail list: the last " + std::to_string(s.blocks[2]) +
+              " target blocks in " + std::to_string(s.segments[2]) + " segments (cell_tail)";
+  }
+  {
+    const int64_t info[8] = {s.blocks[0], s.blocks[2], s.blocks[1], s.segments[0], s.segments[2], s.segments[1], resident, fg.fused ? 1 : 0};
+    memcpy(c->cell_list_info, info, sizeof info);
+  }
 
   const PackKey key = {LAYOUT_CELLMM, K_GAUSSIAN, TT};
   const int image_sig = NE > 1 ? -1 : sig;
@@ -1481,9 +1498,6 @@
   if ((rc = ensure(c, c->part, s.part_doubles(1) * sizeof(double)))) return rc;
   if ((rc = ensure(c, c->sums, (size_t)NE * N * sizeof(double)))) return rc;
   if ((rc = ensure(c, c->cell_sums, (size_t)NE * n_slots * sizeof(double)))) return rc;
-  const int shape = c->opt_cellmm_shape >= 0 ? c->opt_cellmm_shape : ((TT >= 8 && c->N >= CELLMM16_AUTO_N && c->M >= CELLMM16_AUTO_M) ? 1 : 0);
-  FusedCellGrid fg = fused_cell_grid(s, TT, c->opt_cell_fused);
-  if (shape != 1) fg.fused = false;
   CellmmArgs a;
   a.xd = (const float*)c->xs.p;
   a.tmeta = (const float*)c->cell_tmeta.p;
@@ -1509,12 +1523,13 @@
     }
     hipError_t le = hipSuccess;
     if (fg.fused) {
-      CellmmArgs ar = a;
+      CellmmArgs ar = a, at = a;
       cell_args(c, s, 1, 0, a);
       cell_args(c, s, 1, 1, ar);
-      le = launch_cellmm16_fused(TT, a, ar, fg.main_grid, fg.rest_grid, c->stream, &c->last_kernel_name);
+      cell_args(c, s, 1, 2, at);
+      le = launch_cellmm16_fused(TT, a, ar, at, fg.main_grid, fg.tail_grid, fg.rest_grid, c->stream, &c->last_kernel_name);
     } else {
-      for (int r = 0; r < 2 && le == hipSuccess; ++r)
+      for (int r = 0; r < CELL_LISTS && le == hipSuccess; ++r)
         if (s.blocks[r] > 0) {
           cell_args(c, s, 1, r, a);
           le = launch_cellmm_gaussian(cell_tt(c, r), shape, a, dim3((unsigned)s.grid(r)), c->stream, &c->last_kernel_name);
@@ -1524,10 +1539,10 @@
     HIP_TRY(c, le);
     if (NE == 1) HIP_TRY(c, mark(c, 1));
     double* col_sums = (double*)c->cell_sums.p + (size_t)col * n_slots;
-    for (int r = 0; r < 2; ++r)
+    for (int r = 0; r < CELL_LISTS; ++r)
       if (s.blocks[r] > 0)
         hipLaunchKernelGGL(reduce_segments_kernel, dim3(blocks_for(s.slots[r])), dim3(256), 0, c->stream,
-                           (const double*)cell_region(c, s, 1, r), col_sums + (r ? s.slots[0] : 0), s.slots[r], s.segments[r], 0);
+                           (const double*)cell_region(c, s, 1, r), col_sums + s.slot_base(r), s.slots[r], s.segments[r], 0);
     HIP_TRY(c, hipGetLastError());
   }
   if (NE > 1) HIP_TRY(c, mark(c, 1));
@@ -1952,6 +1967,22 @@
   if (target_cell) memcpy(target_cell, tcell.data(), (size_t)N * sizeof(int32_t));
   if (source_centres) memcpy(source_centres, scen.data(), scen.size() * sizeof(double));
   if (target_centres) memcpy(target_centres, tcen.data(), tcen.size() * sizeof(double));
+  return KMVP_OK;
+}
+
+int cell_lists_read(kmvp_ctx* c, int64_t* info, int32_t* target_list) {
+  if (!info) return fail(c, KMVP_E_INVALID, "kmvp_cell_lists: info is NULL");
+  if (!c->have_points || c->cell_state != 1 || c->cell_ver != c->points_ver || c->packed_points_ver != c->points_ver ||
+      c->packed_layout != LAYOUT_CELLMM)
+    return fail(c, KMVP_E_INVALID, "kmvp_cell_lists: no product on cellmm_kernel / cellmm16_kernel has run on the current points");
+  memcpy(info, c->cell_list_info, sizeof c->cell_list_info);
+  if (!target_list) return KMVP_OK;
+  std::vector<int> slot((size_t)c->N);
+  HIP_TRY(c, hipMemcpyAsync(slot.data(), c->cell_slot.p, (size_t)c->N * sizeof(int), hipMemcpyDeviceToHost, c->stream));
+  HIP_TRY(c, hipStreamSynchronize(c->stream));
+  const int64_t block_slots = (int64_t)c->cell_tt * WAVES_PER_BLOCK * CELL_TILE;
+  const int64_t main_end = info[0] * block_slots, tail_end = main_end + info[1] * block_slots;
+  for (int64_t i = 0; i < c->N; ++i) target_list[i] = slot[(size_t)i] < main_end ? 0 : (slot[(size_t)i] < tail_end ? 2 : 1);
   return KMVP_OK;
 }
 
```
